# haampie/Homogenization.jl

Hardware: AMD Instinct MI355X
Metric: fine-DOF updates/sec per V-cycle (3D Tet64) (higher is better)
Workload: dtype f64; 1 GPU; 3D Tet64 checkerboard, 32^3 unit cubes x 6 tets, refinements=5 (BASELINE config 3); cells=196608, nf=6545, levels=6, smoothing_steps=3, smoothing_steps_coarse=2, coarse_solver=device CG, Chebyshev(4)-of-Jacobi preconditioner, rtol 1e-13, spare_vector_bytes=10294394880, lazy_top_form=2

## Files before the change

homogenization.jl_amd/csrc/hmg_apply_small.hip:

```cpp
#include "hmg_device.hpp"
#include "hmg_stencil.hpp"

#include <algorithm>
#include <stdexcept>

namespace hmg {

namespace {
constexpr int SW = 15 * WAVE_ROW;

__device__ __forceinline__ uint32_t small_opaque_zero()
{
    uint32_t z;
    asm volatile("v_mov_b32 %0, 0" : "=v"(z));
    return z;
}
}

template <int SPT, bool FUSED>
__global__ void __launch_bounds__(64, SPT == 1 ? 5 : 4)
k_apply_small(LevelDev lv, const uint16_t *__restrict__ dmask, const int32_t *__restrict__ cell_class, ApplyArgs a)
{
    extern __shared__ double smem[];
    double *W = smem;
    double *xs = smem + SW + lv.lds_g0;
    const int lane = threadIdx.x, nf = lv.nf, m = lv.m;
    double *cs = xs + nf + lv.lds_g1;
    const int64_t ld = lv.ld;

    uint32_t pw[SPT], par[SPT];
    int lp[SPT];
    bool has[SPT];
#pragma unroll
    for (int q = 0; q < SPT; ++q) {
        const int t = lane + 64 * q;
        has[q] = t < nf;
        const int tc = has[q] ? t : nf - 1;
        pw[q] = lv.pos32[tc];
        lp[q] = (int)lv.lpos[tc];
        par[q] = FUSED && a.xcoarse ? lv.par32[tc] : 0u;
    }
    for (int q = lane; q < lv.lds_g0; q += 64) smem[SW + q] = 0.0;
    for (int q = lane; q < lv.lds_g1; q += 64) xs[nf + q] = 0.0;
    const bool neg = a.alpha < 0.0;
    double beta = 0.0, ax = 0.0, c2 = 0.0;
    if constexpr (FUSED) {
        beta = a.x2 ? a.scal[a.s_num] / a.scal[a.s_den] : 0.0;
        ax = a.xacc || a.x3 ? a.scal[a.a_num] / a.scal[a.a_den] : 0.0;
        c2 = a.x3 ? a.scal[a.c_num] / a.scal[a.c_den] : 0.0;
    }
    const bool xzero = FUSED && (a.flags & 128);
    const int64_t G = gridDim.x;
    auto cell_of = [&](int64_t blk) -> int64_t { return a.cell_list ? (int64_t)HMG_KP(int32_t, a.cell_list)[blk] : blk; };

    double pwv[4], pxv[SPT], px2[SPT], pxa[SPT], psv[SPT], pcv = 0.0;
    auto issue = [&](int64_t cell, int wsel) {
        const double *wc = lv.wcache + (size_t)wsel * WAVE_WSTRIDE;
#pragma unroll
        for (int q = 0; q < 4; ++q) pwv[q] = wc[lane + 64 * q < SW ? lane + 64 * q : SW - 1];
        const double *xc = a.x + cell * ld;
#pragma unroll
        for (int q = 0; q < SPT; ++q) {
            const int t = has[q] ? lane + 64 * q : nf - 1;
            pxv[q] = xzero ? 0.0 : xc[t];
            if (FUSED && a.x2) px2[q] = a.x2[cell * ld + t];
            if (FUSED && a.xacc)
                pxa[q] = a.xacc[cell * ld + t];
            else if (FUSED && a.x3)
                pxa[q] = a.x3[cell * ld + t];
            if (a.src) psv[q] = a.src[cell * ld + t];
        }
        if (FUSED && a.xcoarse) pcv = a.xcoarse[cell * a.ldc + (lane < lv.nf_coarse ? lane : lv.nf_coarse - 1)];
    };
    struct Uni {
        int wsel;
        uint32_t dm, mq[4];
    };
    auto uniform_of = [&](int64_t cell) {
        Uni u;
        u.wsel = 2 * HMG_KP(int32_t, cell_class)[cell] + (neg ? 1 : 0);
        u.dm = 0u;
        if (a.flags & 1) {
            const uint32_t w2 = HMG_KP(uint32_t, dmask)[cell >> 1];
            u.dm = (cell & 1) ? w2 >> 16 : w2 & 0xffffu;
        }
#pragma unroll
        for (int q = 0; q < 4; ++q) u.mq[q] = FUSED && a.mult ? HMG_KP(uint32_t, a.mult)[cell * 4 + q] : 0x01010101u;
        return u;
    };

    int64_t blk = blockIdx.x;
    if (blk >= a.nwork) return;
    int64_t cell = cell_of(blk);
    Uni cur = uniform_of(cell);
    issue(cell, cur.wsel);
    int64_t cell_n = blk + G < a.nwork ? cell_of(blk + G) : cell;
    Uni nxt = uniform_of(cell_n);

    for (;;) {
        double rr = 0.0, pap = 0.0, sv[SPT];
#pragma unroll
        for (int q = 0; q < 4; ++q)
            if (lane + 64 * q < SW) W[lane + 64 * q] = pwv[q];
        double v[SPT];
        if constexpr (FUSED) {
            if (a.xcoarse && lane < lv.nf_coarse) cs[lane] = pcv;
#pragma unroll
            for (int q = 0; q < SPT; ++q) {
                const int t = lane + 64 * q;
                double val = pxv[q];
                if (a.xcoarse) {
                    const uint32_t pa = par[q] & 0xffffu, pb = par[q] >> 16;
                    const double ca = lds_ld(cs + pa), cb = lds_ld(cs + pb);
                    const double vi = val + ca;
                    double vm = val;
                    vm += 0.5 * ca;
                    vm = vm + 0.5 * cb;
                    val = pa == pb ? vi : vm;
                }
                if (a.xacc && has[q]) a.xacc[cell * ld + t] = axpy1(ax, px2[q], pxa[q]);
                if (a.x3) {
                    const double t1 = axpy1(ax, px2[q], val);
                    const double p2 = axpy1(beta, px2[q], pxa[q]);
                    val = axpy1(c2, p2, t1);
                } else if (a.x2)
                    val = axpy1(beta, px2[q], val);
                if (a.xout && has[q]) a.xout[cell * ld + t] = val;
                if (!has[q]) val = 0.0;
                rr += val * val;
                v[q] = val;
            }
        } else {
#pragma unroll
            for (int q = 0; q < SPT; ++q) v[q] = pxv[q];
        }
#pragma unroll
        for (int q = 0; q < SPT; ++q) {
            if (has[q]) xs[lp[q]] = v[q];
            sv[q] = a.src ? psv[q] : 0.0;
        }
        const Uni me = cur;
        const int64_t mycell = cell;
        const bool more = blk + G < a.nwork;
        if (more) {
            issue(cell_n, nxt.wsel);
            cell = cell_n;
            cur = nxt;
            cell_n = blk + 2 * G < a.nwork ? cell_of(blk + 2 * G) : cell_n;
            nxt = uniform_of(cell_n);
        }
        double *oc = a.out ? a.out + mycell * ld : nullptr;
#pragma unroll
        for (int q = 0; q < SPT; ++q) {
            const uint32_t word = pw[q] | small_opaque_zero();
            int L, len, A, B, cls;
            decode32<3>(word, m, L, len, A, B, cls);
            double ctr;
            double o = stencil_eval_c<3>(W + cls * WAVE_ROW, xs, L, len, A, B, ctr);
            o = sv[q] + o;
            if (cls > 0 && ((me.dm >> (cls - 1)) & 1u)) o = 0.0;
            if (has[q] && (!FUSED || oc)) oc[lane + 64 * q] = o;
            if (FUSED && has[q]) {
                uint32_t mu = 1u;
                if (cls > 0) {
                    const int e = cls - 1;
                    const uint32_t wd = e < 4 ? me.mq[0] : e < 8 ? me.mq[1] : e < 12 ? me.mq[2] : me.mq[3];
                    mu = (wd >> (8 * (e & 3))) & 0xffu;
                }
                pap += (double)mu * (ctr * o);
            }
        }
        if constexpr (FUSED) {
            const double s_pap = wave_sum63(pap), s_rr = wave_sum63(rr);
            if (lane == 63) {
                a.blockpart[2 * mycell] = s_pap;
                a.blockpart[2 * mycell + 1] = s_rr;
            }
        }
        if (!more) break;
        blk += G;
    }
}


template <bool FUSED>
__global__ void __launch_bounds__(64, 4)
k_apply_pack(LevelDev lv, const uint16_t *__restrict__ dmask, const int32_t *__restrict__ cell_class, ApplyArgs a)
{
    extern __shared__ double smem[];
    const int lane = threadIdx.x, sub = lane >> 4, t = lane & 15, nf = lv.nf, m = lv.m;
    const bool has = t < nf;
    const int tc = has ? t : nf - 1;
    const int imgp = lv.lds_g0 + nf + lv.lds_g1;
    double *xs = smem + sub * imgp + lv.lds_g0;
    const int64_t ld = lv.ld;
    for (int q = lane; q < 4 * imgp; q += 64) smem[q] = 0.0;

    int L, len, A, B, cls;
    decode32<3>(lv.pos32[tc], m, L, len, A, B, cls);
    const int lp = (int)lv.lpos[tc];
    const uint32_t par = FUSED && a.xcoarse ? lv.par32[tc] : 0u;
    const int pa = (int)(par & 0xffffu), pb = (int)(par >> 16);
    const int e = cls > 0 ? cls - 1 : 0;
    const bool neg = a.alpha < 0.0;
    double beta = 0.0, ax = 0.0, c2 = 0.0;
    if constexpr (FUSED) {
        beta = a.x2 ? a.scal[a.s_num] / a.scal[a.s_den] : 0.0;
        ax = a.xacc || a.x3 ? a.scal[a.a_num] / a.scal[a.a_den] : 0.0;
        c2 = a.x3 ? a.scal[a.c_num] / a.scal[a.c_den] : 0.0;
    }
    const bool xzero = FUSED && (a.flags & 128);
    const int64_t G = gridDim.x, nquad = (a.nwork + 3) >> 2;

    struct Meta {
        int cell, wsel;
        uint32_t dm, mw;
        bool valid;
    };
    auto meta_of = [&](int64_t Q) {
        Meta mt;
        int64_t w = 4 * Q + sub;
        mt.valid = w < a.nwork;
        if (!mt.valid) w = a.nwork - 1;
        mt.cell = a.cell_list ? a.cell_list[w] : (int)w;
        mt.wsel = 2 * cell_class[mt.cell] + (neg ? 1 : 0);
        mt.dm = (a.flags & 1) ? (uint32_t)dmask[mt.cell] : 0u;
        mt.mw = FUSED && a.mult && cls > 0 ? (uint32_t)a.mult[(int64_t)mt.cell * 16 + e] : 1u;
        return mt;
    };
    double2 pw2[8];
    double pxv = 0.0, px2 = 0.0, pxa = 0.0, psv = 0.0, pca = 0.0, pcb = 0.0;
    auto issue = [&](const Meta &mt) {
        const double2 *wr = reinterpret_cast<const double2 *>(lv.wcache + (size_t)mt.wsel * WAVE_WSTRIDE + cls * WAVE_ROW);
#pragma unroll
        for (int q = 0; q < 8; ++q) pw2[q] = wr[q];
        const int64_t o = (int64_t)mt.cell * ld + tc;
        pxv = xzero ? 0.0 : a.x[o];
        if (FUSED && a.x2) px2 = a.x2[o];
        if (FUSED && a.xacc)
            pxa = a.xacc[o];
        else if (FUSED && a.x3)
            pxa = a.x3[o];
        if (a.src) psv = a.src[o];
        if (FUSED && a.xcoarse) {
            pca = a.xcoarse[(int64_t)mt.cell * a.ldc + pa];
            pcb = a.xcoarse[(int64_t)mt.cell * a.ldc + pb];
        }
    };

    int64_t Q = blockIdx.x;
    if (Q >= nquad) return;
    Meta cur = meta_of(Q);
    issue(cur);
    Meta nxt = meta_of(Q + G < nquad ? Q + G : Q);

    for (;;) {
        const Meta me = cur;
        const int64_t o = (int64_t)me.cell * ld + t;
        const bool live = has && me.valid;
        double w[16];
#pragma unroll
        for (int q = 0; q < 8; ++q) {
            w[2 * q] = pw2[q].x;
            w[2 * q + 1] = pw2[q].y;
        }
        double val = pxv, rr = 0.0, pap = 0.0;
        if constexpr (FUSED) {
            if (a.xcoarse) {
                const double ca = pca, cb = pcb;
                const double vi = val + ca;
                double vm = val;
                vm += 0.5 * ca;
                vm = vm + 0.5 * cb;
                val = pa == pb ? vi : vm;
            }
            if (a.xacc && live) a.xacc[o] = axpy1(ax, px2, pxa);
            if (a.x3) {
                const double t1 = axpy1(ax, px2, val);
                const double p2 = axpy1(beta, px2, pxa);
                val = axpy1(c2, p2, t1);
            } else if (a.x2)
                val = axpy1(beta, px2, val);
            if (a.xout && live) a.xout[o] = val;
            if (!has) val = 0.0;
            rr += val * val;
        }
        if (has) xs[lp] = val;
        const double sv = a.src ? psv : 0.0;
        const bool more = Q + G < nquad;
        if (more) {
            issue(nxt);
            cur = nxt;
            nxt = meta_of(Q + 2 * G < nquad ? Q + 2 * G : Q + G);
        }
        auto at = [&](int off) { return lds_ld(xs + max(L + off, 0)); };
        const double ctr = lds_ld(xs + L);
        double acc = w[0] * ctr;
        acc += w[1] * lds_ld(xs + L + 1);
        acc += w[2] * at(-1);
        acc += w[3] * lds_ld(xs + L + len - 1);
        acc += w[4] * at(-len);
        acc += w[5] * lds_ld(xs + L + len);
        acc += w[6] * at(-len - 1);
        acc += w[7] * lds_ld(xs + L + A - len);
        acc += w[8] * at(len + 1 - B);
        acc += w[9] * lds_ld(xs + L + A - 1);
        acc += w[10] * at(1 - B);
        acc += w[11] * lds_ld(xs + L + A);
        acc += w[12] * at(-B);
        acc += w[13] * lds_ld(xs + L + A + 1 - len);
        acc += w[14] * at(len - B);
        double out = sv + acc;
        if (cls > 0 && ((me.dm >> (cls - 1)) & 1u)) out = 0.0;
        if (live && (!FUSED || a.out)) a.out[o] = out;
        if constexpr (FUSED) {
            if (has) {
                const uint32_t mu = me.mw;
                pap += (double)mu * (ctr * out);
            }
            pap = dpp_add<0x111, 0xf>(pap);
            rr = dpp_add<0x111, 0xf>(rr);
            pap = dpp_add<0x112, 0xf>(pap);
            rr = dpp_add<0x112, 0xf>(rr);
            pap = dpp_add<0x114, 0xf>(pap);
            rr = dpp_add<0x114, 0xf>(rr);
            pap = dpp_add<0x118, 0xf>(pap);
            rr = dpp_add<0x118, 0xf>(rr);
            if (t == 15 && me.valid) {
                a.blockpart[2 * (int64_t)me.cell] = pap;
                a.blockpart[2 * (int64_t)me.cell + 1] = rr;
            }
        }
        if (!more) break;
        Q += G;
    }
}

bool apply_small_ok(const Launch &L, const LevelDev &lv, const MeshDev &mesh, const ApplyArgs &a, bool fused)
{
    if (!L.apply_small || L.apply_threads != 0) return false;
    if (!L.weight_cache || !lv.wcache || !mesh.cell_class) return false;
    if (lv.dim != 3 || lv.ncls != 15 || lv.nf > 192 || lv.nf < 4 || lv.m > 63 || !lv.pos32 || !lv.lpos) return false;
    if (a.flags & (2 | 8 | 16)) return false;
    if (!(a.alpha == 1.0 || a.alpha == -1.0) || a.lambda != mesh.wc_lambda) return false;
    if (a.rcoarse) return false;
    if (!fused) return !a.xcoarse;
    if ((a.x3 || a.xacc) && !a.x2) return false;
    if (a.x3 && a.xacc) return false;
    if (a.xcoarse && (!lv.par32 || lv.nf_coarse < 1 || lv.nf_coarse > 64 || !a.xout || a.x2 || a.xacc || a.x3)) return false;
    return true;
}

void launch_apply_small(const Launch &L, const LevelDev &lv, const MeshDev &mesh, const ApplyArgs &a0, bool fused)
{
    ApplyArgs a = a0;
    const int64_t nblocks = a.cell_list ? a.ncell_list : a.ncells_prefix ? a.ncells_prefix : mesh.ncells;
    if (nblocks == 0) return;
    if (!a.x) throw std::runtime_error("operator apply: null input vector");
    if (!fused && !a.out) throw std::runtime_error("operator apply: a plain launch needs an output vector");
    if (fused && (!a.blockpart || !a.scal)) throw std::runtime_error("operator apply: fused launch without its reduction scratch");
    if ((a.flags & 1) && !mesh.dmask) throw std::runtime_error("operator apply: constraint requested without a Dirichlet mask");
    if ((a.flags & 128) && !(fused && a.x3 && a.x2 && a.xout && !a.xcoarse))
        throw std::runtime_error("operator apply: the zero-input form exists for the residual with two pending x-updates only");
    a.nwork = nblocks;
    if (lv.nf <= 16 && L.apply_pack && nblocks >= 4 && nblocks < (int64_t(1) << 31)) {
        const int64_t nquad = (nblocks + 3) / 4;
        const dim3 gq((unsigned)std::min<int64_t>(nquad, (int64_t)16 * L.num_cu)), bq(64);
        const size_t ldsq = sizeof(double) * (size_t)(4 * (lv.lds_g0 + lv.nf + lv.lds_g1) + 64);
        if (fused)
            hipLaunchKernelGGL((k_apply_pack<true>), gq, bq, ldsq, L.stream, lv, mesh.dmask, mesh.cell_class, a);
        else
            hipLaunchKernelGGL((k_apply_pack<false>), gq, bq, ldsq, L.stream, lv, mesh.dmask, mesh.cell_class, a);
        check_launch();
        if (L.n_small_launches) *L.n_small_launches += 1;
        return;
    }
    const int64_t grid = std::min<int64_t>(nblocks, (int64_t)(lv.nf > 64 ? 16 : 20) * L.num_cu);
    const size_t lds = sizeof(double) * (size_t)(SW + lv.lds_g0 + lv.nf + lv.lds_g1 + 64);
    const dim3 g((unsigned)grid), b(64);
    if (lv.nf > 64) {
        if (fused)
            hipLaunchKernelGGL((k_apply_small<3, true>), g, b, lds, L.stream, lv, mesh.dmask, mesh.cell_class, a);
        else
            hipLaunchKernelGGL((k_apply_small<3, false>), g, b, lds, L.stream, lv, mesh.dmask, mesh.cell_class, a);
    } else {
        if (fused)
            hipLaunchKernelGGL((k_apply_small<1, true>), g, b, lds, L.stream, lv, mesh.dmask, mesh.cell_class, a);
        else
            hipLaunchKernelGGL((k_apply_small<1, false>), g, b, lds, L.stream, lv, mesh.dmask, mesh.cell_class, a);
    }
    check_launch();
    if (L.n_small_launches) *L.n_small_launches += 1;
}

}
```

homogenization.jl_amd/csrc/hmg_apply_wave.hip:

```cpp
#include "hmg_device.hpp"
#include "hmg_stencil.hpp"

#include <algorithm>
#include <stdexcept>
#include <type_traits>

namespace hmg {

namespace {

__device__ __forceinline__ uint32_t opaque_zero()
{
    uint32_t z;
    asm volatile("v_mov_b32 %0, 0" : "=v"(z));
    return z;
}

__device__ __forceinline__ void wdecode(uint32_t w, int &L, int &len, int &A, int &B)
{
    L = (int)(w & 1023u);
    len = (int)((w >> 10) & 31u);
    A = (int)((w >> 15) & 255u);
    B = (int)((w >> 23) & 255u);
}
// ... 246 lines not shown
                using T_ = std::true_type;
                using F_ = std::false_type;
                if (x3c) {
                    if (xzero)
                        general(F_{}, T_{}, T_{}, std::integral_constant<int, 8>{});
                    else
                        general(F_{}, T_{}, F_{}, std::integral_constant<int, 8>{});
                } else if (xac)
                    general(T_{}, F_{}, F_{}, std::integral_constant<int, 8>{});
                else
                    general(F_{}, F_{}, F_{}, std::integral_constant<int, 16>{});
            }
        }

        double *oc = a.out ? a.out + cell * ld : nullptr;
        double kf[8], kec[2], ki[3][WR];
        __builtin_amdgcn_sched_barrier(0);
        issue_src_interior();
        __builtin_amdgcn_sched_barrier(0);
        {
            const double fm0 = (double)(mq[0] & 0xffu), fm1 = (double)((mq[0] >> 8) & 0xffu), fm2 = (double)((mq[0] >> 16) & 0xffu),
                         fm3 = (double)(mq[0] >> 24);
            wave_face<0, FUSED, FUSED && !RS, SRC>(wc + 1 * WAVE_ROW, xs, TW(0), TW(1), (dm >> 0) & 1u, fm0, sf[0], sf[1], oc, pap, lane, kf[0], kf[1]);
            wave_face<1, FUSED, FUSED && !RS, SRC>(wc + 2 * WAVE_ROW, xs, TW(2), TW(3), (dm >> 1) & 1u, fm1, sf[2], sf[3], oc, pap, lane, kf[2], kf[3]);
            wave_face<2, FUSED, FUSED && !RS, SRC>(wc + 3 * WAVE_ROW, xs, TW(4), TW(5), (dm >> 2) & 1u, fm2, sf[4], sf[5], oc, pap, lane, kf[4], kf[5]);
            wave_face<3, FUSED, FUSED && !RS, SRC>(wc + 4 * WAVE_ROW, xs, TW(6), TW(7), (dm >> 3) & 1u, fm3, sf[6], sf[7], oc, pap, lane, kf[6], kf[7]);
        }
#pragma unroll
        for (int r = 0; r < 2; ++r) {
            const int t = r * 64 + lane;
            const bool valid = t < WNEC;
            const int cls = (int)((TW(14) >> (16 + 8 * r)) & 0xffu);
            const double sv = SRC ? sec[r] : 0.0;
            int L, len, A, B;
            wdecode(TW(8 + r), L, len, A, B);
            double ctr;
            double o = stencil_eval_c<3>(smem + (cls - 5) * WAVE_ROW, xs, L, len, A, B, ctr);
            o = sv + o;
            if ((dm >> (cls - 1)) & 1u) o = 0.0;
            if (valid && (!FUSED || oc)) oc[t] = o;
            if (FUSED && !RS && valid) {
                const int e = cls - 1;
                const uint32_t word = e < 4 ? mq[0] : e < 8 ? mq[1] : e < 12 ? mq[2] : mq[3];
                const uint32_t mu = (word >> (8 * (e & 3))) & 0xffu;
                pap += (double)mu * (ctr * o);
            }
            kec[r] = o;
        }
        {
            double w0[15];
#pragma unroll
            for (int d = 0; d < 15; ++d) w0[d] = wc[d];
#pragma unroll
            for (int r = 0; r < 3; ++r) {
                const uint32_t word = TW(10 + r);
                const int slot0 = (int)(r == 0 ? TW(13) & 0xffffu : r == 1 ? TW(13) >> 16 : TW(14) & 0xffffu);
                if (r < 2 || lane < WNBLK - 128) {
                    const int nv = (int)(word >> 28);
#pragma unroll
                    for (int q = 0; q < WR; ++q) ki[r][q] = SRC && q < nv ? si[r][q] : 0.0;
                    interior_block_core<WR, FUSED, false, RS>(w0, xs, WM, WNF >> 1, word, slot0, oc, pap, ki[r]);
                }
            }
        }

        if constexpr (RS) {
#pragma unroll
            for (int f = 0; f < 8; ++f)
                if (!(f & 1) || lane < WNFI - 64) xs[TW(f) & 1023u] = kf[f];
#pragma unroll
            for (int r = 0; r < 2; ++r)
                if (r * 64 + lane < WNEC) xs[TW(8 + r) & 1023u] = kec[r];
#pragma unroll
            for (int r = 0; r < 3; ++r)
                if (r < 2 || lane < WNBLK - 128) {
                    int pos[WR];
                    block_positions<WR>(WM, TW(10 + r), pos);
                    const int nv = (int)(TW(10 + r) >> 28);
#pragma unroll
                    for (int q = 0; q < WR; ++q)
                        if (q < nv) xs[pos[q]] = ki[r][q];
                }
            double *rc = a.rcoarse + cell * a.ldrc;
#pragma unroll
            for (int q = 0; q < 3; ++q) {
                const int c = lane + 64 * q;
                if (c < WNFC) {
                    const uint4 ta = reinterpret_cast<const uint4 *>(lv.wave_rs)[2 * c];
                    const uint4 tb = reinterpret_cast<const uint4 *>(lv.wave_rs)[2 * c + 1];
                    const uint32_t e[8] = {ta.x, ta.y, ta.z, ta.w, tb.x, tb.y, tb.z, tb.w};
                    const int n = (int)(e[7] >> 16);
                    double tmp = 0.0;
                    tmp += 1.0 * lds_ld(xs + (e[0] & 0xffffu));
#pragma unroll
                    for (int u = 1; u < 15; ++u) {
                        const double t2 = tmp + 0.5 * lds_ld(xs + ((u & 1) ? e[u >> 1] >> 16 : e[u >> 1] & 0xffffu));
                        tmp = u < n ? t2 : tmp;
                    }
                    rc[c] = tmp;
                }
            }
        }
        if (FUSED && !RS) {
            const double s_pap = wave_sum63(pap), s_rr = wave_sum63(rr);
            if (lane == 63) {
                a.blockpart[2 * cell] = s_pap;
                a.blockpart[2 * cell + 1] = s_rr;
            }
        }
    }
}

__global__ void __launch_bounds__(256)
k_weight_cache(LevelDev lv, const double *__restrict__ coef_rep, int64_t nsets, double lambda, double *__restrict__ wcache)
{
    for (int64_t set = blockIdx.x; set < nsets; set += gridDim.x) {
        const int64_t cls = set >> 1;
        const double alpha = (set & 1) ? -1.0 : 1.0;
        double s[7];
        cell_scales<3>(coef_rep + (size_t)cls * 8, alpha, lambda, s, 0);
        double *out = wcache + (size_t)set * WAVE_WSTRIDE;
        for (int idx = threadIdx.x; idx < 15 * WAVE_ROW; idx += 256) {
            const int c = idx / WAVE_ROW, d = idx % WAVE_ROW;
            double w = 0.0;
            if (c < lv.ncls && d < 15) {
                const double *ct = lv.ctab + ((size_t)c * 15 + d) * 7;
#pragma unroll
                for (int t = 0; t < 7; ++t) w += ct[t] * s[t];
            }
            out[idx] = w;
        }
    }
}

void launch_weight_cache(const Launch &L, const LevelDev &lv, const double *coef_rep, int nclasses, double lambda, double *wcache)
{
    if (nclasses <= 0) return;
    if (lv.dim != 3 || lv.ncls != 15 || lv.ndir != 15 || lv.nterm != 7) throw std::runtime_error("weight cache: not a 3D level");
    const int64_t nsets = 2 * (int64_t)nclasses;
    const int64_t grid = std::min<int64_t>(nsets, (int64_t)1 << 20);
    hipLaunchKernelGGL(k_weight_cache, dim3((unsigned)grid), dim3(256), 0, L.stream, lv, coef_rep, nsets, lambda, wcache);
    check_launch();
}

bool apply_wave_ok(const Launch &L, const LevelDev &lv, const MeshDev &mesh, const ApplyArgs &a, bool fused)
{
    if (!L.apply_wave || L.apply_threads != 0) return false;
    if (!lv.wave_tab || !lv.wave_lpos || !lv.wcache || !mesh.cell_class) return false;
    if (lv.dim != 3 || lv.m != WM || lv.nf != WNF || lv.nfi != WNFI || lv.nei != WNEI || lv.ncorner != WNCORNER || lv.nedge != 6 ||
        lv.nface != 4 || lv.nblk != WNBLK || lv.blk_R != WR || lv.off_edge != WOFF_EDGE || lv.off_face != WOFF_FACE ||
        lv.lds_g0 != 0 || lv.lds_g1 < WM + 8 || lv.lds_g1 > 64 || lv.ncls != 15)
        return false;
    if (a.flags & (2 | 8 | 16)) return false;
    if (!(a.alpha == 1.0 || a.alpha == -1.0) || a.lambda != mesh.wc_lambda) return false;
    if (!fused) return !a.xcoarse && !a.rcoarse;
    if (a.xcoarse && a.rcoarse) return false;
    if ((a.x3 || a.xacc) && !(a.x2 && a.xout)) return false;
    if (a.xcoarse) return a.src && a.xout && lv.wave_par && lv.wave_cl && lv.nf_coarse == WNFC && !a.x2 && !a.xacc && !a.x3;
    if (a.rcoarse) return a.src && lv.wave_rs && lv.nf_coarse == WNFC;
    return true;
}

void launch_apply_wave(const Launch &L, const LevelDev &lv, const MeshDev &mesh, const ApplyArgs &a0, bool fused)
{
    ApplyArgs a = a0;
    const int64_t nblocks = a.cell_list ? a.ncell_list : a.ncells_prefix ? a.ncells_prefix : mesh.ncells;
    if (nblocks == 0) return;
    if (!a.x) throw std::runtime_error("operator apply: null input vector");
    if (!fused && !a.out) throw std::runtime_error("operator apply: a plain launch needs an output vector");
    if (fused && (!a.blockpart || !a.scal)) throw std::runtime_error("operator apply: fused launch without its reduction scratch");
    if ((a.flags & 1) && !mesh.dmask) throw std::runtime_error("operator apply: constraint requested without a Dirichlet mask");
    if (a.xcoarse && !a.xout) throw std::runtime_error("operator apply: folded prolongation without xout");
    if (a.rcoarse && a.ldrc <= 0) throw std::runtime_error("operator apply: epilogue restriction without the coarse column stride");
    if ((a.flags & 128) && !(fused && a.x3 && a.x2 && a.xout && !a.xcoarse))
        throw std::runtime_error("operator apply: the zero-input form exists for the residual with two pending x-updates only");
    a.nwork = nblocks;
    if (L.cell_order && !a.cell_list && !a.ncells_prefix && mesh.cell_perm) {
        a.cell_list = mesh.cell_perm;
        a.ncell_list = nblocks;
    }
    int64_t grid = std::min<int64_t>(nblocks, L.wave_grid > 0 ? L.wave_grid : 16 * (int64_t)L.num_cu);
    if (grid >= 8) grid -= grid % 8;
    const size_t lds = sizeof(double) * (size_t)(WVZ + WNF + lv.lds_g1);
    const dim3 g((unsigned)grid), b(64);
#define HMG_WAVE_LAUNCH(F, C, R, S) \
    hipLaunchKernelGGL((k_apply_wave<F, C, R, S>), g, b, lds, L.stream, lv, mesh.dmask, mesh.cell_class, a)
    if (!fused) {
        if (a.src)
            HMG_WAVE_LAUNCH(false, false, false, true);
        else
            HMG_WAVE_LAUNCH(false, false, false, false);
    } else if (a.xcoarse)
        HMG_WAVE_LAUNCH(true, true, false, true);
    else if (a.rcoarse)
        HMG_WAVE_LAUNCH(true, false, true, true);
    else if (a.src)
        HMG_WAVE_LAUNCH(true, false, false, true);
    else
        HMG_WAVE_LAUNCH(true, false, false, false);
#undef HMG_WAVE_LAUNCH
    check_launch();
    if (L.n_wave_launches) *L.n_wave_launches += 1;
}

}
```

homogenization.jl_amd/csrc/hmg_context.cpp:

```cpp
#include "../../include/hmg.h"
#include "hmg_objects.hpp"

#include <algorithm>

namespace hmg {

std::recursive_mutex &lifetime_mutex()
{
    static std::recursive_mutex m;
    return m;
}

std::atomic<int64_t> &device_allocs()
{
    static std::atomic<int64_t> n{0};
    return n;
}

namespace {

void vec_pool_trim(hmg_ctx *c)
{
    LifetimeLock lock(lifetime_mutex());
    if (c->vec_pool.empty()) return;
// ... 97 lines not shown
}

}

void grid_unref(hmg_grid *grid)
{
    LifetimeLock lock(lifetime_mutex());
    if (!grid || --grid->refs > 0) return;
    hmg_ctx *c = grid->ctx;
    if (c) {
        (void)hipSetDevice(c->device);
        (void)hipStreamSynchronize(c->stream);
    }
    probe_unlist(grid);
    release_top_spare(grid);
    release_weight_cache(grid);
    release_smoother_diag(grid);
    if (grid->probe && grid->probe->h) (void)hipHostFree(grid->probe->h);
    if (grid->probe && grid->probe->ev) (void)hipEventDestroy(grid->probe->ev);
    delete grid;
    ctx_unref(c);
}

double read_scalar(hmg_ctx *c, int slot)
{
    double h = 0.0;
    HIPCHK(hipMemcpyAsync(&h, c->L.scal + slot, sizeof(double), hipMemcpyDeviceToHost, c->stream));
    HIPCHK(hipStreamSynchronize(c->stream));
    judge_probes(c);
    return h;
}

}

extern "C" {

const char *hmg_last_error(void) { return last_error().c_str(); }
int hmg_version(void) { return 1; }

static int ctx_create(int device, void *stream, bool use_given, hmg_ctx **out)
{
    HMG_TRY
    need(out != nullptr, "null out pointer");
    int ndev = 0;
    hipError_t e = hipGetDeviceCount(&ndev);
    if (e != hipSuccess || ndev == 0)
        throw std::runtime_error("no HIP device available: libhmg_hip needs an MI355X (gfx950); there is no CPU fallback");
    need(device >= 0 && device < ndev, "device index out of range");
    HIPCHK(hipSetDevice(device));
    std::unique_ptr<hmg_ctx> c(new hmg_ctx);
    c->device = device;
    if (use_given) {
        c->stream = (hipStream_t)stream;
    } else {
        HIPCHK(hipStreamCreateWithFlags(&c->stream, hipStreamNonBlocking));
        c->own_stream = true;
    }
    hipDeviceProp_t prop;
    HIPCHK(hipGetDeviceProperties(&prop, device));
    c->partials.alloc(4096);
    c->scal.alloc(S_COUNT);
    HIPCHK(hipMemsetAsync(c->scal.p, 0, S_COUNT * sizeof(double), c->stream));
    c->L.stream = c->stream;
    c->L.partials = c->partials.p;
    c->L.rpart = nullptr;
    c->L.rpart_cap = 0;
    c->L.scal = c->scal.p;
    c->L.num_cu = prop.multiProcessorCount > 0 ? prop.multiProcessorCount : 256;
    c->L.apply_threads = 0;
    c->L.apply_mass_only = 0;
    c->L.cell_order = 1;
    c->L.weight_cache = 1;
    c->L.apply_wave = 1;
    c->L.wave_grid = 16 * (int64_t)c->L.num_cu;
    c->L.n_wave_launches = &c->wave_launches;
    c->L.apply_slab2 = 1;
    c->L.n_slab2_launches = &c->slab2_launches;
    c->L.n_rows_launches = &c->rows_launches;
    c->L.slab2_grid = 0;
    c->L.slab2_force = 0;
    c->L.restrict_slab2 = 1;
    c->L.apply_pack = 1;
    c->L.apply_small = 1;
    c->L.n_small_launches = &c->small_launches;
    c->L.n_wc_launches = &c->wc_launches;
    c->L.apply_wg512 = 1;
    {
        LifetimeLock lock(lifetime_mutex());
        live_contexts().push_back(c.get());
    }
    *out = c.release();
    HMG_END
}

int hmg_ctx_create(int device, void *stream, hmg_ctx **out) { return ctx_create(device, stream, stream != nullptr, out); }

int hmg_ctx_create_on_stream(int device, void *stream, hmg_ctx **out) { return ctx_create(device, stream, true, out); }

int hmg_ctx_destroy(hmg_ctx *ctx)
{
    HMG_TRY
    ctx_unref(ctx);
    HMG_END
}

int hmg_ctx_sync(hmg_ctx *ctx)
{
    HMG_TRY
    need(ctx != nullptr, "null ctx");
    HIPCHK(hipStreamSynchronize(ctx->stream));
    judge_probes(ctx);
    HMG_END
}

int64_t hmg_ctx_counter(hmg_ctx *ctx, const char *name)
{
    if (!ctx || !name) return -1;
    const std::string n(name);
    if (n == "wave_launches") return ctx->wave_launches;
    if (n == "slab2_launches") return ctx->slab2_launches;
    if (n == "rows_launches") return ctx->rows_launches;
    if (n == "small_launches") return ctx->small_launches;
    if (n == "weight_cache_launches") return ctx->wc_launches;
    if (n == "comm_calls") return ctx->comm_calls;
    if (n == "device_allocs") return device_allocs().load();
    if (n == "spare_bytes") return ctx->spare_bytes;
    if (n == "weight_cache_classes") return ctx->wc_classes;
    if (n == "weight_cache_bytes") return ctx->wc_bytes;
    if (n == "weight_cache_refusals") return ctx->wc_refusals;
    if (n == "fcg_bytes") return ctx->fcg_bytes;
    if (n == "smoother_diag_bytes") return ctx->smoother_diag_bytes;
    if (n == "smoother_diag_builds") return ctx->smoother_diag_builds;
    if (n == "lazy_top_form") return ctx->last_top_form;
    if (n == "lazy_pre_form") return ctx->last_pre_form;
    if (n == "coarse_x_folds") return ctx->coarse_x_folds;
    if (n == "cell_moments_kernel_ns") return ctx->moments_kernel_ns;
    if (n == "cell_moments_download_ns") return ctx->moments_download_ns;
    if (n == "comm_nranks") return ctx->comm ? ctx->comm_nranks : 0;
    return -1;
}

int hmg_ctx_release_memory(hmg_ctx *ctx)
{
    HMG_TRY
    need(ctx != nullptr, "null ctx");
    vec_pool_trim(ctx);
    HMG_END
}

int hmg_ctx_set_option(hmg_ctx *ctx, const char *name, int64_t value)
{
    HMG_TRY
    need(ctx && name, "null argument");
    std::string n(name);
    static const std::pair<const char *, bool hmg_ctx::*> flags[] = {
        {"coarse_probe", &hmg_ctx::coarse_probe}, {"fuse_cg", &hmg_ctx::fuse_cg_default}, {"fold_x", &hmg_ctx::fold_x},
        {"swap_rp", &hmg_ctx::swap_rp}, {"fold_prolong", &hmg_ctx::fold_prolong}, {"zero_entry", &hmg_ctx::zero_entry},
        {"fold_restrict", &hmg_ctx::fold_restrict}, {"lazy_dead", &hmg_ctx::lazy_dead}, {"lazy_pre", &hmg_ctx::lazy_pre}, {"fold_coarse_x", &hmg_ctx::fold_coarse_x}, {"fold_faces", &hmg_ctx::fold_faces},
        {"lean_post", &hmg_ctx::lean_post}, {"lazy_post", &hmg_ctx::lazy_post}, {"prolong_in_image", &hmg_ctx::prolong_in_image},
        {"comm_rehearsal", &hmg_ctx::comm_rehearsal}};
    for (const auto &f : flags)
        if (n == f.first) {
            ctx->*f.second = value != 0;
            return 0;
        }
    if (n == "apply_threads")
        ctx->L.apply_threads = (int)value;
    else if (n == "apply_wg512")
        ctx->L.apply_wg512 = value != 0;
    else if (n == "apply_pack")
        ctx->L.apply_pack = value != 0;
    else if (n == "apply_small")
        ctx->L.apply_small = value != 0;
    else if (n == "weight_cache")
        ctx->L.weight_cache = value != 0;
    else if (n == "weight_cache_classes")
        ctx->wc_max_classes = std::max<int64_t>(0, value);
    else if (n == "apply_slab2")
        ctx->L.apply_slab2 = value != 0;
    else if (n == "restrict_slab2")
        ctx->L.restrict_slab2 = value != 0;
    else if (n == "slab2_force")
        ctx->L.slab2_force = value != 0;
    else if (n == "slab2_grid")
        ctx->L.slab2_grid = std::max<int64_t>(0, value);
    else if (n == "apply_wave")
        ctx->L.apply_wave = value != 0;
    else if (n == "wave_grid")
        ctx->L.wave_grid = std::max<int64_t>(1, value) * (int64_t)ctx->L.num_cu;
    else if (n == "wave_grid_total")
        ctx->L.wave_grid = std::max<int64_t>(1, value);
    else if (n == "cell_order")
        ctx->L.cell_order = value != 0;
    else if (n == "coarse_poly")
        ctx->coarse_poly = std::max<int>(1, std::min<int>(16, (int)value));
    else if (n == "coarse_maxit")
        ctx->coarse_maxit = (int)value;
    else if (n == "coarse_check")
        ctx->coarse_check = std::max<int>(1, (int)value);
    else if (n == "lazy_top")
        ctx->lazy_top = (int)value;
    else if (n == "overlap_min_doubles")
        ctx->overlap_min_doubles = value;
    else if (n == "vec_pool") {
        ctx->vec_pool_on = value != 0;
        if (!ctx->vec_pool_on) vec_pool_trim(ctx);
    }
    else if (n == "time_apply") {
        ctx->timer.on = value > 0;
        ctx->timer.min_level = (int)value;
        ctx->timer.used = 0;
        ctx->timer.ev_level.clear();
        ctx->timer.ev_bytes.clear();
    }
    else
        throw std::runtime_error("unknown option: " + n);
    HMG_END
}

int hmg_ctx_set_option_f64(hmg_ctx *ctx, const char *name, double value)
{
    HMG_TRY
    need(ctx && name, "null argument");
    std::string n(name);
    if (n == "coarse_rtol")
        ctx->coarse_rtol = value;
    else if (n == "coarse_poly_ratio")
        ctx->coarse_poly_ratio = value;
    else
        throw std::runtime_error("unknown option: " + n);
    HMG_END
}

void *hmg_ctx_scalar_bank(hmg_ctx *ctx) { return ctx ? (void *)ctx->L.scal : nullptr; }

int hmg_ctx_set_scalar_bank(hmg_ctx *ctx, void *device_doubles16)
{
    HMG_TRY
    need(ctx != nullptr, "null argument");
    HIPCHK(hipStreamSynchronize(ctx->stream));
    double *to = device_doubles16 ? (double *)device_doubles16 : ctx->scal.p;
    if (to != ctx->L.scal) HIPCHK(hipMemcpy(to, ctx->L.scal, S_COUNT * sizeof(double), hipMemcpyDeviceToDevice));
    ctx->L.scal = to;
    HMG_END
}

static int apply_timing(hmg_ctx *ctx, bool every, int level, int64_t *launches, double *total_ms, double *total_bytes)
{
    HMG_TRY
    need(ctx && launches && total_ms && total_bytes, "null argument");
    HIPCHK(hipStreamSynchronize(ctx->stream));
    const ApplyTimer &tm = ctx->timer;
    double ms = 0.0, by = 0.0;
    int64_t n = 0;
// ... 93 lines not shown
```

homogenization.jl_amd/csrc/hmg_device.hpp:

```cpp
#pragma once
#include <hip/hip_runtime.h>

#include <cstdint>

namespace hmg {

constexpr int TABLE_PAD = 3 * 1024;

__host__ __device__ inline int rows_slot(int m, int i, int j, int nei, int off_int, int &cls)
{
    if (j == 0) {
        cls = i == 0 ? 4 : i == m ? 5 : 1;
        return i == 0 ? 0 : i == m ? 1 : 3 + i - 1;
    }
    if (i == 0) {
        cls = j == m ? 6 : 2;
        return j == m ? 2 : 3 + nei + j - 1;
    }
    if (i + j == m) {
        cls = 3;
        return 3 + 2 * nei + j - 1;
    }
    cls = 0;
    return off_int + (j - 1) * (m - 1) - (((j - 1) * j) >> 1) + i - 1;
}

struct LevelDev {
    int dim, level, m;
    int nf, ld;
    int ncorner, nedge, nface;
    int nei, nfi, nint;
    int off_edge, off_face, off_int;
    int ncls, ndir, nterm;
    int lds_g0, lds_g1;
    int nf_coarse;
    const uint64_t *meta;
    const uint16_t *lpos;
    const uint16_t *sweep_slot;
    int nsweep;
    const uint32_t *pos32;
    const uint32_t *pos32w;
    const uint32_t *sweep32;
    const uint32_t *blk_word;
    const uint16_t *blk_slot;
    int nblk, blk_R;
    const double *ctab;
    const int32_t *hier2slot;
    const int32_t *par_a, *par_b;
    const uint32_t *par32;
    const uint64_t *par64;
    const uint16_t *clpos;
    const uint32_t *rs_word;
    const double *rs_w;
    const uint16_t *rs_lp;
    const int32_t *rptr, *ridx;
    const double *dphi;
    const uint32_t *wave_tab;
    const uint32_t *wave_lpos;
    const uint32_t *wave_par;
    const uint32_t *wave_cl;
    const uint32_t *wave_rs;
    const double *wcache;
};

constexpr int WM = 16, WNF = 969, WNFI = 105, WNEI = 15, WNCORNER = 4, WNBLK = 152, WNFC = 165, WR = 4;
constexpr int WOFF_EDGE = 4, WOFF_FACE = 94, WNEC = 94;
constexpr int WNQ = 16;
constexpr int WVZ = 168;
constexpr int WAVE_TAB_ROWS = 15;
constexpr int WAVE_ROW = 16;
constexpr int WAVE_WSTRIDE = 15 * WAVE_ROW;

struct SlabTables {
    const int *head;
    const uint32_t *ld_word;
    const uint32_t *cp_word;
    const uint16_t *cp_slot;
    int nslab, lds_nodes;
    int max_surf;
    int max_int;
};

struct MeshDev {
    int dim;
    int64_t ncells, nnodes;
    const int32_t *cells;
    const int32_t *face_pairs;
    int64_t nfacepairs;
    const int32_t *face_partner;
    const int32_t *edge_ptr, *edge_ent;
    int64_t nsharededges;
    const int32_t *node_ptr, *node_ent;
    int64_t nsharednodes;
    const int32_t *node_first;
    const uint16_t *dmask, *dupmask;
    const double *coef;
    int64_t ncut_edge_groups, ncut_node_groups;
    int64_t ncut_face_pairs;
    const int32_t *cells_cut, *cells_inner;
    const int32_t *cell_perm;
    int64_t ncells_cut, ncells_inner;
    const uint8_t *mult;
    const int32_t *cell_class;
    int nclasses;
    double wc_lambda;
    double *blockpart;
    SlabTables slab;
};

struct ApplyArgs {
    double alpha, lambda;
    const double *x;
    const double *x2;
    double *xout;
    double *xacc;
    int a_num, a_den;
    const double *x3;
    int c_num, c_den;
    const double *x4;
    int d_num, d_den;
    const double *xcoarse;
    int64_t ldc;
    const double *xc_p, *xc_r;
    const double *src;
    double *out;
    double *rcoarse;
    int64_t ldrc;
    const double *scal;
    int s_num, s_den;
    double *blockpart;
    const uint8_t *mult;
    int flags;
    int64_t ncells_prefix;
    int64_t out_ld;
    const int32_t *cell_list;
    int64_t ncell_list;
    int64_t nwork;
    const int32_t *cell_class;
};

struct CoarseDev {
    int64_t n;
    const int32_t *rowptr, *colidx;
    const double *val, *diag;
    const int32_t *interior;
};

enum { S_RS = 0, S_PAP = 1, S_RS2 = 2, S_TMP = 3, S_C0 = 4, S_C1 = 5, S_C2 = 6, S_C3 = 7, S_PAP2 = 8, S_DONE = 9, S_ITER = 10,
       S_CRR = 11, S_HOST = 12, S_COUNT = 16,
       S_RS3 = S_C1, S_PAP3 = S_TMP };

struct Launch {
    hipStream_t stream;
    double *partials;
    double *rpart;
    int64_t rpart_cap;
    double *scal;
    int num_cu;
    int apply_threads;
    int apply_mass_only;
    int apply_wg512;
    int cell_order;
    int weight_cache;
    int apply_pack;
    int apply_small;
    int64_t *n_small_launches;
    int64_t *n_wc_launches;
    int apply_wave;
    int64_t wave_grid;
    int64_t *n_wave_launches;
    int apply_slab2;
    int64_t *n_slab2_launches;
    int64_t slab2_grid;
    int restrict_slab2;
    int slab2_force;
    int64_t *n_rows_launches;
};

void launch_apply(const Launch &L, const LevelDev &lv, const MeshDev &mesh, double alpha, double lambda,
                  const double *x, const double *src, double *out, int use_mask);
size_t apply_lds_bytes(const LevelDev &lv);
bool apply_restricts(const Launch &L, const LevelDev &lv);
bool apply_folds_coarse_x(const Launch &L, const LevelDev &lv);
bool apply_defers3(const Launch &L, const LevelDev &lv);
void launch_apply_fused_kernel(const Launch &L, const LevelDev &lv, const MeshDev &mesh, ApplyArgs a);
void launch_apply_fused_reduce(const Launch &L, const MeshDev &mesh, int slot_pap, int slot_rr);
void launch_apply_args(const Launch &L, const LevelDev &lv, const MeshDev &mesh, ApplyArgs a);
bool apply_wave_ok(const Launch &L, const LevelDev &lv, const MeshDev &mesh, const ApplyArgs &a, bool fused);
void launch_apply_wave(const Launch &L, const LevelDev &lv, const MeshDev &mesh, const ApplyArgs &a, bool fused);
bool apply_slab2_ok(const Launch &L, const LevelDev &lv, const MeshDev &mesh, const ApplyArgs &a);
void launch_apply_slab2(const Launch &L, const LevelDev &lv, const MeshDev &mesh, const ApplyArgs &a, bool fused);
void launch_apply_rows(const Launch &L, const LevelDev &lv, const MeshDev &mesh, const ApplyArgs &a, bool fused, bool wd);
void launch_prolong_add_wide(const Launch &L, const LevelDev &fine, const LevelDev &coarse, int64_t ncells, const double *xc,
                             double *xf);
int64_t launch_norm2_unique_wide(const Launch &L, const LevelDev &lv, const MeshDev &mesh, const double *x);
bool apply_small_ok(const Launch &L, const LevelDev &lv, const MeshDev &mesh, const ApplyArgs &a, bool fused);
void launch_apply_small(const Launch &L, const LevelDev &lv, const MeshDev &mesh, const ApplyArgs &a, bool fused);
void launch_weight_cache(const Launch &L, const LevelDev &lv, const double *coef_rep, int nclasses, double lambda, double *wcache);

void launch_interface_sum(const Launch &L, const LevelDev &lv, const MeshDev &mesh, double *x, int which = 0,
                          bool faces = true);
void launch_mask(const Launch &L, const LevelDev &lv, const MeshDev &mesh, double *x, int which );
void launch_restrict_slab(const Launch &L, const LevelDev &fine_rtab, const MeshDev &mesh, const SlabTables &st, int ldc,
                          const double *rf, double *bc);
void launch_restrict(const Launch &L, const LevelDev &fine, const LevelDev &coarse, int64_t ncells,
                     const double *rf, double *bc);
void launch_prolong_add(const Launch &L, const LevelDev &fine, const LevelDev &coarse, int64_t ncells,
                        const double *xc, double *xf);

void launch_fill(const Launch &L, double *x, int64_t n, double v);
void launch_copy(const Launch &L, double *dst, const double *src, int64_t n);
void launch_axpy(const Launch &L, double a, const double *x, double *y, int64_t n);
void launch_xpby(const Launch &L, const double *r, double b, double *p, int64_t n);
void launch_dot(const Launch &L, const double *x, const double *y, int64_t n, int slot);
void launch_norm2_unique(const Launch &L, const LevelDev &lv, const MeshDev &mesh, const double *x, int slot);
void launch_copy_dot(const Launch &L, double *p, const double *r, int64_t n, int slot);
void launch_cg_update(const Launch &L, double *x, double *r, const double *p, const double *q, int64_t n,
                      int s_num, int s_den, int s_out);
void launch_cg_rupdate(const Launch &L, const double *r, double *rout, const double *q, int64_t n, int s_num, int s_den,
                       int s_out);
void launch_cg_rupdate_faces(const Launch &L, const LevelDev &lv, const MeshDev &mesh, const double *r, double *rout,
                             const double *q, int64_t n, int s_num, int s_den, int s_out);
void launch_cg_rupdate_faces_x(const Launch &L, const LevelDev &lv, const MeshDev &mesh, const double *r, double *rout,
                               const double *q, int64_t n, int s_num, int s_den, int s_out, double *x, const double *p, int a_num,
                               int a_den, int b_num, int b_den, const double *p0, int z_num, int z_den);
void launch_cg_xp_update(const Launch &L, double *x, double *p, const double *r, int64_t n, int a_num, int a_den,
                         int s_num, int s_den, int with_p);
void launch_cg_x2_update(const Launch &L, double *x, const double *p, const double *r, int64_t n, int a_num, int a_den, int b_num,
                         int b_den, int c_num, int c_den);
void launch_cg_pupdate(const Launch &L, double *p, const double *r, int64_t n, int s_num, int s_den);

void launch_gather_base(const Launch &L, const MeshDev &mesh, int ld1, const double *v1, double *u);
void launch_scatter_base(const Launch &L, const MeshDev &mesh, int ld1, const double *u, double *v1);

void launch_gather_owned(const Launch &L, const MeshDev &mesh, const int32_t *nodes_g, const int32_t *owned, int ld1,
                         const double *v1, double *ug);
void launch_scatter_cells(const Launch &L, const int32_t *cell_nodes, int64_t ncells, int npc, int ld1, const double *u,
                          double *v1);

void launch_permute(const Launch &L, const LevelDev &lv, int64_t ncells, const double *src, double *dst,
                    int to_storage);
void launch_fill_random(const Launch &L, const LevelDev &lv, int64_t ncells, double *x, uint64_t seed,
                        int64_t cell_offset);

void launch_coarse_gather_rhs(const Launch &L, const CoarseDev &A, const double *u, double *b);
void launch_coarse_scatter_sol(const Launch &L, const CoarseDev &A, int64_t nnodes, const double *x, double *u);
void launch_coarse_init(const Launch &L, const CoarseDev &A, const double *b, double *x, double *r, double *z,
                        double *p, double zscale = 1.0, double *dcheb = nullptr);
void launch_coarse_cheb(const Launch &L, const CoarseDev &A, const double *r, const double *zin, double *zout, double *d, double c1,
                        double c2, int last);
void launch_coarse_rz_from_cheb(const Launch &L, const CoarseDev &A);
void launch_coarse_update(const Launch &L, const CoarseDev &A, double *x, double *r, double *z, const double *p,
                          const double *q, int slot_old, double zscale = 1.0, double *dcheb = nullptr);
void launch_coarse_residual_norm(const Launch &L, const CoarseDev &A);
void launch_coarse_direction(const Launch &L, const CoarseDev &A, double *p, double *q, const double *z, int slot_old, int slot_new,
                             double rtol2, int mode, int count_it, int rz_from_cheb = 0);

void launch_rhs_dphi(const Launch &L, const LevelDev &lv, int64_t ncells, const double *pvec, double *b);

void launch_integrate(const Launch &L, const LevelDev &lv, const MeshDev &mesh, int mode, int64_t nsub, const double *v,
                      const double *second, int slot);
void launch_integrate_load(const Launch &L, const LevelDev &lv, const MeshDev &mesh, int64_t nsub, const double *v,
                           const double *load, int slot);

struct CutPackArgs {
    int64_t n[3];
    const int64_t *pos[3];
    const int32_t *cell_lid[3];
    const uint8_t *first[3];
};
void launch_cut_pack(const Launch &L, const LevelDev &lv, const CutPackArgs &c, double *buf, double *x, int unpack);
void launch_seg_sum(const Launch &L, const int64_t *plan, int64_t ndoubles, double *buf, const double *stage);

}
```

homogenization.jl_amd/csrc/hmg_host.hpp:

```cpp
#pragma once
#include <algorithm>
#include <cstdint>
#include <string>
#include <thread>
#include <vector>

namespace hmg {

int setup_threads();

template <class F>
void parallel_for(int64_t n, F f)
{
    const int T = (int)std::max<int64_t>(1, std::min<int64_t>(setup_threads(), n / 4096));
    if (T == 1) {
        f((int64_t)0, n);
        return;
    }
    std::vector<std::thread> th;
    for (int t = 0; t < T; ++t) th.emplace_back([&, t] { f(n * t / T, n * (t + 1) / T); });
    for (auto &x : th) x.join();
}

template <class T, class Cmp>
// ... 68 lines not shown
    int dim = 0;
    int64_t nnodes = 0, ncells = 0;
    std::vector<double> coords;
    std::vector<int32_t> cells;

    std::vector<int32_t> face_pairs;
    std::vector<int32_t> edge_ptr, edge_ent;
    std::vector<int32_t> node_ptr, node_ent;
    std::vector<int32_t> node_first;
    std::vector<int32_t> node_all_ptr, node_all_ent;
    std::vector<uint16_t> dmask, dupmask;
    std::vector<uint8_t> mult;
    std::vector<uint8_t> node_on_boundary;

    int64_t ncut_edge_groups = 0, ncut_node_groups = 0;
    int64_t ncut_face_pairs = 0;
    std::vector<int32_t> cells_cut, cells_inner;

    std::vector<double> detj, jinv;
};

void build_mesh_tables(int dim, int64_t nnodes, const double *coords, int64_t ncells,
                       const int64_t *cells_1based, MeshTables &out);

void restrict_mesh_tables(const MeshTables &full, int64_t ncells_prefix, int64_t nnodes_prefix,
                          MeshTables &out);

inline int sym_ncomp(int dim) { return dim * (dim + 1) / 2; }
inline int sym_index(int dim, int a, int b)
{
    if (a > b) std::swap(a, b);
    return a * dim - a * (a - 1) / 2 + (b - a);
}
void build_cell_coefficients(const MeshTables &mesh, const double *sigma, int sn, std::vector<double> &coef);

struct CoarseMatrix {
    int64_t n = 0;
    std::vector<int32_t> interior;
    std::vector<int32_t> node2int;
    std::vector<int32_t> rowptr, colidx;
    std::vector<double> val, diag;
};
void assemble_coarse_matrix(const MeshTables &mesh, const double *sigma, int sn, double lambda,
                            CoarseMatrix &out);


struct AddressTables {
    std::vector<uint16_t> lpos;
    std::vector<uint32_t> pos32;
    std::vector<uint32_t> pos32w;
    std::vector<uint32_t> sweep32;
    std::vector<uint16_t> sweep_slot;
};
AddressTables build_address_tables(const LevelTables &T);

struct BlockedInterior {
    int nblk = 0, R = 0;
    std::vector<uint32_t> word;
    std::vector<uint16_t> slot;
};
BlockedInterior build_blocked_interior(const LevelTables &T);

struct SlabWindows {
    int nslab = 0, lds_nodes = 0, max_surf = 0, max_int = 0;
    std::vector<int> head;
    std::vector<uint32_t> ld_word;
    std::vector<uint32_t> cp_word;
    std::vector<uint16_t> cp_slot;
    int rs_max_surf = 0, rs_max_int = 0;
    std::vector<int> rs_head;
    std::vector<uint32_t> rs_word;
    std::vector<uint16_t> rs_slot;
    std::vector<double> rtab;
};
SlabWindows build_slab_windows(const LevelTables &T, const LevelTables *coarse, int lds_kb);

struct TransferTables {
    std::vector<uint32_t> par32;
    std::vector<uint16_t> clpos;
    std::vector<uint64_t> par64;
    std::vector<uint32_t> rs_word;
    std::vector<double> rs_w;
    std::vector<uint16_t> rs_lp;
};
TransferTables build_transfer_tables(const LevelTables &T, const LevelTables *coarse, const BlockedInterior &blk);

struct WaveTables {
    std::vector<uint32_t> tab, lpos, par, cl, rs;
};
WaveTables build_wave_tables(const LevelTables &T, const LevelTables *coarse, const BlockedInterior &blk,
                             const std::vector<uint16_t> &clpos);

struct MeshKernelTables {
    std::vector<int32_t> face_partner;
    std::vector<uint16_t> dmask;
    std::vector<int32_t> cell_perm;
    std::vector<int32_t> cells_cut, cells_inner;
};
MeshKernelTables build_mesh_kernel_tables(const MeshTables &M, bool xcd_lists);

struct Partition {
    int rank = 0, nranks = 1;
    MeshTables global;
    std::vector<int32_t> cells_g;
    std::vector<int32_t> nodes_g;
    std::vector<int32_t> owned_node;
    int64_t nglobal[3] = {0, 0, 0};
    std::vector<int64_t> gid[3];
    std::vector<int32_t> cell_lid[3];
    bool global_ids = true;
    struct Segment {
        std::vector<int32_t> members;
        int64_t count[3] = {0, 0, 0};
    };
    std::vector<Segment> segs;
    std::vector<int32_t> seg_of[3];
    std::vector<int64_t> seg_idx[3];
};

void build_partition(int dim, int64_t nnodes, const double *coords, int64_t ncells, const int64_t *cells_1based,
                     const int32_t *owner, int rank, int nranks, MeshTables &local, Partition &part,
                     const int32_t *cut_owner = nullptr, bool halo_only = false);

std::string &last_error();

}
```

homogenization.jl_amd/csrc/hmg_kernel_tables.cpp:

```cpp
#include "hmg_device.hpp"
#include "hmg_host.hpp"

#include <algorithm>
#include <numeric>
#include <stdexcept>
#include <utility>

namespace hmg {

namespace {

uint32_t word32w(uint32_t i, uint32_t j, uint32_t k, uint32_t c) { return (i & 127u) | (j & 127u) << 7 | (k & 127u) << 14 | c << 21; }

uint32_t word_lattice(uint32_t L, uint32_t j, uint32_t k) { return L | ((j & 127u) << 16) | ((k & 127u) << 23); }

uint32_t lattice_pos(const LevelTables &T, int slot) { return (uint32_t)(T.meta[(size_t)slot] & 0xffffu); }

struct LatticeIndex {
    int n;
    std::vector<int32_t> slot;
    explicit LatticeIndex(const LevelTables &T) : n(T.m + 1), slot((size_t)n * n * (T.dim == 3 ? n : 1), -1)
    {
        for (int q = 0; q < T.nf; ++q) slot[idx(T.slot_ijk[3 * q], T.slot_ijk[3 * q + 1], T.slot_ijk[3 * q + 2])] = q;
    }
// ... 127 lines not shown
    for (int e = 0; e < T.nedge; ++e) seg.push_back({T.off_edge + e * T.nei, T.off_edge + (e + 1) * T.nei});
    for (int f = 0; f < T.nface; ++f) seg.push_back({T.off_face + f * T.nfi, T.off_face + (f + 1) * T.nfi});
    seg.push_back({T.off_int, T.nf});
    auto run = [&](std::pair<int, int> sg, int ka, int kb) {
        auto in = [&](int t) { return T.slot_ijk[3 * t + 2] >= ka && T.slot_ijk[3 * t + 2] < kb; };
        int b = sg.second, e = sg.first;
        for (int t = sg.first; t < sg.second; ++t)
            if (in(t)) { b = std::min(b, t); e = t + 1; }
        for (int t = b; t < e; ++t)
            if (!in(t)) throw std::runtime_error("apply slabs: plane range is not contiguous");
        return b < e ? std::make_pair(b, e) : std::make_pair(0, 0);
    };
    S.head.assign((size_t)S.nslab * 8, 0);
    for (int sl = 0; sl < S.nslab; ++sl) {
        S.head[sl * 8 + 0] = sk[sl];
        S.head[sl * 8 + 1] = (int)S.ld_word.size();
        for (const auto &sg : seg) {
            const auto ld = run(sg, sl == 0 ? 0 : sk[sl] + 1, sk[sl + 1] + 1);
            for (int t = ld.first; t < ld.second; ++t) S.ld_word.push_back(lattice_pos(T, t) | ((uint32_t)t << 16));
        }
        S.head[sl * 8 + 2] = (int)S.ld_word.size() - S.head[sl * 8 + 1];
    }
    auto eval_lists = [&](std::vector<int> &head, std::vector<uint32_t> &word, std::vector<uint16_t> &slot, int &max_surf,
                          int &max_int, auto out) {
        for (int sl = 0; sl < S.nslab; ++sl) {
            int *h = &head[(size_t)sl * 8];
            h[3] = (int)word.size();
            for (size_t si = 0; si < seg.size(); ++si) {
                const bool interior = si + 1 == seg.size();
                if (interior) h[5] = (int)word.size() - h[3];
                const auto cp = run(seg[si], sk[sl], sk[sl + 1]);
                for (int t = cp.first; t < cp.second; ++t) {
                    const int o = out(t);
                    if (o < 0) continue;
                    const uint32_t i = T.slot_ijk[3 * t], j = T.slot_ijk[3 * t + 1], k = T.slot_ijk[3 * t + 2];
                    word.push_back(interior ? word_lattice(lattice_pos(T, t), j, k) : word32w(i, j, k, T.slot_cls[t]));
                    slot.push_back((uint16_t)o);
                }
            }
            h[4] = (int)word.size() - h[3];
            max_surf = std::max(max_surf, h[5]);
            max_int = std::max(max_int, h[4] - h[5]);
        }
    };
    eval_lists(S.head, S.cp_word, S.cp_slot, S.max_surf, S.max_int, [](int t) { return t; });
    if ((int)S.ld_word.size() != T.nf || (int)S.cp_word.size() != T.nf)
        throw std::runtime_error("apply slabs: the slab lists do not cover the cell exactly once");
    for (int sl = 0; sl < S.nslab; ++sl)
        for (int q = S.head[sl * 8 + 3] + S.head[sl * 8 + 5] + 1; q < S.head[sl * 8 + 3] + S.head[sl * 8 + 4]; ++q)
            if (S.cp_slot[(size_t)q] != S.cp_slot[(size_t)q - 1] + 1)
                throw std::runtime_error("apply slabs: interior slots of a slab are not consecutive");
    S.ld_word.resize(S.ld_word.size() + TABLE_PAD, 0u);
    S.cp_word.resize(S.cp_word.size() + TABLE_PAD, 0u);
    S.cp_slot.resize(S.cp_slot.size() + TABLE_PAD, (uint16_t)0);
    if (!coarse) return S;
    const LatticeIndex cslot(*coarse);
    S.rs_head = S.head;
    eval_lists(S.rs_head, S.rs_word, S.rs_slot, S.rs_max_surf, S.rs_max_int, [&](int t) {
        const int i = T.slot_ijk[3 * t], j = T.slot_ijk[3 * t + 1], k = T.slot_ijk[3 * t + 2];
        if ((i | j | k) & 1) return -1;
        const int cs = cslot(i / 2, j / 2, k / 2);
        if (cs < 0) throw std::runtime_error("slab restriction: even node without a coarse slot");
        return cs;
    });
    if ((int)S.rs_word.size() != coarse->nf) throw std::runtime_error("slab restriction: lists do not cover the coarse cell");
    S.rs_word.resize(S.rs_word.size() + TABLE_PAD, 0u);
    S.rs_slot.resize(S.rs_slot.size() + TABLE_PAD, (uint16_t)0);
    S.rtab.assign(T.ctab.size(), 0.0);
    for (int c = 0; c < T.ncls; ++c)
        for (int d = 0; d < T.ndir; ++d) S.rtab[((size_t)c * T.ndir + d) * T.nterm + T.nterm - 1] = restriction_weight(T, c, d);
    return S;
}

TransferTables build_transfer_tables(const LevelTables &T, const LevelTables *coarse, const BlockedInterior &blk)
{
    TransferTables X;
    if (!coarse || coarse->nf <= 0x10000) {
        X.par32.resize(T.par_a.size());
        for (size_t q = 0; q < X.par32.size(); ++q) {
            if ((uint32_t)T.par_a[q] > 0xffffu || (uint32_t)T.par_b[q] > 0xffffu) throw std::runtime_error("coarse slot exceeds 16 bits");
            X.par32[q] = (uint32_t)T.par_a[q] | ((uint32_t)T.par_b[q] << 16);
        }
    }
    if (!(coarse && T.dim == 3 && blk.nblk > 0 && T.nf <= 0xffff)) return X;
    const LevelTables &C = *coarse;
    const LatticeIndex fslot(T);
    X.clpos.resize((size_t)C.nf);
    X.rs_word.resize((size_t)C.nf);
    for (int c = 0; c < C.nf; ++c) {
        const int i = 2 * C.slot_ijk[3 * c], j = 2 * C.slot_ijk[3 * c + 1], k = 2 * C.slot_ijk[3 * c + 2];
        const int fs = fslot(i, j, k);
        if (fs < 0) throw std::runtime_error("prolongation tables: coarse node without a fine lattice node");
        if (i > 127 || j > 127 || k > 127) throw std::runtime_error("restriction tables: bad coarse node");
        X.clpos[c] = (uint16_t)lattice_pos(T, fs);
        X.rs_word[c] = word32w(i, j, k, T.slot_cls[fs]);
    }
    X.par64.resize((size_t)T.nf);
    for (int q = 0; q < T.nf; ++q) {
        const uint64_t a = X.clpos[(size_t)T.par_a[q]], b = X.clpos[(size_t)T.par_b[q]], self = lattice_pos(T, q);
        if (T.par_a[q] == T.par_b[q] && a != self) throw std::runtime_error("prolongation tables: identity row off its node");
        X.par64[q] = a | (b << 16) | (self << 32);
    }
    X.rs_w.resize((size_t)T.ncls * T.ndir);
    for (int c = 0; c < T.ncls; ++c)
        for (int d = 0; d < T.ndir; ++d) X.rs_w[(size_t)c * T.ndir + d] = restriction_weight(T, c, d);
    if (T.nf <= 2048) {
        X.rs_lp.resize(T.ridx.size());
        for (size_t e = 0; e < X.rs_lp.size(); ++e) X.rs_lp[e] = (uint16_t)lattice_pos(T, T.ridx[e]);
    }
    return X;
}

WaveTables build_wave_tables(const LevelTables &T, const LevelTables *coarse, const BlockedInterior &blk,
                             const std::vector<uint16_t> &clpos)
{
    WaveTables W;
    if (!(T.dim == 3 && T.m == WM && T.nf == WNF && blk.nblk == WNBLK && blk.R == WR && T.lds_g0 == 0 && T.nfi == WNFI &&
          T.nei == WNEI && T.ncorner == WNCORNER && T.nedge == 6 && T.nface == 4 && T.off_edge == WOFF_EDGE &&
          T.off_face == WOFF_FACE))
        return W;
    const int m = T.m, WDUMMY = WVZ - 1;
    auto surf_word = [&](int t, bool valid) -> uint32_t {
        const uint32_t L = lattice_pos(T, t);
        const int j = T.slot_ijk[3 * t + 1], k = T.slot_ijk[3 * t + 2];
        const int len = m + 1 - j - k, n = m - k, Tk = (n + 1) * (n + 2) / 2, A = Tk - j, Bo = Tk + n + 2 - j;
        if (L > 1023u || len < 0 || len > 31 || A < 0 || A > 255 || Bo < 0 || Bo > 255)
            throw std::runtime_error("wave tables: addressing word out of range");
        return L | ((uint32_t)len << 10) | ((uint32_t)A << 15) | ((uint32_t)Bo << 23) | (valid ? 1u << 31 : 0u);
    };
    W.tab.assign((size_t)WAVE_TAB_ROWS * 64, 0u);
    W.lpos.assign(8 * 64, 0u);
    for (int l = 0; l < 64; ++l) {
        for (int r = 0; r < 8; ++r) {
            const int f = r >> 1, ti = (r & 1) * 64 + l;
            const bool valid = ti < WNFI;
            W.tab[(size_t)r * 64 + l] = surf_word(WOFF_FACE + f * WNFI + (valid ? ti : 0), valid);
        }
        uint32_t cls[2];
        for (int r = 0; r < 2; ++r) {
            const int t = r * 64 + l;
            const bool valid = t < WNEC;
            W.tab[(size_t)(8 + r) * 64 + l] = surf_word(valid ? t : 0, valid);
            cls[r] = T.slot_cls[(size_t)(valid ? t : WOFF_EDGE)];
            if (cls[r] < 5 || cls[r] > 14) throw std::runtime_error("wave tables: edge / corner class out of range");
        }
        uint32_t bsl[3];
        for (int r = 0; r < 3; ++r) {
            const int u = r * 64 + l;
            const bool valid = u < WNBLK;
            W.tab[(size_t)(10 + r) * 64 + l] = valid ? blk.word[(size_t)u] : (blk.word[0] & 0x0fffffffu);
            bsl[r] = blk.slot[(size_t)(valid ? u : 0)];
        }
        W.tab[(size_t)13 * 64 + l] = bsl[0] | (bsl[1] << 16);
        W.tab[(size_t)14 * 64 + l] = bsl[2] | (cls[0] << 16) | (cls[1] << 24);
        for (int q = 0; q < WNQ; ++q) {
            const int t = l + 64 * q;
            W.lpos[(size_t)(q / 2) * 64 + l] |= 8u * (uint32_t)(t < WNF ? WVZ + (int)lattice_pos(T, t) : WDUMMY) << (16 * (q & 1));
        }
    }
    if (!(coarse && !clpos.empty() && coarse->nf == WNFC)) return W;
    W.par.assign(16 * 64, 0u);
    W.cl.assign(3 * 64, 8u * (uint32_t)WDUMMY);
    W.rs.assign((size_t)192 * 8, 0u);
    for (int t = 0; t < T.nf; ++t) W.par[(size_t)t] = (uint32_t)clpos[(size_t)T.par_a[t]] | ((uint32_t)clpos[(size_t)T.par_b[t]] << 16);
    for (int c = 0; c < coarse->nf; ++c) {
        W.cl[(size_t)c] = 8u * (uint32_t)(WVZ + clpos[(size_t)c]);
// ... 31 lines not shown
```

homogenization.jl_amd/csrc/hmg_kernels.hip:

```cpp
#include "hmg_device.hpp"
#include "hmg_stencil.hpp"

#include <cstdio>
#include <stdexcept>
#include <string>

namespace hmg {

__global__ void __launch_bounds__(256) k_finalize(const double *__restrict__ partials, int n, double *scal, int slot)
{
    __shared__ double red[4];
    double v = 0.0;
    for (int i = threadIdx.x; i < n; i += 256) v += partials[i];
    double s = block_sum(v, red);
    if (threadIdx.x == 0) scal[slot] = s;
}

#ifdef HMG_PHASE_TIMING
#define HMG_STAMP(i)                                                                     \
    do {    \
        if (a.blockpart && !a.cell_list && tid == 0)                                     \
            a.blockpart[2 * (size_t)a.nwork + 8 * cell + (i)] = (double)wall_clock64(); \
    } while (0)
#define HMG_SLAB_T0() const long long _t0 = wall_clock64(); long long _tl = _t0; double _ph[5] = {0, 0, 0, 0, 0}
#define HMG_SLAB_PHASE(i)                              \
    do {                                               \
        const long long _n = wall_clock64();           \
        _ph[i] += (double)(_n - _tl);                  \
        _tl = _n;                                      \
    } while (0)
#define HMG_SLAB_STORE()                                                                      \
    do {                                                                                      \
        if (a.blockpart && tid == 0) {                                                        \
            double *_o = a.blockpart + 2 * (size_t)a.nwork + 8 * cell;                        \
            _o[0] = (double)_t0;                                                              \
            for (int _q = 0; _q < 5; ++_q) _o[1 + _q] = _ph[_q];                              \
            _o[6] = (double)wall_clock64();                                                   \
        }                                                                                     \
    } while (0)
#else
#define HMG_STAMP(i)
#define HMG_SLAB_T0()
#define HMG_SLAB_PHASE(i)
#define HMG_SLAB_STORE()
#endif

template <int DIM, int NT, int SPT, bool FUSED, int RB, bool WD = false, bool CG = false, bool RS = false, bool WC = false, int LF = 0>
__global__ void __launch_bounds__(NT, NT >= 640 ? 8 : RB && NT == 512 ? 6 : 1)
k_apply(LevelDev lv, const double *__restrict__ coef, const uint16_t *__restrict__ dmask, ApplyArgs a)
{
    constexpr int NDIR = DIM == 3 ? 15 : 7;
    constexpr int NTERM = DIM == 3 ? 7 : 4;
    constexpr int WS = RB ? WSZ_RB : WSZ;
    extern __shared__ double smem[];
    double *W = smem;
    double *xs = smem + WS + lv.lds_g0;
    const int tid = threadIdx.x;
    constexpr bool LOOP = NT == 64;
    int64_t blk = blockIdx.x;
    do {
    const int64_t cell = a.cell_list ? (int64_t)a.cell_list[blk] : blk;
    const int nf = lv.nf;
    HMG_STAMP(0);

    size_t wbase16 = 0;
    if constexpr (WC) wbase16 = (size_t)(2 * HMG_KP(int32_t, a.cell_class)[cell] + (a.alpha < 0.0 ? 1 : 0)) * WAVE_WSTRIDE;
    const double cv = RB && !WC ? coef[cell * 8 + (tid & 7)] : 0.0;
    if (!RB && (tid >= NT - 256 || NT <= 256)) {
        const int first = NT <= 256 ? tid : tid - (NT - 256);
        const int step = NT <= 256 ? NT : 256;
        if constexpr (WC) {
            for (int idx = first; idx < lv.ncls * NDIR; idx += step)
                W[idx] = lv.wcache[wbase16 + (size_t)((idx / NDIR) * WAVE_ROW + idx % NDIR)];
        } else {
        double s[NTERM];
        cell_scales<DIM>(coef + cell * 8, a.alpha, a.lambda, s, a.flags);
        for (int idx = first; idx < lv.ncls * NDIR; idx += step) {
            const double *c = lv.ctab + (size_t)idx * NTERM;
            double w = 0.0;
#pragma unroll
            for (int t = 0; t < NTERM; ++t) w += c[t] * s[t];
            W[idx] = w;
        }
        }
    }
    for (int q = tid; q < lv.lds_g0; q += NT) smem[WS + q] = 0.0;
    for (int q = tid; q < lv.lds_g1; q += NT) xs[nf + q] = 0.0;
    const int m = lv.m;
    constexpr int NW = NT / 64, WPF = NW / 4 > 0 ? NW / 4 : 1, NE = NW >= 6 ? 1 : 2;
    constexpr int FI = RB && NT == 512 ? 4 : 2;
    constexpr int NPASS = RB && NT == 512 ? 2 : 1;
    constexpr bool EARLY = RB && (NT <= 256 || WC);
    const int wave = tid >> 6, lane = tid & 63;
    const int face = wave / WPF, ft0 = (wave % WPF) * (FI * 64);
    int edge[NE], ebase[NE];
#pragma unroll
    for (int q = 0; q < NE; ++q) {
        edge[q] = NW - 1 - wave + q * NW;
        if (edge[q] >= lv.nedge) edge[q] = -1;
        ebase[q] = lv.off_edge + (edge[q] < 0 ? 0 : edge[q]) * lv.nei;
    }
    uint32_t fw[FI], ew[NE][1], cw = 0u;
#pragma unroll
    for (int q = 0; q < FI; ++q) fw[q] = 0u;
    uint32_t p0 = 0u, p1 = 0u;
    double wv = 0.0;
    double c7[NTERM];
    uint32_t q0 = 0u, q1 = 0u;
    int s0 = 0, s1 = 0;
    uint32_t mq[4] = {0, 0, 0, 0};
    uint32_t mqr[4] = {0, 0, 0, 0};
    uint32_t dm = 0u;
    const uint32_t *iw = RB ? lv.blk_word : lv.sweep32;
    const uint16_t *is = RB ? lv.blk_slot : lv.sweep_slot;
    double cwl = 0.0;
    auto issue_rows = [&]() {
        if constexpr (WC) {
            if (a.flags & 1) {
                const uint32_t w2 = HMG_KP(uint32_t, dmask)[cell >> 1];
                dm = (cell & 1) ? w2 >> 16 : w2 & 0xffffu;
            }
            if (RB) {
                int row = 0;
                if (lane < 15)
                    row = lane;
                else if (lane >= 16 && lane < 31)
                    row = (1 + face) * WAVE_ROW + lane - 16;
                else if (lane >= 32 && lane < 47 && edge[0] >= 0)
                    row = (1 + lv.nface + edge[0]) * WAVE_ROW + lane - 32;
                else if (NE > 1 && lane >= 48 && lane < 63 && edge[NE - 1] >= 0)
                    row = (1 + lv.nface + edge[NE - 1]) * WAVE_ROW + lane - 48;
                wv = lv.wcache[wbase16 + row];
                if (wave == NW - 1) {
                    const int cl = lane < 60 ? lane : 59;
                    cwl = lv.wcache[wbase16 + (1 + lv.nface + lv.nedge + cl / 15) * WAVE_ROW + cl % 15];
                }
            }
            if (FUSED && a.mult) {
#pragma unroll
                for (int q = 0; q < 4; ++q) mqr[q] = HMG_KP(uint32_t, a.mult)[cell * 4 + q];
            }
            return;
        }
        dm = (a.flags & 1) ? dmask[cell] : 0u;
        if (RB) {
            int row = 0;
            if (lane < 15)
                row = lane;
            else if (lane >= 16 && lane < 31)
                row = (1 + face) * NDIR + lane - 16;
            else if (lane >= 32 && lane < 47 && edge[0] >= 0)
                row = (1 + lv.nface + edge[0]) * NDIR + lane - 32;
            else if (NE > 1 && lane >= 48 && lane < 63 && edge[NE - 1] >= 0)
                row = (1 + lv.nface + edge[NE - 1]) * NDIR + lane - 48;
#pragma unroll
            for (int t = 0; t < NTERM; ++t) c7[t] = lv.ctab[(size_t)row * NTERM + t];
        }
        if (FUSED && a.mult) {
            const uint32_t *mp = reinterpret_cast<const uint32_t *>(a.mult + cell * 16);
#pragma unroll
            for (int q = 0; q < 4; ++q) mqr[q] = mp[q];
        }
    };
    auto issue_words = [&]() {
        if (RB) {
#pragma unroll
            for (int q = 0; q < FI; ++q) {
                const int ti = ft0 + q * 64 + lane;
                if (ti < lv.nfi) fw[q] = lv.pos32[lv.off_face + face * lv.nfi + ti];
            }
// ... 355 lines not shown
    for (int d = 0; d < NDIR; ++d) w0[d] = RB ? readlane_f64(wv, d) : to_sgpr(W[d]);
    if (RB) {
        if constexpr (!RS) {
        if (DIM == 3 && tid < nsw) {
            if (sc)
                interior_block<RB ? RB : 1, FUSED, true>(w0, xs, m, nf >> 1, q0, s0, sc, oc, pap, wdot, wself);
            else
                interior_block<RB ? RB : 1, FUSED, false>(w0, xs, m, nf >> 1, q0, s0, sc, oc, pap);
        }
        if (DIM == 3 && NPASS > 1 && tid + NT < nsw) {
            if (sc)
                interior_block<RB ? RB : 1, FUSED, true>(w0, xs, m, nf >> 1, q1, s1, sc, oc, pap, wdot, wself);
            else
                interior_block<RB ? RB : 1, FUSED, false>(w0, xs, m, nf >> 1, q1, s1, sc, oc, pap);
        }
        }
    } else {
        const int nit_sweep = (nsw + NT - 1) / NT;
        for (int it = 0; it < nit_sweep; ++it) {
            const int u = tid + it * NT;
            const uint32_t pw = q0;
            const int t = s0;
            q0 = q1;
            s0 = s1;
            q1 = iw[u + 2 * NT];
            s1 = (int)is[u + 2 * NT];
            if (t != 0xffff) {
                const double sv = sc ? sc[t] : 0.0;
                int L, len, A, B, cls;
                decode32<DIM>(pw, m, L, len, A, B, cls);
                double ctr;
                double o = stencil_eval_v<DIM>(w0, xs + L, len, A, B, ctr);
                if (!wdot) o = sv + o;
                if (!FUSED || oc) oc[t] = o;
                if (FUSED) pap += (wdot ? fma(wself, ctr, sv) : ctr) * o;
            }
        }
    }
    HMG_STAMP(5);
    if constexpr (RS && RB != 0 && DIM == 3) {
        int fl[FI], el[NE], cl = 0;
        uint32_t b0 = 0u, b1 = 0u;
        if (face < 4) {
#pragma unroll
            for (int q = 0; q < FI; ++q) {
                const int ti = ft0 + q * 64 + lane;
                fl[q] = ti < lv.nfi ? (int)lv.lpos[lv.off_face + face * lv.nfi + ti] : 0;
            }
        }
#pragma unroll
        for (int q = 0; q < NE; ++q) el[q] = edge[q] >= 0 && lane < lv.nei ? (int)lv.lpos[ebase[q] + lane] : 0;
        if (wave == NW - 1 && lane < lv.ncorner) cl = (int)lv.lpos[lane];
        if (tid < nsw) b0 = lv.blk_word[tid];
        if (NPASS > 1 && tid + NT < nsw) b1 = lv.blk_word[tid + NT];
        __syncthreads();
        if (face < 4) {
#pragma unroll
            for (int q = 0; q < FI; ++q)
                if (ft0 + q * 64 + lane < lv.nfi) xs[fl[q]] = kf[q];
        }
#pragma unroll
        for (int q = 0; q < NE; ++q)
            if (edge[q] >= 0 && lane < lv.nei) xs[el[q]] = ke[q];
        if (wave == NW - 1 && lane < lv.ncorner) xs[cl] = kc;
        {
            int pos[RB ? RB : 1];
            if (tid < nsw) {
                block_positions<RB ? RB : 1>(m, b0, pos);
                const int nv = (int)(b0 >> 28);
#pragma unroll
                for (int r = 0; r < (RB ? RB : 1); ++r)
                    if (r < nv) xs[pos[r]] = ki[0][r];
            }
            if (NPASS > 1 && tid + NT < nsw) {
                block_positions<RB ? RB : 1>(m, b1, pos);
                const int nv = (int)(b1 >> 28);
#pragma unroll
                for (int r = 0; r < (RB ? RB : 1); ++r)
                    if (r < nv) xs[pos[r]] = ki[NPASS - 1][r];
            }
        }
        __syncthreads();
        double *rc = a.rcoarse + cell * a.ldrc;
        if (lv.rs_lp) {
            for (int c = tid; c < lv.nf_coarse; c += NT) {
                const int b = lv.rptr[c], n = lv.rptr[c + 1] - b;
                int lp[15];
#pragma unroll
                for (int q = 0; q < 15; ++q) lp[q] = lv.rs_lp[b + (q < n ? q : 0)];
                double tmp = 0.0;
                tmp += 1.0 * lds_ld(xs + lp[0]);
#pragma unroll
                for (int q = 1; q < 15; ++q)
                    if (q < n) tmp += 0.5 * lds_ld(xs + lp[q]);
                rc[c] = tmp;
            }
        } else
        for (int c = tid; c < lv.nf_coarse; c += NT) {
            int L, len, A, B, cls, k;
            decode32w(lv.rs_word[c], m, L, len, A, B, cls, k);
            const double *w = lv.rs_w + cls * NDIR;
            auto at = [&](int off) { return lds_ld(xs + max(L + off, 0)); };
            double acc = w[0] * lds_ld(xs + L);
            acc += w[1] * lds_ld(xs + L + 1);
            acc += w[2] * at(-1);
            acc += w[3] * lds_ld(xs + L + len - 1);
            acc += w[4] * at(-len);
            acc += w[5] * lds_ld(xs + L + len);
            acc += w[6] * at(-len - 1);
            acc += w[7] * lds_ld(xs + L + A - len);
            acc += w[8] * at(len + 1 - B);
            acc += w[9] * lds_ld(xs + L + A - 1);
            acc += w[10] * at(1 - B);
            acc += w[11] * lds_ld(xs + L + A);
            acc += w[12] * at(-B);
            acc += w[13] * lds_ld(xs + L + A + 1 - len);
            acc += w[14] * at(len - B);
            rc[c] = 0.0 + acc;
        }
    }
    if (FUSED && !RS) {
        __syncthreads();
        const double s_pap = block_sum(pap, smem);
        const double s_rr = block_sum(rr, smem);
        if (tid == 0) {
            a.blockpart[2 * cell] = s_pap;
            a.blockpart[2 * cell + 1] = s_rr;
        }
    }
    HMG_STAMP(6);
    if (LOOP) {
        blk += gridDim.x;
        if (blk >= a.nwork) break;
        __syncthreads();
    }
    } while (LOOP);
}

template <int DIM, int NT, bool FUSED, bool WD = false>
__global__ void __launch_bounds__(NT, 8)
k_apply_slab(LevelDev lv, const double *__restrict__ coef, const uint16_t *__restrict__ dmask, ApplyArgs a, SlabTables st)
{
    constexpr int NDIR = DIM == 3 ? 15 : 7;
    constexpr int NTERM = DIM == 3 ? 7 : 4;
    constexpr int HB = FUSED ? 3 : 4;
    constexpr int MV = 5;
    extern __shared__ double smem[];
    double *W = smem;
    double *img = smem + WSZ;
    const int tid = threadIdx.x;
    const int64_t cell = a.cell_list ? (int64_t)a.cell_list[blockIdx.x] : (int64_t)blockIdx.x;
    const int m = lv.m;

    if (a.flags & 4) {
        for (int idx = tid; idx < lv.ncls * NDIR; idx += NT) W[idx] = lv.ctab[(size_t)idx * NTERM + NTERM - 1];
    } else {
        double s[NTERM];
        cell_scales<DIM>(coef + cell * 8, a.alpha, a.lambda, s, a.flags);
        for (int idx = tid; idx < lv.ncls * NDIR; idx += NT) {
            const double *c = lv.ctab + (size_t)idx * NTERM;
            double w = 0.0;
#pragma unroll
            for (int t = 0; t < NTERM; ++t) w += c[t] * s[t];
            W[idx] = w;
        }
    }
    const double *xc = a.x + cell * lv.ld;
    const double *x2c = FUSED && a.x2 ? a.x2 + cell * lv.ld : nullptr;
    double *xoc = FUSED && a.xout ? a.xout + cell * lv.ld : nullptr;
    double *xac = FUSED && a.xacc ? a.xacc + cell * lv.ld : nullptr;
    const double *x3c = FUSED && a.x3 ? a.x3 + cell * lv.ld : nullptr;
    const double beta = to_sgpr(x2c ? a.scal[a.s_num] / a.scal[a.s_den] : 0.0);
    const double ax = to_sgpr(xac || x3c ? a.scal[a.a_num] / a.scal[a.a_den] : 0.0);
    const double c2 = to_sgpr(x3c ? a.scal[a.c_num] / a.scal[a.c_den] : 0.0);
    const uint32_t dm = (a.flags & 1) ? dmask[cell] : 0u;
    const double *sc = a.src ? a.src + cell * lv.ld : nullptr;
    double *oc = a.out ? a.out + cell * (a.out_ld ? a.out_ld : (int64_t)lv.ld) : nullptr;
    uint32_t mq[4] = {0, 0, 0, 0};
    if (FUSED) {
        const uint32_t *mp = reinterpret_cast<const uint32_t *>(a.mult + cell * 16);
#pragma unroll
        for (int q = 0; q < 4; ++q) mq[q] = a.mult ? __builtin_amdgcn_readfirstlane(mp[q]) : 0x01010101u;
    }
    const bool wdot = WD && FUSED && (a.flags & 8);
    const double wself = (wdot && (a.flags & 256)) ? 0.0 : 1.0;
    double rr = 0.0, pap = 0.0;
    auto plane_off = [&](int k) {
        if (k <= 0) return 0;
        if (k > m + 1) k = m + 1;
        const long long n1 = m + 1, n2 = m + 1 - k;
        return (int)((n1 * (n1 + 1) * (n1 + 2) - n2 * (n2 + 1) * (n2 + 2)) / 6);
    };
    HMG_SLAB_T0();
    __syncthreads();
    HMG_SLAB_PHASE(0);
    double w0[NDIR];
#pragma unroll
    for (int d = 0; d < NDIR; ++d) w0[d] = to_sgpr(W[d]);
    int lo_prev = 0;
    for (int sl = 0; sl < st.nslab; ++sl) {
        const int *hd = st.head + 8 * sl;
// ... 96 lines not shown
                if (!wdot) o = sv + o;
                if ((dm >> (cls - 1)) & 1u) o = 0.0;
                if (!FUSED || oc) oc[t] = o;
                if (FUSED) {
                    const int en = cls - 1;
                    const uint32_t word = en < 4 ? mq[0] : en < 8 ? mq[1] : en < 12 ? mq[2] : mq[3];
                    const uint32_t mu = (word >> (8 * (en & 3))) & 0xffu;
                    pap += (double)mu * ((wdot ? fma(wself, ctr, sv) : ctr) * o);
                }
            }
        }
        HMG_SLAB_PHASE(3);
        const int n_int = cp_cnt - cp_surf;
        const int nit_i = (n_int + NT - 1) / NT;
        for (int it = 0; it < nit_i; ++it) {
            const int v = it * NT + tid;
            const uint32_t pw = q0;
            const int t = t0;
            q0 = q1;
            t0 = t1;
            q1 = st.cp_word[ib + v + 2 * NT];
            t1 = (int)st.cp_slot[ib + v + 2 * NT];
            if (v < n_int) {
                const double sv = sc ? sc[t] : 0.0;
                int L, len, A, B;
                decode_lattice(pw, m, L, len, A, B);
                double ctr;
                double o = stencil_eval_v<DIM>(w0, xs + L, len, A, B, ctr);
                if (!wdot) o = sv + o;
                if (!FUSED || oc) oc[t] = o;
                if (FUSED) pap += (wdot ? fma(wself, ctr, sv) : ctr) * o;
            }
        }
        lo_prev = lo;
        HMG_SLAB_PHASE(4);
    }
    HMG_SLAB_STORE();
    if (FUSED) {
        __syncthreads();
        const double s_pap = block_sum(pap, smem);
        const double s_rr = block_sum(rr, smem);
        if (tid == 0) {
            a.blockpart[2 * cell] = s_pap;
            a.blockpart[2 * cell + 1] = s_rr;
        }
    }
}

__global__ void __launch_bounds__(256)
k_reduce_pairs(const double *__restrict__ blockpart, int64_t n, double *partials)
{
    __shared__ double red[4];
    double s0 = 0.0, s1 = 0.0;
    for (int64_t c = (int64_t)blockIdx.x * 256 + threadIdx.x; c < n; c += (int64_t)gridDim.x * 256) {
        s0 += blockpart[2 * c];
        s1 += blockpart[2 * c + 1];
    }
    const double r0 = block_sum(s0, red);
    const double r1 = block_sum(s1, red);
    if (threadIdx.x == 0) {
        partials[blockIdx.x] = r0;
        partials[2048 + blockIdx.x] = r1;
    }
}

__global__ void __launch_bounds__(256)
k_reduce_weighted(const double *__restrict__ blockpart, const double *__restrict__ coef, int jterm, int64_t n, double *partials)
{
    __shared__ double red[4];
    double s0 = 0.0;
    for (int64_t c = (int64_t)blockIdx.x * 256 + threadIdx.x; c < n; c += (int64_t)gridDim.x * 256)
        s0 += blockpart[2 * c] * coef[c * 8 + jterm];
    const double r0 = block_sum(s0, red);
    if (threadIdx.x == 0) partials[blockIdx.x] = r0;
}

size_t apply_lds_bytes(const LevelDev &lv)
{
    return sizeof(double) * (size_t)(WSZ + lv.lds_g0 + lv.nf + lv.lds_g1);
}

bool apply_restricts(const Launch &L, const LevelDev &lv)
{
    if (!(lv.dim == 3 && apply_lds_bytes(lv) <= 160 * 1024 && L.apply_threads == 0 && lv.rs_word &&
          lv.rs_w && lv.nf_coarse > 0 && lv.nei <= 64 && lv.nedge == 6 && lv.ncorner == 4))
        return false;
    if (lv.nf > 2048)
        return lv.blk_R == 6 && lv.nblk <= 960 && L.apply_wg512 && lv.nfi <= 512;
    return lv.nf > 192 && lv.nf <= 1024 && lv.blk_R == 4 && lv.nblk <= 192 && lv.nfi <= 128 && lv.rs_lp != nullptr;
}

bool apply_defers3(const Launch &L, const LevelDev &lv)
{
    return apply_restricts(L, lv) && lv.nf > 2048 && lv.nf <= 13 * 512;
}

bool apply_folds_coarse_x(const Launch &L, const LevelDev &lv)
{
    return lv.dim == 3 && apply_lds_bytes(lv) <= 160 * 1024 && L.apply_threads == 0 && L.apply_wg512 && lv.blk_R == 6 && lv.nblk <= 960 &&
           lv.nei <= 64 && lv.nedge == 6 && lv.ncorner == 4 && lv.nfi <= 512 && lv.par64 && lv.clpos && lv.nf > 2048 &&
           lv.nf <= 13 * 512 && lv.nf_coarse > 0 && lv.nf_coarse <= 2 * 512;
}

static size_t apply_lds_bytes_rb(const LevelDev &lv)
{
    return sizeof(double) * (size_t)(WSZ_RB + lv.lds_g0 + lv.nf + lv.lds_g1);
}

template <bool FUSED>
static void check_apply_bases(const ApplyArgs &a, const MeshDev &mesh)
{
    if (!a.x) throw std::runtime_error("operator apply: null input vector");
    if (!FUSED && !a.out) throw std::runtime_error("operator apply: a plain launch needs an output vector");
    if (a.rcoarse && a.ldrc <= 0) throw std::runtime_error("operator apply: epilogue restriction without the coarse column stride");
    if (FUSED && (!a.blockpart || !a.scal)) throw std::runtime_error("operator apply: fused launch without its reduction scratch");
    if (!mesh.coef) throw std::runtime_error("operator apply: no operator coefficients on the device (hmg_grid_set_operator)");
    if ((a.flags & 1) && !mesh.dmask) throw std::runtime_error("operator apply: constraint requested without a Dirichlet mask");
    if (a.xcoarse && !a.xout) throw std::runtime_error("operator apply: folded prolongation without xout");
    if ((a.flags & 128) && !(FUSED && a.x3 && a.x2 && a.xout && !a.xcoarse))
        throw std::runtime_error("operator apply: the zero-input form exists for the residual with two pending x-updates only");
}

static bool weight_cache_ok(const Launch &L, const LevelDev &lv, const MeshDev &mesh, const ApplyArgs &a)
{
    return L.weight_cache && lv.wcache && mesh.cell_class && lv.dim == 3 && lv.ncls == 15 && !(a.flags & (2 | 8 | 16)) &&
           (a.alpha == 1.0 || a.alpha == -1.0) && a.lambda == mesh.wc_lambda;
}

template <int DIM, int NT, int SPT, bool FUSED, int RB = 0, bool WD = false, bool CG = false, bool RS = false, bool WC = false, int LF = 0>
static void launch_apply_generic(const Launch &L, const LevelDev &lv, const MeshDev &mesh, const ApplyArgs &a, size_t lds)
{
    auto kern = k_apply<DIM, NT, SPT, FUSED, RB, WD, CG, RS, WC, LF>;
    if (a.rcoarse && !RS) throw std::runtime_error("operator apply: this instantiation cannot restrict in its epilogue");
    if (a.xc_p && !(CG && LF == 5)) throw std::runtime_error("operator apply: this instantiation cannot finish the coarse x");
    if (a.x4 && LF != 4) throw std::runtime_error("operator apply: this instantiation cannot carry a third pending x-update");
    if ((a.flags & 128) && !(FUSED && (RS || RB == 0)))
        throw std::runtime_error("operator apply: this instantiation cannot take a zero input that is not in memory");
    if (FUSED && a.xcoarse && !CG) lds += sizeof(double) * (size_t)lv.nf_coarse;
    if (lds > 48 * 1024)
        HMG_HIP_CHECK(hipFuncSetAttribute((const void *)kern, hipFuncAttributeMaxDynamicSharedMemorySize, (int)lds));
    const int64_t nblocks = a.cell_list ? a.ncell_list : a.ncells_prefix ? a.ncells_prefix : mesh.ncells;
    if (nblocks == 0) return;
    check_apply_bases<FUSED>(a, mesh);
    ApplyArgs b = a;
    b.nwork = nblocks;
    b.cell_class = WC ? mesh.cell_class : nullptr;
    if (WC && !weight_cache_ok(L, lv, mesh, a)) throw std::runtime_error("operator apply: class-weight cache not usable for this launch");
    if (L.cell_order && RB && !a.cell_list && !a.ncells_prefix && mesh.cell_perm) {
        b.cell_list = mesh.cell_perm;
        b.ncell_list = nblocks;
    }
    const int64_t grid = NT == 64 ? std::min<int64_t>(nblocks, 32 * (int64_t)L.num_cu) : nblocks;
    hipLaunchKernelGGL(kern, dim3((unsigned)grid), dim3(NT), lds, L.stream, lv, mesh.coef, mesh.dmask, b);
    check_launch();
    if (WC && L.n_wc_launches) *L.n_wc_launches += 1;
}

template <int DIM, bool FUSED, bool WD = false>
static void launch_apply_dim(const Launch &L, const LevelDev &lv, const MeshDev &mesh, const ApplyArgs &a)
{
    const size_t lds = apply_lds_bytes(lv);
    if (a.x4 && !(FUSED && DIM == 3 && !WD && a.x3 && a.x2 && a.xout && a.rcoarse && !a.xcoarse && !a.xacc && !(a.flags & 128) &&
                  apply_defers3(L, lv)))
        throw std::runtime_error("operator apply: a third pending x-update (x4) where no kernel carries it");
    if ((a.xc_p || a.xc_r) && !(FUSED && DIM == 3 && !WD && a.xc_p && a.xc_r && a.xcoarse && (a.flags & 64) && !a.x2 && !a.xacc && !a.x3 &&
                                !a.rcoarse && apply_folds_coarse_x(L, lv)))
        throw std::runtime_error("operator apply: pending coarse x-updates (xc_p, xc_r) where no kernel carries them");
    if constexpr (DIM == 3 && !WD) {
        if (apply_wave_ok(L, lv, mesh, a, FUSED)) {
            launch_apply_wave(L, lv, mesh, a, FUSED);
            return;
        }
        if (apply_small_ok(L, lv, mesh, a, FUSED)) {
            launch_apply_small(L, lv, mesh, a, FUSED);
            return;
        }
    }
    const bool force_slab2 = DIM == 3 && !WD && L.slab2_force && mesh.slab.head && mesh.slab.nslab >= 2 && lv.nf > 2048 &&
                             !a.xcoarse && !a.rcoarse && !(a.flags & (4 | 8));
    if (DIM == 2 && lds > 160 * 1024) {
        launch_apply_rows(L, lv, mesh, a, FUSED, WD);
        return;
    }
    if (lds > 160 * 1024 || force_slab2) {
        if (DIM != 3 || !mesh.slab.head) throw std::runtime_error("operator apply: cell does not fit the LDS");
        if constexpr (DIM == 3 && !WD) {
            if (apply_slab2_ok(L, lv, mesh, a)) {
                launch_apply_slab2(L, lv, mesh, a, FUSED);
                return;
            }
        }
        auto kern = k_apply_slab<3, 1024, FUSED, WD>;
        const size_t bytes = sizeof(double) * (size_t)(WSZ + mesh.slab.lds_nodes);
        HMG_HIP_CHECK(hipFuncSetAttribute((const void *)kern, hipFuncAttributeMaxDynamicSharedMemorySize, (int)bytes));
        const int64_t nblocks = a.cell_list ? a.ncell_list : a.ncells_prefix ? a.ncells_prefix : mesh.ncells;
        if (nblocks == 0) return;
        check_apply_bases<FUSED>(a, mesh);
        ApplyArgs b = a;
        b.nwork = nblocks;
        if (L.cell_order && !a.cell_list && !a.ncells_prefix && mesh.cell_perm) {
            b.cell_list = mesh.cell_perm;
            b.ncell_list = nblocks;
        }
        hipLaunchKernelGGL(kern, dim3((unsigned)nblocks), dim3(1024), bytes, L.stream, lv, mesh.coef, mesh.dmask, b,
                           mesh.slab);
        check_launch();
        return;
    }
    const int nf = lv.nf;
    int nt = WD ? 0 : L.apply_threads;
    if (nt == 0) nt = nf <= 192 ? 64 : nf <= 2048 ? 256 : 1024;
    if (nt <= 64) {
        if constexpr (DIM == 3 && !WD) {
            if (weight_cache_ok(L, lv, mesh, a)) {
                if (nf > 64)
                    launch_apply_generic<DIM, 64, 3, FUSED, 0, false, false, false, DIM == 3>(L, lv, mesh, a, lds);
// ... 287 lines not shown
void launch_mask(const Launch &L, const LevelDev &lv, const MeshDev &mesh, double *x, int which)
{
    hipLaunchKernelGGL(k_mask, dim3((unsigned)mesh.ncells), dim3(64), 0, L.stream, lv, mesh.ncells,
                       which == 0 ? mesh.dmask : mesh.dupmask, x);
    check_launch();
}

template <int NT>
__global__ void __launch_bounds__(NT)
k_prolong_add(LevelDev fine, int nfc, int ldc, const double *__restrict__ xc, double *xf)
{
    extern __shared__ double smem[];
    const int64_t cell = blockIdx.x;
    const double *c = xc + cell * ldc;
    for (int t = threadIdx.x; t < nfc; t += NT) smem[t] = c[t];
    __syncthreads();
    double *f = xf + cell * fine.ld;
    for (int t = threadIdx.x; t < fine.nf; t += NT) {
        const int a = fine.par_a[t], b = fine.par_b[t];
        double y = f[t];
        if (a == b)
            y += 1.0 * smem[a];
        else {
            y += 0.5 * smem[a];
            y += 0.5 * smem[b];
        }
        f[t] = y;
    }
}

template <int NT, int SPT>
__global__ void __launch_bounds__(NT)
k_prolong_add_big(LevelDev fine, int nfc, int ldc, const double *__restrict__ xc, double *xf)
{
    extern __shared__ double smem[];
    const int64_t cell = blockIdx.x;
    const double *c = xc + cell * ldc;
    for (int t0 = threadIdx.x; t0 < nfc; t0 += NT * SPT) {
        double v[SPT];
#pragma unroll
        for (int q = 0; q < SPT; ++q) {
            const int t = t0 + q * NT;
            v[q] = t < nfc ? c[t] : 0.0;
        }
#pragma unroll
        for (int q = 0; q < SPT; ++q) {
            const int t = t0 + q * NT;
            if (t < nfc) smem[t] = v[q];
        }
    }
    __syncthreads();
    double *f = xf + cell * fine.ld;
    for (int t0 = threadIdx.x; t0 < fine.nf; t0 += NT * SPT) {
        double y[SPT];
        uint32_t w[SPT];
#pragma unroll
        for (int q = 0; q < SPT; ++q) {
            const int t = t0 + q * NT;
            if (t < fine.nf) {
                y[q] = f[t];
                w[q] = fine.par32[t];
            }
        }
#pragma unroll
        for (int q = 0; q < SPT; ++q) {
            const int t = t0 + q * NT;
            if (t < fine.nf) {
                const uint32_t a = w[q] & 0xffffu, b = w[q] >> 16;
                double r = y[q];
                if (a == b)
                    r += 1.0 * smem[a];
                else {
                    r += 0.5 * smem[a];
                    r += 0.5 * smem[b];
                }
                f[t] = r;
            }
        }
    }
}

template <int NT, bool USE_LDS>
__global__ void __launch_bounds__(NT)
k_restrict(LevelDev fine, int nfc, int ldc, const double *__restrict__ rf, double *bc)
{
    extern __shared__ double smem[];
    const int64_t cell = blockIdx.x;
    const double *f = rf + cell * fine.ld;
    const double *fs = f;
    if (USE_LDS) {
        constexpr int SPT = 8;
        for (int t0 = threadIdx.x; t0 < fine.nf; t0 += NT * SPT) {
            double v[SPT];
#pragma unroll
            for (int q = 0; q < SPT; ++q) {
                const int t = t0 + q * NT;
                v[q] = t < fine.nf ? f[t] : 0.0;
            }
#pragma unroll
            for (int q = 0; q < SPT; ++q) {
                const int t = t0 + q * NT;
                if (t < fine.nf) smem[t] = v[q];
            }
        }
        __syncthreads();
        fs = smem;
    }
    double *c = bc + cell * ldc;
    for (int t = threadIdx.x; t < nfc; t += NT) {
        const int b = fine.rptr[t], n = fine.rptr[t + 1] - b;
        int idx[15];
#pragma unroll
        for (int q = 0; q < 15; ++q) idx[q] = fine.ridx[b + (q < n ? q : 0)];
        double tmp = 0.0;
        tmp += 1.0 * fs[idx[0]];
#pragma unroll
        for (int q = 1; q < 15; ++q)
            if (q < n) tmp += 0.5 * fs[idx[q]];
        c[t] = tmp;
    }
}

void launch_prolong_add(const Launch &L, const LevelDev &fine, const LevelDev &coarse, int64_t ncells,
                        const double *xc, double *xf)
{
    size_t lds = sizeof(double) * coarse.nf;
    if (lds > 160 * 1024 && fine.dim == 2) {
        launch_prolong_add_wide(L, fine, coarse, ncells, xc, xf);
        return;
    }
    if (lds > 160 * 1024) throw std::runtime_error("prolongation: coarse cell does not fit LDS");
    if (fine.nf <= 256) {
        auto k = k_prolong_add<64>;
        hipLaunchKernelGGL(k, dim3((unsigned)ncells), dim3(64), lds, L.stream, fine, coarse.nf, coarse.ld, xc, xf);
    } else if (fine.nf > 8192) {
        auto k = k_prolong_add_big<1024, 4>;
        if (lds > 48 * 1024)
            HMG_HIP_CHECK(hipFuncSetAttribute((const void *)k, hipFuncAttributeMaxDynamicSharedMemorySize, (int)lds));
        hipLaunchKernelGGL(k, dim3((unsigned)ncells), dim3(1024), lds, L.stream, fine, coarse.nf, coarse.ld, xc, xf);
    } else {
        auto k = k_prolong_add<256>;
        if (lds > 48 * 1024)
            HMG_HIP_CHECK(hipFuncSetAttribute((const void *)k, hipFuncAttributeMaxDynamicSharedMemorySize, (int)lds));
        hipLaunchKernelGGL(k, dim3((unsigned)ncells), dim3(256), lds, L.stream, fine, coarse.nf, coarse.ld, xc, xf);
    }
    check_launch();
}

void launch_restrict_slab(const Launch &L, const LevelDev &fine_rtab, const MeshDev &mesh, const SlabTables &st,
                          int ldc, const double *rf, double *bc)
{
    ApplyArgs a{};
    a.alpha = 1.0;
    a.x = rf;
    a.out = bc;
    a.out_ld = ldc;
    a.flags = 4;
    {
        MeshDev m2 = mesh;
        m2.slab = st;
        if (L.restrict_slab2 && apply_slab2_ok(L, fine_rtab, m2, a)) {
            launch_apply_slab2(L, fine_rtab, m2, a, false);
            return;
        }
    }
    auto kern = k_apply_slab<3, 1024, false>;
    const size_t bytes = sizeof(double) * (size_t)(WSZ + st.lds_nodes);
    HMG_HIP_CHECK(hipFuncSetAttribute((const void *)kern, hipFuncAttributeMaxDynamicSharedMemorySize, (int)bytes));
    hipLaunchKernelGGL(kern, dim3((unsigned)mesh.ncells), dim3(1024), bytes, L.stream, fine_rtab, mesh.coef, mesh.dmask, a, st);
    check_launch();
}

void launch_restrict(const Launch &L, const LevelDev &fine, const LevelDev &coarse, int64_t ncells,
                     const double *rf, double *bc)
{
    size_t lds = sizeof(double) * fine.nf;
    if (fine.nf <= 256) {
        hipLaunchKernelGGL((k_restrict<64, true>), dim3((unsigned)ncells), dim3(64), lds, L.stream, fine, coarse.nf,
                           coarse.ld, rf, bc);
    } else if (lds <= 160 * 1024 && fine.nf > 2048) {
        auto k = k_restrict<1024, true>;
        if (lds > 48 * 1024)
            HMG_HIP_CHECK(hipFuncSetAttribute((const void *)k, hipFuncAttributeMaxDynamicSharedMemorySize, (int)lds));
        hipLaunchKernelGGL(k, dim3((unsigned)ncells), dim3(1024), lds, L.stream, fine, coarse.nf, coarse.ld, rf, bc);
    } else if (lds <= 160 * 1024) {
        auto k = k_restrict<256, true>;
        if (lds > 48 * 1024)
            HMG_HIP_CHECK(hipFuncSetAttribute((const void *)k, hipFuncAttributeMaxDynamicSharedMemorySize, (int)lds));
        hipLaunchKernelGGL(k, dim3((unsigned)ncells), dim3(256), lds, L.stream, fine, coarse.nf, coarse.ld, rf, bc);
    } else {
        hipLaunchKernelGGL((k_restrict<256, false>), dim3((unsigned)ncells), dim3(256), 0, L.stream, fine, coarse.nf,
                           coarse.ld, rf, bc);
    }
    check_launch();
}

constexpr int SB = 256;

static inline int strided_blocks(const Launch &L, int64_t n, int per_thread)
{
    int64_t b = (n + (int64_t)256 * per_thread - 1) / ((int64_t)256 * per_thread);
    int64_t cap = (int64_t)L.num_cu * 8;
    if (b > cap) b = cap;
    if (b < 1) b = 1;
    return (int)b;
}

static inline int64_t stream_blocks(int64_t n)
{
    const int64_t b = ((n >> 1) + SB - 1) / SB;
    return b < 1 ? 1 : b;
}

static void check_grid(int64_t nb)
{
    if (nb > 0x7fffffffLL) throw std::runtime_error("vector too long for one launch");
}

__global__ void __launch_bounds__(256) k_reduce_partials(const double *__restrict__ part, int64_t nb, double *out)
{
    __shared__ double red[4];
    const int64_t per = (nb + gridDim.x - 1) / gridDim.x;
    const int64_t b0 = (int64_t)blockIdx.x * per, b1 = b0 + per < nb ? b0 + per : nb;
    double a = 0.0;
    for (int64_t i = b0 + threadIdx.x; i < b1; i += 256) a += part[i];
    const double s = block_sum(a, red);
    if (threadIdx.x == 0) out[blockIdx.x] = s;
}

__global__ void __launch_bounds__(SB) k_fill(double *x, int64_t n, double v)
{
    const int64_t i = (int64_t)blockIdx.x * SB + threadIdx.x;
    if (i < (n >> 1)) reinterpret_cast<double2 *>(x)[i] = make_double2(v, v);
    if ((n & 1) && blockIdx.x == 0 && threadIdx.x == 0) x[n - 1] = v;
}

__global__ void __launch_bounds__(SB) k_copy(double *dst, const double *__restrict__ src, int64_t n)
{
    const int64_t i = (int64_t)blockIdx.x * SB + threadIdx.x;
    if (i < (n >> 1)) reinterpret_cast<double2 *>(dst)[i] = reinterpret_cast<const double2 *>(src)[i];
    if ((n & 1) && blockIdx.x == 0 && threadIdx.x == 0) dst[n - 1] = src[n - 1];
}

__global__ void __launch_bounds__(SB) k_axpy(double a, const double *__restrict__ x, double *y, int64_t n)
{
    const int64_t i = (int64_t)blockIdx.x * SB + threadIdx.x;
    if (i < (n >> 1)) {
        double2 *y2 = reinterpret_cast<double2 *>(y);
        const double2 xv = reinterpret_cast<const double2 *>(x)[i];
        double2 yv = y2[i];
        yv.x = axpy1(a, xv.x, yv.x);
        yv.y = axpy1(a, xv.y, yv.y);
        y2[i] = yv;
    }
    if ((n & 1) && blockIdx.x == 0 && threadIdx.x == 0) y[n - 1] = axpy1(a, x[n - 1], y[n - 1]);
}

__global__ void __launch_bounds__(SB) k_xpby(const double *__restrict__ r, double b, double *p, int64_t n)
{
    const int64_t i = (int64_t)blockIdx.x * SB + threadIdx.x;
    if (i < (n >> 1)) {
        double2 *p2 = reinterpret_cast<double2 *>(p);
        const double2 rv = reinterpret_cast<const double2 *>(r)[i];
        double2 pv = p2[i];
        pv.x = axpy1(b, pv.x, rv.x);
        pv.y = axpy1(b, pv.y, rv.y);
        p2[i] = pv;
    }
    if ((n & 1) && blockIdx.x == 0 && threadIdx.x == 0) p[n - 1] = axpy1(b, p[n - 1], r[n - 1]);
}

__global__ void __launch_bounds__(SB)
k_dot(const double *__restrict__ x, const double *__restrict__ y, int64_t n, double *partials)
{
    __shared__ double red[4];
// ... 935 lines not shown
```

homogenization.jl_amd/csrc/hmg_objects.hpp:

```cpp
#pragma once

#include "../../include/hmg.h"
#include "hmg_device.hpp"
#include "hmg_host.hpp"

#include <atomic>
#include <memory>
#include <mutex>
#include <stdexcept>
#include <string>
#include <vector>

struct ncclComm;

using namespace hmg;

#define HIPCHK(expr)                                                                            \
    do {                                                                                        \
        hipError_t _e = (expr);                                                                 \
        if (_e != hipSuccess)                                                                   \
            throw std::runtime_error(std::string("HIP error: ") + hipGetErrorString(_e) + " (" #expr ")"); \
    } while (0)

namespace hmg {

std::recursive_mutex &lifetime_mutex();
using LifetimeLock = std::lock_guard<std::recursive_mutex>;

std::atomic<int64_t> &device_allocs();

hipError_t device_malloc(void **p, size_t bytes);

struct DryUploads {
    static DryUploads *&current()
    {
        static thread_local DryUploads *c = nullptr;
        return c;
    }
    bool dry;
    uint64_t *hash;
    DryUploads *prev;
    DryUploads(bool dry_, uint64_t *hash_) : dry(dry_), hash(hash_), prev(current()) { current() = this; }
    ~DryUploads() { current() = prev; }
    DryUploads(const DryUploads &) = delete;
    DryUploads &operator=(const DryUploads &) = delete;
    static bool active() { return current() && current()->dry; }
    static void note(const void *data, size_t bytes)
    {
        uint64_t h = *current()->hash ^ (bytes * 0x9e3779b97f4a7c15ull);
        const unsigned char *b = (const unsigned char *)data;
        for (size_t i = 0; i < bytes; ++i) h = (h ^ b[i]) * 1099511628211ull;
        *current()->hash = h;
    }
};

template <class T>
struct DevBuf {
    T *p = nullptr;
    size_t n = 0;
    DevBuf() = default;
    DevBuf(const DevBuf &) = delete;
    DevBuf &operator=(const DevBuf &) = delete;
    ~DevBuf() { release(); }
    void release()
    {
        if (p) (void)hipFree(p);
        p = nullptr;
        n = 0;
    }
    void alloc(size_t count)
    {
        release();
        n = count;
        if (!count || DryUploads::active()) return;
        HIPCHK(device_malloc((void **)&p, count * sizeof(T)));
    }
    void upload(const std::vector<T> &h, hipStream_t s)
    {
        alloc(h.size());
        if (DryUploads::active()) {
            DryUploads::note(h.data(), h.size() * sizeof(T));
            return;
        }
        if (!h.empty()) {
            HIPCHK(hipMemcpyAsync(p, h.data(), h.size() * sizeof(T), hipMemcpyHostToDevice, s));
            HIPCHK(hipStreamSynchronize(s));
        }
    }
};

struct LevelBufs {
    DevBuf<uint64_t> meta;
    DevBuf<uint16_t> lpos, sweep_slot;
    DevBuf<int> slab_head, slab_rs_head;
    DevBuf<uint32_t> slab_ld_word, slab_cp_word, slab_rs_word;
    DevBuf<uint16_t> slab_cp_slot, slab_rs_slot;
    DevBuf<double> rtab;
    int nslab = 0, slab_lds_nodes = 0, slab_max_surf = 0, slab_rs_max_surf = 0, slab_max_int = 0, slab_rs_max_int = 0;
    DevBuf<uint32_t> pos32, pos32w, sweep32, par32, blk_word;
    DevBuf<uint64_t> par64;
    DevBuf<uint16_t> clpos;
    DevBuf<uint32_t> rs_word;
    DevBuf<double> rs_w;
    DevBuf<uint16_t> rs_lp;
    DevBuf<uint16_t> blk_slot;
    DevBuf<uint32_t> wave_tab, wave_lpos, wave_par, wave_cl, wave_rs;
    DevBuf<double> wcache;
    DevBuf<double> ctab;
    DevBuf<int32_t> hier2slot, par_a, par_b, rptr, ridx;
    DevBuf<double> dphi;
};

struct CutKind {
    int64_t nglobal = 0;
    int64_t nentries = 0;
    std::vector<int64_t> gid;
    std::vector<int32_t> seg;
    std::vector<int64_t> sidx;
    DevBuf<int32_t> cell_lid;
    DevBuf<uint8_t> first;
};

struct CutLevel {
    bool ready = false;
    DevBuf<int64_t> pos[3];
    int64_t ndoubles = 0;
    std::vector<int64_t> ops;
    int64_t nstage = 0;
    DevBuf<int64_t> plan;
};

struct ApplyTimer {
    bool on = false;
    int min_level = 0;
    std::vector<std::pair<hipEvent_t, hipEvent_t>> pool;
    std::vector<int> ev_level;
    std::vector<double> ev_bytes;
    size_t used = 0;
};

struct CoarseProbe {
    double *h = nullptr;
    hipEvent_t ev = nullptr;
    bool pending = false;
    int budget = 0;
    int generation = 0;
};

}

struct hmg_ctx {
    int refs = 1;
    ApplyTimer timer;
    bool fuse_cg_default = true;
    bool fold_x = true;
    bool swap_rp = true;
    bool fold_prolong = true;
    bool lazy_dead = true;
    bool lazy_pre = true;
    bool fold_faces = true;
    bool lean_post = true;
    bool lazy_post = true;
    bool fold_coarse_x = true;
    int lazy_top = 2;
    bool zero_entry = true;
    bool fold_restrict = true;
    bool prolong_in_image = true;
    int device = 0;
    hipStream_t stream = nullptr;
    bool own_stream = false;
    DevBuf<double> partials, scal, rpart;
    Launch L{};
    int coarse_maxit = 5000;
    int coarse_check = 25;
    bool coarse_probe = true;
    double coarse_rtol = 1e-13;
    int coarse_poly = 4;
    double coarse_poly_ratio = 20.0;
    ncclComm *comm = nullptr;
    int comm_nranks = 1, comm_rank = 0;
    hipStream_t comm_stream = nullptr;
    hipEvent_t ev_packed = nullptr, ev_summed = nullptr;
    int64_t comm_calls = 0, comm_doubles = 0;
    int64_t small_launches = 0;
    int64_t wc_launches = 0;
    int64_t wave_launches = 0;
    int64_t slab2_launches = 0;
    int64_t rows_launches = 0;
    int64_t wc_max_classes = 0;
    int64_t wc_classes = 0, wc_bytes = 0;
    int64_t wc_refusals = 0;
    int64_t spare_bytes = 0;
    int64_t fcg_bytes = 0;
    int64_t smoother_diag_bytes = 0;
    int64_t smoother_diag_builds = 0;
    int64_t moments_kernel_ns = 0, moments_download_ns = 0;
    int64_t coarse_x_folds = 0;
    int last_pre_form = 0;
    int last_top_form = 0;
    bool vec_pool_on = true;
    std::vector<std::pair<size_t, void *>> vec_pool;
    bool comm_rehearsal = false;
    int64_t overlap_min_doubles = 524288;
    std::vector<struct hmg_grid *> probe_grids;
};

struct hmg_grid {
    int refs = 1;
    hmg_ctx *ctx = nullptr;
    int dim = 0, nlevels = 0;
    std::vector<LevelTables> lt;
    std::vector<std::unique_ptr<LevelBufs>> lb;
    std::vector<LevelDev> ld;
    MeshTables mesh_full, mesh;
    bool shrunk = false;
    MeshDev md{};
    DevBuf<int32_t> d_cells, d_face_pairs, d_face_partner, d_edge_ptr, d_edge_ent, d_node_ptr, d_node_ent, d_node_first;
    DevBuf<uint16_t> d_dmask, d_dupmask;
    DevBuf<uint8_t> d_mult;
    DevBuf<double> d_blockpart;
    bool fuse_cg = true;
    DevBuf<double> d_coef;
    std::vector<double> sigma, coef;
    int sig_n = 0;
    DevBuf<int32_t> d_cell_class;
    DevBuf<double> d_coef_rep;
    int nclasses = 0;
    std::vector<int32_t> cell_class;
    int64_t wc_limit = 0;
    bool wc_trim = false;
    int64_t wc_counted_classes = 0, wc_counted_bytes = 0;
    double wc_lambda = 0.0;
    bool wc_ready = false;
    double lambda = 0.0;
    bool has_op = false;
    uint64_t op_epoch = 0;
    CoarseMatrix cm;
    CoarseDev cd{};
    bool coarse_ready = false;
    DevBuf<int32_t> c_rowptr, c_colidx, c_interior;
    DevBuf<double> c_val, c_diag, c_b, c_x, c_r, c_z, c_p, c_q, c_u, c_z2, c_d;
    DevBuf<double> top_spare;
    bool top_spare_refused = false;
    int smoother = 0;
    std::vector<std::unique_ptr<DevBuf<double>>> dinv;
    bool dinv_ready = false;
    std::vector<char> dinv_level_ready;
    bool dinv_build_counted = false;
    double c_lmax = 2.0;
    int coarse_last_it = 0;
    int coarse_budget = 0;
    int coarse_generation = 0;
    int64_t coarse_misses = 0;
    std::unique_ptr<CoarseProbe> probe{new CoarseProbe};
    std::unique_ptr<Partition> part;
    std::vector<double> sigma_global;
    std::vector<double> part_coords;
    std::vector<int64_t> part_cells;
    std::vector<int32_t> part_owner, part_cut_owner;
    bool part_halo = true;
    int64_t part_nnodes = 0, part_ncells = 0;
    DevBuf<int32_t> d_nodes_g, d_owned, d_cells_gnode;
    CutKind cut[3];
    int64_t cut_agreed[3] = {0, 0, 0};
    bool cut_agreed_ready = false;
    std::vector<std::unique_ptr<CutLevel>> cutlv;
    bool sharers = false;
    hmg_exchange_fn exchange = nullptr, scalar_sum = nullptr;
    hmg_exchange_fn ex_begin = nullptr;
    int (*ex_end)(void *) = nullptr;
    hmg_p2p_fn p2p = nullptr, p2p_begin = nullptr;
    double *stage = nullptr;
    int64_t stage_cap = 0;
    DevBuf<double> own_stage;
    bool overlap = true;
    DevBuf<int32_t> d_cells_cut, d_cells_inner, d_cell_perm;
    void *ex_user = nullptr;
    double *ex_buf = nullptr;
    int64_t ex_cap = 0;
    DevBuf<double> own_exbuf;

    uint64_t upload_hash = 1469598103934665603ull;

    const MeshTables &cur() const { return shrunk ? mesh : mesh_full; }
};

struct hmg_vec {
    hmg_grid *g = nullptr;
    int level = 0;
    double *d = nullptr;
    bool own = false;
    int64_t alloc_cells = 0;
    size_t bytes = 0;
};

namespace hmg {

inline int fail(const std::exception &e)
{
    last_error() = e.what();
    return 1;
}

#define HMG_TRY try {
#define HMG_END                      \
    }                                \
    catch (const std::exception &e)  \
    {                                \
        return fail(e);              \
    }                                \
    catch (...)                      \
    {                                \
        last_error() = "unknown error"; \
        return 1;                    \
    }                                \
    return 0;

inline void need(bool c, const char *msg)
{
    if (!c) throw std::runtime_error(msg);
}

inline const LevelDev &lev(const hmg_grid *g, int level)
{
    need(g != nullptr, "null grid");
    need(g->ctx != nullptr, "this grid was created without a device context (host tables only): no compute path exists on the CPU");
    need(level >= 1 && level <= g->nlevels, "level out of range");
    return g->ld[level - 1];
}

inline void check_vec(const hmg_grid *g, int level, const hmg_vec *v, const char *name)
{
    if (!v) throw std::runtime_error(std::string("null vector: ") + name);
    if (v->g != g) throw std::runtime_error(std::string("vector belongs to another grid: ") + name);
    if (v->level != level) throw std::runtime_error(std::string("vector has the wrong level: ") + name);
    if (v->alloc_cells < g->md.ncells) throw std::runtime_error(std::string("vector too small: ") + name);
}

inline int64_t vec_len(const hmg_vec *v) { return (int64_t)v->g->ld[v->level - 1].ld * v->g->md.ncells; }

inline bool has_exchange(const hmg_grid *g) { return g->exchange || g->ex_begin || g->p2p || g->p2p_begin; }

double *vec_alloc(hmg_ctx *c, size_t bytes);
void vec_release(hmg_ctx *c, void *p, size_t bytes);
void grid_unref(hmg_grid *grid);
double read_scalar(hmg_ctx *c, int slot);

void ensure_weight_cache(hmg_grid *g);
void release_weight_cache(hmg_grid *g);

void set_slab(hmg_grid *g, const LevelDev &lv);
void apply(hmg_grid *g, const LevelDev &lv, double alpha, const double *x, const double *src, double *out, int mask);
void restrict_level(hmg_grid *g, int level_fine, const double *rf, double *bc);
void interface_sum(hmg_grid *g, const LevelDev &lv, double *x, bool faces = true);
void scalar_sum(hmg_grid *g, int slot, int count);
bool reserve_top_spare(hmg_grid *g, bool must);
void release_top_spare(hmg_grid *g);
bool wants_top_spare(const hmg_grid *g, int level);
void ensure_smoother_diag(hmg_grid *g, int level, double *scratch);
void ensure_smoother_diag(hmg_grid *g, int top, hmg_vec **states);
void release_smoother_diag(hmg_grid *g);
void vcycle(hmg_grid *g, int k, int steps, int steps_coarse, hmg_vec **st, bool top = true, bool zero_guess = false);

void coarse_solve(hmg_grid *g, hmg_vec *b1, hmg_vec *x1);
void probe_unlist(hmg_grid *g);
void judge_probes(hmg_ctx *c);

void exchange_cut(hmg_grid *g, const LevelDev &lv, double *x);
void cut_pack(hmg_grid *g, const LevelDev &lv, double *x, int unpack);
void exchange_prepare(hmg_grid *g, const LevelDev &lv);
void exchange_run(hmg_grid *g, const LevelDev &lv, bool async);
void exchange_finish(hmg_grid *g, const LevelDev &lv, bool async);
void comm_drop(hmg_ctx *c);

}
```

homogenization.jl_amd/csrc/hmg_smooth.cpp:

```cpp
#include "../../include/hmg.h"
#include "hmg_objects.hpp"
#include "hmg_pcg.hpp"

#include <algorithm>
#include <cmath>

namespace hmg {

void set_slab(hmg_grid *g, const LevelDev &lv)
{
    const LevelBufs &B = *g->lb[lv.level - 1];
    g->md.slab.head = B.slab_head.p;
    g->md.slab.ld_word = B.slab_ld_word.p;
    g->md.slab.cp_word = B.slab_cp_word.p;
    g->md.slab.cp_slot = B.slab_cp_slot.p;
    g->md.slab.nslab = B.nslab;
    g->md.slab.lds_nodes = B.slab_lds_nodes;
    g->md.slab.max_surf = B.slab_max_surf;
    g->md.slab.max_int = B.slab_max_int;
}

namespace {

struct TimedRegion {
    hmg_ctx *c;
    bool timed;
    int level;
    double bytes;
    TimedRegion(hmg_grid *g, const LevelDev &lv, double bytes_) : c(g->ctx), level(lv.level), bytes(bytes_)
    {
        ApplyTimer &t = c->timer;
        timed = t.on && lv.level >= t.min_level;
        if (!timed) return;
        if (t.used == t.pool.size()) {
            hipEvent_t a, b;
            HIPCHK(hipEventCreate(&a));
            HIPCHK(hipEventCreate(&b));
            t.pool.emplace_back(a, b);
        }
        HIPCHK(hipEventRecord(t.pool[t.used].first, c->stream));
    }
    void stop()
    {
        if (!timed) return;
        ApplyTimer &t = c->timer;
        HIPCHK(hipEventRecord(t.pool[t.used].second, c->stream));
        t.used += 1;
        t.ev_level.push_back(level);
        t.ev_bytes.push_back(bytes);
        timed = false;
    }
};

}

void apply(hmg_grid *g, const LevelDev &lv, double alpha, const double *x, const double *src, double *out, int mask)
{
    TimedRegion tr(g, lv, 8.0 * (double)lv.nf * (double)g->md.ncells * (src ? 3.0 : 2.0));
    set_slab(g, lv);
    ensure_weight_cache(g);
    launch_apply(g->ctx->L, lv, g->md, alpha, g->lambda, x, src, out, mask);
    tr.stop();
}

void restrict_level(hmg_grid *g, int level_fine, const double *rf, double *bc)
{
    const LevelDev &fine = lev(g, level_fine), &coarse = lev(g, level_fine - 1);
    const LevelBufs &B = *g->lb[level_fine - 1];
    if (B.slab_rs_head.p) {
        LevelDev fr = fine;
        fr.ctab = B.rtab.p;
        SlabTables st{};
        st.head = B.slab_rs_head.p;
        st.ld_word = B.slab_ld_word.p;
        st.cp_word = B.slab_rs_word.p;
        st.cp_slot = B.slab_rs_slot.p;
        st.nslab = B.nslab;
        st.lds_nodes = B.slab_lds_nodes;
        st.max_surf = B.slab_rs_max_surf;
        st.max_int = B.slab_rs_max_int;
        launch_restrict_slab(g->ctx->L, fr, g->md, st, coarse.ld, rf, bc);
        return;
    }
    launch_restrict(g->ctx->L, fine, coarse, g->md.ncells, rf, bc);
}

void interface_sum(hmg_grid *g, const LevelDev &lv, double *x, bool faces)
{
    launch_interface_sum(g->ctx->L, lv, g->md, x, 0, faces);
    if (has_exchange(g)) exchange_cut(g, lv, x);
}

void scalar_sum(hmg_grid *g, int slot, int count)
{
    if (g->scalar_sum) {
        if (g->scalar_sum(g->ex_user, g->ctx->L.scal + slot, count) != 0)
            throw std::runtime_error("scalar_sum callback failed");
    }
}

namespace {

void agree_on_cut(hmg_grid *g)
{
    if (g->cut_agreed_ready) return;
    const Partition &P = *g->part;
    hmg_ctx *c = g->ctx;
    if (P.global_ids) {
        for (int k = 0; k < 3; ++k) g->cut_agreed[k] = g->cut[k].nglobal;
    } else if (!g->scalar_sum) {
        for (int k = 0; k < 3; ++k) g->cut_agreed[k] = -1;
    } else {
        double lead[3] = {0.0, 0.0, 0.0};
        for (const Partition::Segment &S : P.segs)
            if (!S.members.empty() && S.members.front() == P.rank)
                for (int k = 0; k < 3; ++k) lead[k] += (double)S.count[k];
        double *d = c->L.scal + S_HOST;
        HIPCHK(hipMemcpyAsync(d, lead, sizeof(lead), hipMemcpyHostToDevice, c->stream));
        scalar_sum(g, S_HOST, 3);
        HIPCHK(hipMemcpyAsync(lead, d, sizeof(lead), hipMemcpyDeviceToHost, c->stream));
        HIPCHK(hipStreamSynchronize(c->stream));
        for (int k = 0; k < 3; ++k) g->cut_agreed[k] = (int64_t)std::llround(lead[k]);
    }
    g->cut_agreed_ready = true;
}

void apply_then_sum(hmg_grid *g, const LevelDev &lv, ApplyArgs a, bool fused, int slot_pap, int slot_rr,
                    bool sum_out = true, bool faces = true)
{
    hmg_ctx *c = g->ctx;
    const Launch &L = c->L;
    set_slab(g, lv);
    ensure_weight_cache(g);
    const double streams = ((a.flags & 128) ? 0.0 : 1.0) + (a.out ? 1.0 : 0.0) + (a.src ? 1.0 : 0.0) + (a.x2 ? 1.0 : 0.0) + (a.xout ? 1.0 : 0.0) +
                           (a.xacc ? 2.0 : 0.0) + (a.x3 ? 1.0 : 0.0) + (a.x4 ? 1.0 : 0.0) + (a.xcoarse ? (double)lv.nf_coarse / (double)lv.nf : 0.0) +
                           (a.rcoarse ? (double)lv.nf_coarse / (double)lv.nf : 0.0) + (a.xc_p ? 2.0 * (double)lv.nf_coarse / (double)lv.nf : 0.0);
    TimedRegion tr(g, lv, 8.0 * (double)lv.nf * (double)g->md.ncells * streams);
    if (has_exchange(g) && g->part) agree_on_cut(g);
    const bool has_cut = has_exchange(g) && g->part && g->cut_agreed[0] >= 0 &&
                         g->cut_agreed[0] + g->cut_agreed[1] + g->cut_agreed[2] > 0;
    const int64_t global_cut = has_cut ? g->cut_agreed[0] * lv.nfi + g->cut_agreed[1] * lv.nei + g->cut_agreed[2] : 0;
    const bool overlap = has_cut && (g->sharers ? g->p2p_begin != nullptr : g->ex_begin != nullptr) && g->ex_end && g->overlap &&
                         global_cut >= std::max<int64_t>(1, c->overlap_min_doubles);
    auto launch = [&](const int32_t *list, int64_t n) {
        ApplyArgs b = a;
        b.cell_list = list;
        b.ncell_list = n;
        if (fused)
            launch_apply_fused_kernel(L, lv, g->md, b);
        else
            launch_apply_args(L, lv, g->md, b);
    };
    auto sums = [&]() {
        if (!fused || slot_pap < 0) return;
        launch_apply_fused_reduce(L, g->md, slot_pap, slot_rr);
        if (slot_rr >= 0 && (slot_rr == slot_pap + 1 || slot_rr + 1 == slot_pap))
            scalar_sum(g, std::min(slot_rr, slot_pap), 2);
        else {
            if (slot_rr >= 0) scalar_sum(g, slot_rr, 1);
            scalar_sum(g, slot_pap, 1);
        }
    };
    if (!a.out && a.rcoarse) {
        need(fused && !sum_out, "epilogue restriction belongs to the cell-local residual");
        launch(nullptr, 0);
        tr.stop();
        return;
    }
    if (!a.out) {
        need(fused, "apply without an output vector");
        launch(nullptr, 0);
        tr.stop();
        sums();
        return;
    }
    if (!sum_out) {
        launch(nullptr, 0);
        tr.stop();
        return;
    }
    if (!overlap) {
        launch(nullptr, 0);
        tr.stop();
        sums();
        interface_sum(g, lv, a.out, faces);
        return;
    }
    if (g->md.ncells_cut > 0) launch(g->md.cells_cut, g->md.ncells_cut);
    launch_interface_sum(L, lv, g->md, a.out, 1);
    exchange_prepare(g, lv);
    cut_pack(g, lv, a.out, 0);
    exchange_run(g, lv, true);
    if (g->md.ncells_inner > 0)
        launch(g->md.cells_inner, g->md.ncells_inner);
    tr.stop();
    launch_interface_sum(L, lv, g->md, a.out, 2, faces);
    sums();
    exchange_finish(g, lv, true);
    cut_pack(g, lv, a.out, 1);
}

enum class Role {
    Plain,
    Pre,
    PostTop,
    PostBelow,
};

enum class Tail {
    Full,
    ScratchP,
    Top2,
    Top3,
    DeadXp,
    DeadDefer,
    DeadDefer2,
    DeadDefer3,
    DeadX2,
};

struct SmoothForm {
    bool swap_rp = false;
    bool ride = false;
    Tail tail = Tail::Full;
    bool hand_up = false;
    bool x_zero = false;
};

struct DeferredX {
    int rs = -1;
    int pap = S_PAP;
    bool two_updates = false;
    int a_num = -1, a_den = -1, b_num = -1, b_den = -1;
    bool three_updates = false;
    int d_num = -1, d_den = -1;
    const double *p = nullptr, *r = nullptr;
};

SmoothForm smooth_form(const hmg_grid *g, int level, int steps, Role role)
{
    const LevelDev &lv = lev(g, level);
    const hmg_ctx *c = g->ctx;
    const bool lean = c->lean_post && (role == Role::PostTop || role == Role::PostBelow);
    const bool dead = role == Role::Pre || (lean && role == Role::PostBelow);
    SmoothForm f;
    if (!g->fuse_cg || g->smoother == 1) {
        f.tail = dead ? Tail::DeadXp : lean ? Tail::ScratchP : Tail::Full;
        return f;
    }
    const bool faces = c->fold_faces && lv.dim == 3 && lv.nfi > 0;
    f.swap_rp = role != Role::Plain && c->swap_rp && steps > 0;
    f.ride = faces;
    if (role == Role::Pre && c->fold_x) {
        f.tail = steps >= 2 && c->lazy_dead ? Tail::DeadDefer2 : Tail::DeadDefer;
        if (f.tail == Tail::DeadDefer2 && steps >= 3 && c->lazy_pre && faces && c->fold_restrict && apply_defers3(c->L, lv) &&
            g->top_spare.n >= (size_t)lv.ld * (size_t)g->md.ncells)
            f.tail = Tail::DeadDefer3;
    }
    else if (dead)
        f.tail = steps >= 2 && c->lazy_post ? Tail::DeadX2 : Tail::DeadXp;
    else if (lean && steps >= 2 && c->lazy_top > 0 && faces)
        f.tail = steps >= 3 && c->lazy_top > 1 && g->top_spare.n >= (size_t)lv.ld * (size_t)g->md.ncells ? Tail::Top3 : Tail::Top2;
    else if (lean)
        f.tail = Tail::ScratchP;
    return f;
}

}

bool reserve_top_spare(hmg_grid *g, bool must)
{
    hmg_ctx *c = g->ctx;
    const LevelDev &lv = g->ld[(size_t)g->nlevels - 1];
    const size_t n = (size_t)lv.ld * (size_t)g->mesh_full.ncells;
    if (g->top_spare.n >= n && n > 0) return true;
    if (g->top_spare_refused && !must) return false;
    HIPCHK(hipSetDevice(c->device));
    void *q = nullptr;
    if (device_malloc(&q, n * sizeof(double)) != hipSuccess) {
        (void)hipGetLastError();
        g->top_spare_refused = true;
        if (must)
            throw std::runtime_error("the spare direction vector of the finest level (" + std::to_string((n * sizeof(double)) >> 20) +
                                     " MiB, option lazy_top = 2) does not fit the device memory; V-cycles take the two-update form");
        return false;
    }
    c->spare_bytes -= (int64_t)(g->top_spare.n * sizeof(double));
    g->top_spare.release();
    g->top_spare.p = (double *)q;
    g->top_spare.n = n;
    g->top_spare_refused = false;
    c->spare_bytes += (int64_t)(n * sizeof(double));
    return true;
}

void release_top_spare(hmg_grid *g)
{
    if (g->ctx) {
        if (g->top_spare.p) (void)hipStreamSynchronize(g->ctx->stream);
        g->ctx->spare_bytes -= (int64_t)(g->top_spare.n * sizeof(double));
    }
    g->top_spare.release();
}

bool wants_top_spare(const hmg_grid *g, int level)
{
    return g->ctx && g->smoother == 0 && g->ctx->lazy_top > 1 && level == g->nlevels && g->dim == 3 && g->ld[(size_t)level - 1].nfi > 0;
}

void ensure_smoother_diag(hmg_grid *g, int level, double *scratch)
{
    if (g->smoother != 1 || level < 2) return;
    need(g->has_op, "operator not set");
    need(g->dinv.size() == (size_t)g->nlevels && level <= g->nlevels, "Jacobi-preconditioned smoother: the inverse diagonals were not reserved");
    if (!g->dinv_ready) {
        g->dinv_level_ready.assign((size_t)g->nlevels, 0);
        g->dinv_build_counted = false;
        g->dinv_ready = true;
    }
    if (g->dinv_level_ready[(size_t)level - 1]) return;
    const LevelDev &lv = lev(g, level);
    double *d = g->dinv[(size_t)level - 1]->p;
    need(scratch != nullptr && scratch != d, "Jacobi-preconditioned smoother: no scratch vector to form the diagonal with");
    for (int limb = diag_limbs() - 1; limb >= 0; --limb) {
        launch_operator_diag(g->ctx->L, lv, g->md, g->lambda, limb, scratch);
        interface_sum(g, lv, scratch);
        launch_diag_accum(g->ctx->L, lv, g->md, scratch, d, limb);
    }
    launch_dinv_finish(g->ctx->L, lv, g->md, d);
    g->dinv_level_ready[(size_t)level - 1] = 1;
    if (!g->dinv_build_counted) {
        g->ctx->smoother_diag_builds += 1;
        g->dinv_build_counted = true;
    }
}

void ensure_smoother_diag(hmg_grid *g, int top, hmg_vec **states)
{
    if (g->smoother != 1) return;
    for (int level = 2; level <= top; ++level) ensure_smoother_diag(g, level, states[5 * (level - 1) + 4]->d);
}

void release_smoother_diag(hmg_grid *g)
{
    int64_t bytes = 0;
    for (const auto &d : g->dinv)
        if (d) bytes += (int64_t)(d->n * sizeof(double));
    if (g->ctx) {
        if (bytes > 0) (void)hipStreamSynchronize(g->ctx->stream);
        g->ctx->smoother_diag_bytes -= bytes;
    }
    g->dinv.clear();
    g->dinv_level_ready.clear();
    g->dinv_ready = false;
}

namespace {

void first_residual(hmg_grid *g, int level, hmg_vec *x, hmg_vec *b, hmg_vec *r, const SmoothForm &f, const hmg_vec *xcoarse,
                    const DeferredX *cx)
{
    const LevelDev &lv = lev(g, level);
    const Launch &L = g->ctx->L;
    const int64_t n = vec_len(x);
    {
        ApplyArgs a{};
        a.alpha = -1.0;
        a.lambda = g->lambda;
        a.x = x->d;
        a.src = b->d;
        a.out = r->d;
        a.flags = 1;
        if (f.x_zero) {
            need(!xcoarse, "zero initial guess with a coarse-grid correction");
            launch_copy(L, r->d, b->d, n);
            launch_mask(L, lv, g->md, r->d, 0);
            interface_sum(g, lv, r->d);
        } else if (xcoarse) {
            a.xcoarse = xcoarse->d;
            a.ldc = lev(g, level - 1).ld;
            a.xout = x->d;
            if (g->ctx->prolong_in_image && apply_lds_bytes(lv) > 48 * 1024) a.flags |= 64;
            if (cx && cx->rs >= 0) {
                need(cx->two_updates && cx->p && cx->r && (a.flags & 64), "pending coarse x-updates where the residual cannot carry them");
                a.xc_p = cx->p;
                a.xc_r = cx->r;
                a.a_num = cx->a_num;
                a.a_den = cx->a_den;
                a.s_num = cx->b_num;
                a.s_den = cx->b_den;
                a.c_num = cx->rs;
                a.c_den = cx->pap;
                g->ctx->coarse_x_folds += 1;
            }
            apply_then_sum(g, lv, a, true, -1, -1);
        } else {
            apply_then_sum(g, lv, a, false, -1, -1);
        }
    }
}

void smooth_pcg(hmg_grid *g, int level, int steps, hmg_vec *x, hmg_vec *r, hmg_vec *p, hmg_vec *Ap, const SmoothForm &f)
{
    const LevelDev &lv = lev(g, level);
    const Launch &L = g->ctx->L;
    const int64_t n = vec_len(x);
    need(g->dinv_ready && g->dinv.size() == (size_t)g->nlevels && g->dinv_level_ready[(size_t)level - 1] && g->dinv[(size_t)level - 1] &&
             (g->dinv[(size_t)level - 1]->p || n == 0),
         "Jacobi-preconditioned smoother: no inverse diagonal for this level");
    need(f.tail == Tail::Full || f.tail == Tail::ScratchP || f.tail == Tail::DeadXp, "Jacobi-preconditioned smoother: unknown tail");
    const double *dinv = g->dinv[(size_t)level - 1]->p;
    int cur = S_RS, other = S_RS2;
    launch_pcg_start(L, p->d, r->d, dinv, n, cur);
    scalar_sum(g, cur, 1);
    for (int i = 0; i < steps; ++i) {
        if (g->fuse_cg) {
            ApplyArgs a{};
            a.alpha = 1.0;
            a.lambda = g->lambda;
            a.x = p->d;
            a.out = Ap->d;
            a.flags = 1;
            apply_then_sum(g, lv, a, true, S_PAP, -1);
        } else {
            apply(g, lv, 1.0, p->d, nullptr, Ap->d, 1);
            interface_sum(g, lv, Ap->d);
            launch_dot(L, p->d, Ap->d, n, S_PAP);
            scalar_sum(g, S_PAP, 1);
        }
        const bool last = i == steps - 1;
        if (last && f.tail != Tail::Full) {
            if (f.tail == Tail::ScratchP) {
                launch_pcg_rupdate(L, r->d, Ap->d, dinv, n, cur, S_PAP, other);
                scalar_sum(g, other, 1);
            }
            launch_cg_xp_update(L, x->d, p->d, r->d, n, cur, S_PAP, cur, other, 0);
            return;
        }
        launch_pcg_rupdate(L, r->d, Ap->d, dinv, n, cur, S_PAP, other);
        scalar_sum(g, other, 1);
        launch_pcg_xp(L, x->d, p->d, r->d, dinv, n, cur, S_PAP, other, cur);
        std::swap(cur, other);
    }
}

DeferredX smooth(hmg_grid *g, int level, int steps, hmg_vec *x, hmg_vec *b, hmg_vec *r, hmg_vec *p, hmg_vec *Ap,
                 const SmoothForm &f, const hmg_vec *xcoarse = nullptr, const DeferredX *cx = nullptr)
{
    const LevelDev &lv = lev(g, level);
    const Launch &L = g->ctx->L;
    const int64_t n = vec_len(x);
    first_residual(g, level, x, b, r, f, xcoarse, cx);
    if (g->smoother == 1) {
        smooth_pcg(g, level, steps, x, r, p, Ap, f);
        return {};
    }
    int cur = S_RS, other = S_RS2;
    if (!g->fuse_cg || steps <= 0) {
        launch_copy_dot(L, p->d, r->d, n, cur);
// ... 61 lines not shown
            apply_then_sum(g, lv, a, true, S_PAP2, -1, true, false);
            launch_cg_rupdate_faces(L, lv, g->md, r->d, r->d, Ap->d, n, cur, S_PAP2, S_RS3);
            scalar_sum(g, S_RS3, 1);
            continue;
        }
        step(i, f.ride);
    }
    if (f.tail == Tail::Top2 || f.tail == Tail::Top3) g->ctx->last_top_form = f.tail == Tail::Top3 ? 2 : 1;
    ApplyArgs a = args(last);
    switch (f.tail) {
    case Tail::Full:
    case Tail::ScratchP:
        step(last, f.ride && f.tail == Tail::ScratchP);
        launch_cg_xp_update(L, x->d, p->d, r->d, n, other, S_PAP, cur, other, f.tail == Tail::Full ? 1 : 0);
        return {};
    case Tail::DeadXp:
    case Tail::DeadDefer:
        a.out = nullptr;
        apply_then_sum(g, lv, a, true, S_PAP, last == 0 ? cur : -1, true, true);
        if (last == 0 && f.swap_rp) exchange_rp();
        if (f.tail == Tail::DeadDefer) return DeferredX{cur};
        launch_cg_xp_update(L, x->d, p->d, r->d, n, cur, S_PAP, cur, other, 0);
        return {};
    case Tail::DeadDefer2:
    case Tail::DeadX2:
        a.out = a.xout = a.xacc = nullptr;
        apply_then_sum(g, lv, a, true, S_PAP2, -1);
        if (f.tail == Tail::DeadX2 && f.hand_up) {
            DeferredX d{cur, S_PAP2, true, other, S_PAP, cur, other};
            d.p = p->d;
            d.r = r->d;
            return d;
        }
        if (f.tail == Tail::DeadX2) {
            launch_cg_x2_update(L, x->d, p->d, r->d, n, other, S_PAP, cur, other, cur, S_PAP2);
            return {};
        }
        return DeferredX{cur, S_PAP2, true, other, S_PAP, cur, other};
    case Tail::DeadDefer3:
        a.x2 = g->top_spare.p;
        a.out = a.xout = a.xacc = nullptr;
        a.s_num = S_RS3;
        a.s_den = cur;
        apply_then_sum(g, lv, a, true, S_PAP3, -1);
        {
            DeferredX d{S_RS3, S_PAP3, true, cur, S_PAP2, S_RS3, cur};
            d.three_updates = true;
            d.d_num = other;
            d.d_den = S_PAP;
            return d;
        }
    case Tail::Top2:
        a.xout = a.xacc = nullptr;
        apply_then_sum(g, lv, a, true, S_PAP2, -1, true, false);
        launch_cg_rupdate_faces_x(L, lv, g->md, r->d, r->d, Ap->d, n, cur, S_PAP2, other, x->d, p->d, other, S_PAP, cur, other,
                                  nullptr, 0, 0);
        scalar_sum(g, other, 1);
        return {};
    case Tail::Top3:
        a.x2 = g->top_spare.p;
        a.xout = a.xacc = nullptr;
        a.s_num = S_RS3;
        a.s_den = cur;
        apply_then_sum(g, lv, a, true, S_PAP3, -1, true, false);
        launch_cg_rupdate_faces_x(L, lv, g->md, r->d, r->d, Ap->d, n, S_RS3, S_PAP3, other, x->d, g->top_spare.p, cur, S_PAP2,
                                  S_RS3, cur, p->d, other, S_PAP);
        scalar_sum(g, other, 1);
        return {};
    }
    return {};
}

bool zero_entry_ok(const hmg_grid *g, int k, int steps)
{
    if (!g->ctx->zero_entry) return false;
    if (k == 1) return true;
    if (g->smoother == 1) return false;
    if (steps != 2 || smooth_form(g, k, steps, Role::Pre).tail != Tail::DeadDefer2) return false;
    const LevelDev &lv = g->ld[k - 1];
    if (lv.blk_R > 0) return g->ctx->fold_restrict && apply_restricts(g->ctx->L, lv);
    return true;
}

int vcycle_down(hmg_grid *g, int k, int steps, hmg_vec **st, bool inside = false, bool x_zero = false, int steps_next = -1)
{
    hmg_vec **cur = st + 5 * (k - 1);
    hmg_vec **nxt = st + 5 * (k - 2);
    const Launch &L = g->ctx->L;
    SmoothForm form = smooth_form(g, k, steps, Role::Pre);
    need(!x_zero || form.tail == Tail::DeadDefer2, "zero initial guess: the pre-smoother does not defer both x-updates");
    form.x_zero = x_zero;
    const DeferredX dx = smooth(g, k, steps, cur[0], cur[1], cur[2], cur[3], cur[4], form);
    const int deferred = dx.rs < 0 ? 0 : dx.three_updates ? 3 : dx.two_updates ? 2 : 1;
    const bool skip_fill = inside && steps_next >= 0 && zero_entry_ok(g, k - 1, steps_next);
    if (dx.rs >= 0) {
        ApplyArgs a{};
        a.alpha = -1.0;
        a.lambda = g->lambda;
        a.x = cur[0]->d;
        a.x2 = dx.three_updates ? g->top_spare.p : cur[3]->d;
        a.xout = cur[0]->d;
        if (dx.three_updates) {
            need(g->ctx->fold_restrict && apply_defers3(L, lev(g, k)), "three pending x-updates where the local residual cannot carry them");
            a.x4 = cur[3]->d;
            a.d_num = dx.d_num;
            a.d_den = dx.d_den;
        }
        if (dx.two_updates) {
            a.x3 = cur[2]->d;
            a.a_num = dx.a_num;
            a.a_den = dx.a_den;
            a.s_num = dx.b_num;
            a.s_den = dx.b_den;
            a.c_num = dx.rs;
            a.c_den = dx.pap;
        } else {
            a.s_num = dx.rs;
            a.s_den = dx.pap;
        }
        a.src = cur[1]->d;
        a.out = cur[2]->d;
        a.flags = 1 | (x_zero ? 128 : 0);
        if (g->ctx->fold_restrict && apply_restricts(L, lev(g, k))) {
            if (inside) a.out = nullptr;
            a.rcoarse = nxt[1]->d;
            a.ldrc = lev(g, k - 1).ld;
            apply_then_sum(g, lev(g, k), a, true, -1, -1, false);
            if (!skip_fill) launch_fill(L, nxt[0]->d, vec_len(nxt[0]), 0.0);
            return deferred;
        }
        apply_then_sum(g, lev(g, k), a, true, -1, -1, false);
    } else {
        apply(g, lev(g, k), -1.0, cur[0]->d, cur[1]->d, cur[2]->d, 1);
    }
    restrict_level(g, k, cur[2]->d, nxt[1]->d);
    if (!skip_fill) launch_fill(L, nxt[0]->d, vec_len(nxt[0]), 0.0);
    return deferred;
}

DeferredX vcycle_up(hmg_grid *g, int k, int steps, hmg_vec **st, Role role, const DeferredX *cx = nullptr, bool hand_up = false)
{
    hmg_vec **cur = st + 5 * (k - 1);
    hmg_vec **nxt = st + 5 * (k - 2);
    const Launch &L = g->ctx->L;
    const bool fold_p = g->ctx->fold_prolong && g->fuse_cg && apply_lds_bytes(lev(g, k)) <= 160 * 1024 &&
                        apply_lds_bytes(lev(g, k)) + sizeof(double) * (size_t)lev(g, k - 1).nf <= 80 * 1024;
    need(!(cx && cx->rs >= 0) || fold_p, "pending coarse x-updates without the folded prolongation");
    if (!fold_p) launch_prolong_add(L, lev(g, k), lev(g, k - 1), g->md.ncells, nxt[0]->d, cur[0]->d);
    SmoothForm form = smooth_form(g, k, steps, role);
    form.hand_up = hand_up && form.tail == Tail::DeadX2;
    return smooth(g, k, steps, cur[0], cur[1], cur[2], cur[3], cur[4], form, fold_p ? nxt[0] : nullptr, cx);
}

bool coarse_x_folds(const hmg_grid *g, int k, int steps_below)
{
    const hmg_ctx *c = g->ctx;
    if (k < 3 || g->smoother == 1 || !c->fold_coarse_x || !c->lazy_post || !c->fold_prolong || !c->lean_post || !g->fuse_cg || !c->prolong_in_image) return false;
    const LevelDev &lv = g->ld[(size_t)k - 1];
    if (!(apply_lds_bytes(lv) > 48 * 1024 && apply_lds_bytes(lv) <= 160 * 1024 &&
          apply_lds_bytes(lv) + sizeof(double) * (size_t)g->ld[(size_t)k - 2].nf <= 80 * 1024))
        return false;
    return apply_folds_coarse_x(c->L, lv) && smooth_form(g, k - 1, steps_below, Role::PostBelow).tail == Tail::DeadX2;
}

DeferredX vcycle_level(hmg_grid *g, int k, int steps, int steps_coarse, hmg_vec **st, bool top, bool zero_guess, bool hand_up)
{
    if (k == 1) {
        hmg_vec **cur = st;
        coarse_solve(g, cur[1], cur[0]);
        return {};
    }
    const bool x_zero = (zero_guess || !top) && zero_entry_ok(g, k, steps);
    if (top && zero_guess && !x_zero) launch_fill(g->ctx->L, st[5 * (k - 1)]->d, vec_len(st[5 * (k - 1)]), 0.0);
    const int deferred = vcycle_down(g, k, steps, st, true, x_zero, steps_coarse);
    if (top) g->ctx->last_pre_form = deferred;
    const DeferredX cx = vcycle_level(g, k - 1, steps_coarse, steps_coarse, st, false, false, coarse_x_folds(g, k, steps_coarse));
    if (top) g->ctx->last_top_form = 0;
    return vcycle_up(g, k, steps, st, top ? Role::PostTop : Role::PostBelow, &cx, hand_up);
}

}

void vcycle(hmg_grid *g, int k, int steps, int steps_coarse, hmg_vec **st, bool top, bool zero_guess)
{
    (void)vcycle_level(g, k, steps, steps_coarse, st, top, zero_guess, false);
}

}

extern "C" {

int hmg_grid_reserve_spare(hmg_grid *g, int enable)
{
    HMG_TRY
    need(g != nullptr, "null grid");
    need(g->ctx != nullptr, "this grid was created without a device context (host tables only)");
    if (enable) {
        (void)reserve_top_spare(g, true);
    } else {
        release_top_spare(g);
        g->top_spare_refused = true;
    }
    HMG_END
}

int hmg_grid_set_smoother(hmg_grid *g, int kind)
{
    HMG_TRY
    need(g != nullptr, "null grid");
    need(g->ctx != nullptr, "this grid was created without a device context (host tables only)");
    need(kind == 0 || kind == 1, "smoother kind must be 0 (CG) or 1 (Jacobi-preconditioned CG)");
    HIPCHK(hipSetDevice(g->ctx->device));
    if (kind == 1 && g->dinv.size() != (size_t)g->nlevels) {
        release_smoother_diag(g);
        std::vector<std::unique_ptr<DevBuf<double>>> bufs((size_t)g->nlevels);
        int64_t bytes = 0;
        for (int level = 2; level <= g->nlevels; ++level) {
            const size_t n = (size_t)g->ld[(size_t)level - 1].ld * (size_t)g->mesh_full.ncells;
            bufs[(size_t)level - 1].reset(new DevBuf<double>);
            try {
                bufs[(size_t)level - 1]->alloc(n);
            } catch (const std::exception &) {
                (void)hipGetLastError();
                throw std::runtime_error("hmg_grid_set_smoother: the inverse diagonal of level " + std::to_string(level) + " (" +
                                         std::to_string((n * sizeof(double)) >> 20) + " MiB) does not fit the device memory; the smoother is unchanged");
            }
            bytes += (int64_t)(n * sizeof(double));
        }
        g->dinv = std::move(bufs);
        g->ctx->smoother_diag_bytes += bytes;
    }
    if (kind == 0) {
        release_smoother_diag(g);
    }
    g->smoother = kind;
    g->dinv_ready = false;
    g->op_epoch += 1;
    HMG_END
}

int hmg_grid_smoother(const hmg_grid *g) { return g ? g->smoother : -1; }

int hmg_grid_smoother_diag(hmg_grid *g, int level, hmg_vec *out)
{
    HMG_TRY
    need(g != nullptr, "null grid");
    need(g->smoother == 1, "hmg_grid_smoother_diag: the grid's smoother has no diagonal (hmg_grid_set_smoother(grid, 1))");
    need(level >= 2 && level <= g->nlevels, "level out of range (2..nlevels: level 1 has no smoother)");
    check_vec(g, level, out, "out");
    ensure_smoother_diag(g, level, out->d);
    launch_copy(g->ctx->L, out->d, g->dinv[(size_t)level - 1]->p, vec_len(out));
    HMG_END
}

int hmg_smooth(hmg_grid *g, int level, int steps, hmg_vec *x, hmg_vec *b, hmg_vec *r, hmg_vec *p, hmg_vec *Ap)
{
    HMG_TRY
    need(g && g->has_op, "operator not set");
    check_vec(g, level, x, "x");
    check_vec(g, level, b, "b");
    check_vec(g, level, r, "r");
    check_vec(g, level, p, "p");
    check_vec(g, level, Ap, "Ap");
    ensure_smoother_diag(g, level, Ap->d);
    smooth(g, level, steps, x, b, r, p, Ap, smooth_form(g, level, steps, Role::Plain));
    HMG_END
}
// ... 160 lines not shown
```

homogenization.jl_amd/csrc/hmg_upload.cpp:

```cpp
#include "../../include/hmg.h"
#include "hmg_objects.hpp"

#include <cmath>
#include <cstdlib>
#include <cstring>
#include <unordered_map>

namespace hmg {
namespace {

void upload_mesh(hmg_grid *g)
{
    const MeshTables &M = g->cur();
    const char *xcd_env = std::getenv("HMG_XCD_LISTS");
    const MeshKernelTables K = build_mesh_kernel_tables(M, !(xcd_env && xcd_env[0] == '0'));
    DryUploads dry_scope(!g->ctx, &g->upload_hash);
    hipStream_t s = g->ctx ? g->ctx->stream : nullptr;
    g->d_cells.upload(M.cells, s);
    g->d_face_pairs.upload(M.face_pairs, s);
    g->d_face_partner.upload(K.face_partner, s);
    g->d_edge_ptr.upload(M.edge_ptr, s);
    g->d_edge_ent.upload(M.edge_ent, s);
    g->d_node_ptr.upload(M.node_ptr, s);
    g->d_node_ent.upload(M.node_ent, s);
// ... 11 lines not shown
    g->d_cells_inner.upload(K.cells_inner, s);
    g->d_cell_perm.upload(K.cell_perm, s);
    MeshDev &d = g->md;
    d.dim = M.dim;
    d.ncells = M.ncells;
    d.nnodes = M.nnodes;
    d.cells = g->d_cells.p;
    d.face_pairs = g->d_face_pairs.p;
    d.face_partner = g->d_face_partner.p;
    d.nfacepairs = (int64_t)M.face_pairs.size() / 3;
    d.edge_ptr = g->d_edge_ptr.p;
    d.edge_ent = g->d_edge_ent.p;
    d.nsharededges = (int64_t)M.edge_ptr.size() - 1;
    d.node_ptr = g->d_node_ptr.p;
    d.node_ent = g->d_node_ent.p;
    d.nsharednodes = (int64_t)M.node_ptr.size() - 1;
    d.node_first = g->d_node_first.p;
    d.dmask = g->d_dmask.p;
    d.dupmask = g->d_dupmask.p;
    d.mult = g->d_mult.p;
    d.blockpart = g->d_blockpart.p;
    d.cells_cut = g->d_cells_cut.p;
    d.cells_inner = g->d_cells_inner.p;
    d.ncells_cut = (int64_t)M.cells_cut.size();
    d.ncells_inner = (int64_t)M.cells_inner.size();
    d.cell_perm = g->d_cell_perm.p;
    d.ncut_edge_groups = M.ncut_edge_groups;
    d.ncut_node_groups = M.ncut_node_groups;
    d.ncut_face_pairs = M.ncut_face_pairs;
    d.coef = g->d_coef.p;
}

void upload_levels(hmg_grid *g)
{
    DryUploads dry_scope(!g->ctx, &g->upload_hash);
    hipStream_t s = g->ctx ? g->ctx->stream : nullptr;
    const char *kb_env = std::getenv("HMG_SLAB_LDS_KB");
    const int slab_kb = kb_env ? std::max(16, std::min(158, std::atoi(kb_env))) : 70;
    g->ld.resize(g->nlevels);
    for (int l = 0; l < g->nlevels; ++l) {
        const LevelTables &T = g->lt[l];
        const LevelTables *C = l > 0 ? &g->lt[l - 1] : nullptr;
        const AddressTables A = build_address_tables(T);
        const BlockedInterior blk = build_blocked_interior(T);
        const SlabWindows sw = build_slab_windows(T, C, slab_kb);
        const TransferTables X = build_transfer_tables(T, C, blk);
        const WaveTables W = build_wave_tables(T, C, blk, X.clpos);
        g->lb.emplace_back(new LevelBufs);
        LevelBufs &B = *g->lb.back();
        B.meta.upload(T.meta, s);
        B.lpos.upload(A.lpos, s);
        B.pos32.upload(A.pos32, s);
        B.pos32w.upload(A.pos32w, s);
        B.sweep32.upload(A.sweep32, s);
        B.blk_word.upload(blk.word, s);
        B.blk_slot.upload(blk.slot, s);
        B.slab_head.upload(sw.head, s);
        B.slab_ld_word.upload(sw.ld_word, s);
        B.slab_cp_word.upload(sw.cp_word, s);
        B.slab_cp_slot.upload(sw.cp_slot, s);
        B.slab_rs_head.upload(sw.rs_head, s);
        B.slab_rs_word.upload(sw.rs_word, s);
        B.slab_rs_slot.upload(sw.rs_slot, s);
        B.rtab.upload(sw.rtab, s);
        B.sweep_slot.upload(A.sweep_slot, s);
        B.ctab.upload(T.ctab, s);
        B.hier2slot.upload(T.hier2slot, s);
        B.par_a.upload(T.par_a, s);
        B.par32.upload(X.par32, s);
        B.par_b.upload(T.par_b, s);
        B.clpos.upload(X.clpos, s);
        B.par64.upload(X.par64, s);
        B.rs_word.upload(X.rs_word, s);
        B.rs_w.upload(X.rs_w, s);
        B.rs_lp.upload(X.rs_lp, s);
        B.wave_tab.upload(W.tab, s);
        B.wave_lpos.upload(W.lpos, s);
        B.wave_par.upload(W.par, s);
        B.wave_cl.upload(W.cl, s);
        B.wave_rs.upload(W.rs, s);
        B.rptr.upload(T.rptr, s);
        B.ridx.upload(T.ridx, s);
        B.dphi.upload(T.dphi, s);
        B.nslab = sw.nslab;
        B.slab_lds_nodes = sw.lds_nodes;
        B.slab_max_surf = sw.max_surf;
        B.slab_max_int = sw.max_int;
        B.slab_rs_max_surf = sw.rs_max_surf;
        B.slab_rs_max_int = sw.rs_max_int;
        LevelDev &D = g->ld[l];
        D.dim = T.dim;
        D.level = T.level;
        D.m = T.m;
        D.nf = T.nf;
        D.ld = T.ld;
        D.ncorner = T.ncorner;
        D.nedge = T.nedge;
        D.nface = T.nface;
        D.nei = T.nei;
        D.nfi = T.nfi;
        D.nint = T.nint;
        D.off_edge = T.off_edge;
        D.off_face = T.off_face;
        D.off_int = T.off_int;
        D.ncls = T.ncls;
        D.ndir = T.ndir;
        D.nterm = T.nterm;
        D.lds_g0 = T.lds_g0;
        D.lds_g1 = T.lds_g1;
        D.nf_coarse = C ? C->nf : 0;
        D.meta = B.meta.p;
        D.lpos = B.lpos.p;
        D.sweep_slot = B.sweep_slot.p;
        D.pos32 = B.pos32.p;
        D.pos32w = B.pos32w.p;
        D.sweep32 = B.sweep32.p;
        D.nsweep = (int)T.sweep_meta.size();
        D.blk_word = B.blk_word.p;
        D.blk_slot = B.blk_slot.p;
        D.nblk = blk.nblk;
        D.blk_R = blk.R;
        D.ctab = B.ctab.p;
        D.hier2slot = B.hier2slot.p;
        D.par_a = B.par_a.p;
        D.par32 = B.par32.p;
        D.par_b = B.par_b.p;
        D.par64 = B.par64.p;
        D.clpos = B.clpos.p;
        D.rs_word = B.rs_word.p;
        D.rs_w = B.rs_w.p;
        D.rs_lp = B.rs_lp.p;
        D.rptr = B.rptr.p;
        D.ridx = B.ridx.p;
        D.dphi = B.dphi.p;
        D.wave_tab = B.wave_tab.p;
        D.wave_lpos = B.wave_lpos.p;
        D.wave_par = B.wave_par.p;
        D.wave_cl = B.wave_cl.p;
        D.wave_rs = B.wave_rs.p;
        D.wcache = nullptr;
    }
}

void build_cell_classes(hmg_grid *g)
{
    g->nclasses = 0;
    g->wc_ready = false;
    g->md.cell_class = nullptr;
    g->md.nclasses = 0;
    g->cell_class.clear();
    for (auto &d : g->ld) d.wcache = nullptr;
    bool any = false;
    for (const auto &d : g->ld) any = any || d.level >= 2;
    if (!any || g->dim != 3) return;
    const int64_t n = g->cur().ncells;
    const int64_t limit = g->wc_limit;
    struct Key {
        uint64_t b[8];
        bool operator==(const Key &o) const { return std::memcmp(b, o.b, sizeof(b)) == 0; }
    };
    struct Hash {
        size_t operator()(const Key &k) const
        {
            uint64_t h = 1469598103934665603ull;
            for (int q = 0; q < 8; ++q) h = (h ^ k.b[q]) * 1099511628211ull;
            return (size_t)h;
        }
    };
    std::unordered_map<Key, int32_t, Hash> ids;
    std::vector<int32_t> cls((size_t)n);
    std::vector<double> rep;
    for (int64_t c = 0; c < n; ++c) {
        Key k;
        std::memcpy(k.b, g->coef.data() + (size_t)c * 8, sizeof(k.b));
        auto it = ids.find(k);
        if (it == ids.end()) {
            if (limit > 0 && (int64_t)ids.size() >= limit) {
                release_weight_cache(g);
                return;
            }
            it = ids.emplace(k, (int32_t)ids.size()).first;
            rep.insert(rep.end(), g->coef.begin() + (size_t)c * 8, g->coef.begin() + (size_t)c * 8 + 8);
        }
        cls[(size_t)c] = it->second;
    }
    g->nclasses = (int)ids.size();
    hipStream_t s = g->ctx ? g->ctx->stream : nullptr;
    g->d_cell_class.upload(cls, s);
    g->d_coef_rep.upload(rep, s);
    g->cell_class.swap(cls);
    g->md.cell_class = g->d_cell_class.p;
    g->md.nclasses = g->nclasses;
}

}

void release_weight_cache(hmg_grid *g)
{
    bool held = false;
    for (auto &b : g->lb) held = held || (b && b->wcache.p);
    if (held && g->ctx) (void)hipStreamSynchronize(g->ctx->stream);
    for (auto &b : g->lb)
        if (b) b->wcache.release();
    for (auto &d : g->ld) d.wcache = nullptr;
    if (g->ctx) {
        g->ctx->wc_classes -= g->wc_counted_classes;
        g->ctx->wc_bytes -= g->wc_counted_bytes;
    }
    g->wc_counted_classes = g->wc_counted_bytes = 0;
    g->wc_ready = false;
}

void ensure_weight_cache(hmg_grid *g)
{
// ... 453 lines not shown
```

Measured before the change: 11.41 billion fine-DOF updates/s.

## Fold restriction into small-level residual apply and deliver masked coarse residual

Adds RS variants of the small and packed per-cell apply kernels. They compute the residual, write it into LDS and restrict it to the coarse column in the epilogue, which removes a separate restriction launch on coarse levels. A second coarse copy with Dirichlet entries zeroed (rcoarse2) can also be written, either there, in the wave kernel or in the plain restrict kernel. The next level's zero-guess pre-smoother then skips its copy-and-mask of the right-hand side. In exchange the RS kernels need more LDS and registers, use a smaller grid cap, and add extra global writes.

```diff
diff --git a/homogenization.jl_amd/csrc/hmg_apply_small.hip b/homogenization.jl_amd/csrc/hmg_apply_small.hip
--- a/homogenization.jl_amd/csrc/hmg_apply_small.hip
+++ b/homogenization.jl_amd/csrc/hmg_apply_small.hip
@@ -15,11 +15,40 @@
     asm volatile("v_mov_b32 %0, 0" : "=v"(z));
     return z;
 }
-}
-
-template <int SPT, bool FUSED>
-__global__ void __launch_bounds__(64, SPT == 1 ? 5 : 4)
-k_apply_small(LevelDev lv, const uint16_t *__restrict__ dmask, const int32_t *__restrict__ cell_class, ApplyArgs a)
+
+struct RsList {
+    uint32_t e[8];
+};
+__device__ __forceinline__ RsList rs_list_of(const LevelDev &lv, int c, bool with_bit)
+{
+    RsList r;
+    const int b = lv.rptr[c], n = lv.rptr[c + 1] - b;
+    uint32_t pos[16];
+#pragma unroll
+    for (int q = 0; q < 15; ++q) pos[q] = q < n ? (uint32_t)lv.lpos[lv.ridx[b + q]] : 0u;
+    pos[15] = (uint32_t)n | ((with_bit ? (uint32_t)lv.rs_bit[c] : 31u) << 8);
+#pragma unroll
+    for (int q = 0; q < 8; ++q) r.e[q] = pos[2 * q] | (pos[2 * q + 1] << 16);
+    return r;
+}
+__device__ __forceinline__ double rs_sum(const RsList &r, const double *xs)
+{
+    const int n = (int)((r.e[7] >> 16) & 0xffu);
+    double tmp = 0.0;
+    tmp += 1.0 * lds_ld(xs + (r.e[0] & 0xffffu));
+#pragma unroll
+    for (int u = 1; u < 15; ++u) {
+        const double t2 = tmp + 0.5 * lds_ld(xs + ((u & 1) ? r.e[u >> 1] >> 16 : r.e[u >> 1] & 0xffffu));
+        tmp = u < n ? t2 : tmp;
+    }
+    return tmp;
+}
+__device__ __forceinline__ double rs_masked(const RsList &r, uint32_t dm, double v) { return ((dm >> (r.e[7] >> 24)) & 1u) ? 0.0 : v; }
+}
+
+template <int SPT, bool FUSED, bool RS>
+__device__ __forceinline__ void apply_small_body(LevelDev lv, const uint16_t *__restrict__ dmask, const int32_t *__restrict__ cell_class,
+                                                 ApplyArgs a)
 {
     extern __shared__ double smem[];
     double *W = smem;
@@ -52,6 +81,9 @@
     const bool xzero = FUSED && (a.flags & 128);
     const int64_t G = gridDim.x;
     auto cell_of = [&](int64_t blk) -> int64_t { return a.cell_list ? (int64_t)HMG_KP(int32_t, a.cell_list)[blk] : blk; };
+    const bool rs_lane = RS && lane < lv.nf_coarse;
+    RsList rsl{};
+    if constexpr (RS) rsl = rs_list_of(lv, rs_lane ? lane : 0, a.rcoarse2 != nullptr);
 
     double pwv[4], pxv[SPT], px2[SPT], pxa[SPT], psv[SPT], pcv = 0.0;
     auto issue = [&](int64_t cell, int wsel) {
@@ -84,6 +116,7 @@
             const uint32_t w2 = HMG_KP(uint32_t, dmask)[cell >> 1];
             u.dm = (cell & 1) ? w2 >> 16 : w2 & 0xffffu;
         }
+
 #pragma unroll
         for (int q = 0; q < 4; ++q) u.mq[q] = FUSED && a.mult ? HMG_KP(uint32_t, a.mult)[cell * 4 + q] : 0x01010101u;
         return u;
@@ -150,6 +183,7 @@
             nxt = uniform_of(cell_n);
         }
         double *oc = a.out ? a.out + mycell * ld : nullptr;
+        double res[SPT];
 #pragma unroll
         for (int q = 0; q < SPT; ++q) {
             const uint32_t word = pw[q] | small_opaque_zero();
@@ -160,7 +194,8 @@
             o = sv[q] + o;
             if (cls > 0 && ((me.dm >> (cls - 1)) & 1u)) o = 0.0;
             if (has[q] && (!FUSED || oc)) oc[lane + 64 * q] = o;
-            if (FUSED && has[q]) {
+            if constexpr (RS) res[q] = o;
+            if (FUSED && !RS && has[q]) {
                 uint32_t mu = 1u;
                 if (cls > 0) {
                     const int e = cls - 1;
@@ -170,7 +205,17 @@
                 pap += (double)mu * (ctr * o);
             }
         }
-        if constexpr (FUSED) {
+        if constexpr (RS) {
+#pragma unroll
+            for (int q = 0; q < SPT; ++q)
+                if (has[q]) xs[lp[q]] = res[q];
+            const double tmp = rs_sum(rsl, xs);
+            if (rs_lane) {
+                a.rcoarse[mycell * a.ldrc + lane] = tmp;
+                if (a.rcoarse2) a.rcoarse2[mycell * a.ldrc + lane] = rs_masked(rsl, me.dm, tmp);
+            }
+        }
+        if constexpr (FUSED && !RS) {
             const double s_pap = wave_sum63(pap), s_rr = wave_sum63(rr);
             if (lane == 63) {
                 a.blockpart[2 * mycell] = s_pap;
@@ -182,10 +227,24 @@
     }
 }
 
-
-template <bool FUSED>
+template <int SPT, bool FUSED>
+__global__ void __launch_bounds__(64, SPT == 1 ? 5 : 4)
+k_apply_small(LevelDev lv, const uint16_t *__restrict__ dmask, const int32_t *__restrict__ cell_class, ApplyArgs a)
+{
+    apply_small_body<SPT, FUSED, false>(lv, dmask, cell_class, a);
+}
+
+template <int SPT>
 __global__ void __launch_bounds__(64, 4)
-k_apply_pack(LevelDev lv, const uint16_t *__restrict__ dmask, const int32_t *__restrict__ cell_class, ApplyArgs a)
+k_apply_small_rs(LevelDev lv, const uint16_t *__restrict__ dmask, const int32_t *__restrict__ cell_class, ApplyArgs a)
+{
+    apply_small_body<SPT, true, true>(lv, dmask, cell_class, a);
+}
+
+
+template <bool FUSED, bool RS>
+__device__ __forceinline__ void apply_pack_body(const LevelDev &lv, const uint16_t *__restrict__ dmask, const int32_t *__restrict__ cell_class,
+                                                const ApplyArgs &a)
 {
     extern __shared__ double smem[];
     const int lane = threadIdx.x, sub = lane >> 4, t = lane & 15, nf = lv.nf, m = lv.m;
@@ -211,6 +270,16 @@
     }
     const bool xzero = FUSED && (a.flags & 128);
     const int64_t G = gridDim.x, nquad = (a.nwork + 3) >> 2;
+    const bool rs_lane = RS && t < lv.nf_coarse;
+    typedef __attribute__((address_space(3))) uint32_t lds_u32;
+    volatile lds_u32 *rst = (volatile lds_u32 *)(lds_u32 *)reinterpret_cast<uint32_t *>(smem + 4 * imgp + 64) + 8 * t;
+    if constexpr (RS) {
+        if (sub == 0) {
+            const RsList r0 = rs_list_of(lv, rs_lane ? t : 0, a.rcoarse2 != nullptr);
+#pragma unroll
+            for (int q = 0; q < 8; ++q) rst[q] = r0.e[q];
+        }
+    }
 
     struct Meta {
         int cell, wsel;
@@ -225,7 +294,7 @@
         mt.cell = a.cell_list ? a.cell_list[w] : (int)w;
         mt.wsel = 2 * cell_class[mt.cell] + (neg ? 1 : 0);
         mt.dm = (a.flags & 1) ? (uint32_t)dmask[mt.cell] : 0u;
-        mt.mw = FUSED && a.mult && cls > 0 ? (uint32_t)a.mult[(int64_t)mt.cell * 16 + e] : 1u;
+        mt.mw = FUSED && !RS && a.mult && cls > 0 ? (uint32_t)a.mult[(int64_t)mt.cell * 16 + e] : 1u;
         return mt;
     };
     double2 pw2[8];
@@ -313,7 +382,18 @@
         double out = sv + acc;
         if (cls > 0 && ((me.dm >> (cls - 1)) & 1u)) out = 0.0;
         if (live && (!FUSED || a.out)) a.out[o] = out;
-        if constexpr (FUSED) {
+        if constexpr (RS) {
+            if (has) xs[lp] = out;
+            RsList rsl;
+#pragma unroll
+            for (int q = 0; q < 8; ++q) rsl.e[q] = rst[q];
+            const double tmp = rs_sum(rsl, xs);
+            if (rs_lane && me.valid) {
+                a.rcoarse[(int64_t)me.cell * a.ldrc + t] = tmp;
+                if (a.rcoarse2) a.rcoarse2[(int64_t)me.cell * a.ldrc + t] = rs_masked(rsl, me.dm, tmp);
+            }
+        }
+        if constexpr (FUSED && !RS) {
             if (has) {
                 const uint32_t mu = me.mw;
                 pap += (double)mu * (ctr * out);
@@ -336,6 +416,26 @@
     }
 }
 
+template <bool FUSED>
+__global__ void __launch_bounds__(64, 4)
+k_apply_pack(LevelDev lv, const uint16_t *__restrict__ dmask, const int32_t *__restrict__ cell_class, ApplyArgs a)
+{
+    apply_pack_body<FUSED, false>(lv, dmask, cell_class, a);
+}
+
+__global__ void __launch_bounds__(64, 4)
+k_apply_pack_rs(LevelDev lv, const uint16_t *__restrict__ dmask, const int32_t *__restrict__ cell_class, ApplyArgs a)
+{
+    apply_pack_body<true, true>(lv, dmask, cell_class, a);
+}
+
+bool apply_small_restricts(const Launch &L, const LevelDev &lv)
+{
+    return L.fold_restrict_small && L.apply_small && L.apply_threads == 0 && L.weight_cache && lv.wcache && lv.dim == 3 && lv.ncls == 15 &&
+           lv.nf <= 192 && lv.nf >= 4 && lv.m <= 63 && lv.pos32 && lv.lpos && lv.rptr && lv.ridx && lv.nf_coarse >= 1 &&
+           lv.nf_coarse <= ((lv.nf <= 16 && L.apply_pack) ? 16 : 64);
+}
+
 bool apply_small_ok(const Launch &L, const LevelDev &lv, const MeshDev &mesh, const ApplyArgs &a, bool fused)
 {
     if (!L.apply_small || L.apply_threads != 0) return false;
@@ -343,7 +443,9 @@
     if (lv.dim != 3 || lv.ncls != 15 || lv.nf > 192 || lv.nf < 4 || lv.m > 63 || !lv.pos32 || !lv.lpos) return false;
     if (a.flags & (2 | 8 | 16)) return false;
     if (!(a.alpha == 1.0 || a.alpha == -1.0) || a.lambda != mesh.wc_lambda) return false;
-    if (a.rcoarse) return false;
+    if (a.rcoarse && !(fused && a.src && !a.xcoarse && lv.rptr && lv.ridx && lv.nf_coarse >= 1 && lv.nf_coarse <= (lv.nf <= 16 ? 16 : 64) &&
+                       (!a.rcoarse2 || (lv.rs_bit && (a.flags & 1)))))
+        return false;
     if (!fused) return !a.xcoarse;
     if ((a.x3 || a.xacc) && !a.x2) return false;
     if (a.x3 && a.xacc) return false;
@@ -362,12 +464,19 @@
     if ((a.flags & 1) && !mesh.dmask) throw std::runtime_error("operator apply: constraint requested without a Dirichlet mask");
     if ((a.flags & 128) && !(fused && a.x3 && a.x2 && a.xout && !a.xcoarse))
         throw std::runtime_error("operator apply: the zero-input form exists for the residual with two pending x-updates only");
+    if (a.rcoarse && !(fused && a.ldrc > 0 && lv.rptr && lv.ridx && lv.nf_coarse >= 1 && lv.nf_coarse <= 64))
+        throw std::runtime_error("operator apply: epilogue restriction where the small-level kernels cannot take it");
+    if (a.rcoarse2 && !(a.rcoarse && lv.rs_bit && mesh.dmask && (a.flags & 1)))
+        throw std::runtime_error("operator apply: the constrained copy of the coarse column needs the epilogue restriction, its entity bits and the cell masks");
     a.nwork = nblocks;
     if (lv.nf <= 16 && L.apply_pack && nblocks >= 4 && nblocks < (int64_t(1) << 31)) {
         const int64_t nquad = (nblocks + 3) / 4;
         const dim3 gq((unsigned)std::min<int64_t>(nquad, (int64_t)16 * L.num_cu)), bq(64);
         const size_t ldsq = sizeof(double) * (size_t)(4 * (lv.lds_g0 + lv.nf + lv.lds_g1) + 64);
-        if (fused)
+        if (a.rcoarse) {
+            if (lv.nf_coarse > 16) throw std::runtime_error("operator apply: epilogue restriction of a packed level with more than 16 coarse slots");
+            hipLaunchKernelGGL(k_apply_pack_rs, gq, bq, ldsq + 16 * 8 * sizeof(uint32_t), L.stream, lv, mesh.dmask, mesh.cell_class, a);
+        } else if (fused)
             hipLaunchKernelGGL((k_apply_pack<true>), gq, bq, ldsq, L.stream, lv, mesh.dmask, mesh.cell_class, a);
         else
             hipLaunchKernelGGL((k_apply_pack<false>), gq, bq, ldsq, L.stream, lv, mesh.dmask, mesh.cell_class, a);
@@ -375,10 +484,15 @@
         if (L.n_small_launches) *L.n_small_launches += 1;
         return;
     }
-    const int64_t grid = std::min<int64_t>(nblocks, (int64_t)(lv.nf > 64 ? 16 : 20) * L.num_cu);
+    const int64_t grid = std::min<int64_t>(nblocks, (int64_t)(lv.nf > 64 || a.rcoarse ? 16 : 20) * L.num_cu);
     const size_t lds = sizeof(double) * (size_t)(SW + lv.lds_g0 + lv.nf + lv.lds_g1 + 64);
     const dim3 g((unsigned)grid), b(64);
-    if (lv.nf > 64) {
+    if (a.rcoarse) {
+        if (lv.nf > 64)
+            hipLaunchKernelGGL((k_apply_small_rs<3>), g, b, lds, L.stream, lv, mesh.dmask, mesh.cell_class, a);
+        else
+            hipLaunchKernelGGL((k_apply_small_rs<1>), g, b, lds, L.stream, lv, mesh.dmask, mesh.cell_class, a);
+    } else if (lv.nf > 64) {
         if (fused)
             hipLaunchKernelGGL((k_apply_small<3, true>), g, b, lds, L.stream, lv, mesh.dmask, mesh.cell_class, a);
         else
diff --git a/homogenization.jl_amd/csrc/hmg_apply_wave.hip b/homogenization.jl_amd/csrc/hmg_apply_wave.hip
--- a/homogenization.jl_amd/csrc/hmg_apply_wave.hip
+++ b/homogenization.jl_amd/csrc/hmg_apply_wave.hip
@@ -352,6 +352,12 @@
                         if (q < nv) xs[pos[q]] = ki[r][q];
                 }
             double *rc = a.rcoarse + cell * a.ldrc;
+            double *rc2 = a.rcoarse2 ? a.rcoarse2 + cell * a.ldrc : nullptr;
+            uint32_t dm2 = 0u;
+            if (rc2) {
+                const uint32_t w2 = HMG_KP(uint32_t, dmask)[cell >> 1];
+                dm2 = (cell & 1) ? w2 >> 16 : w2 & 0xffffu;
+            }
 #pragma unroll
             for (int q = 0; q < 3; ++q) {
                 const int c = lane + 64 * q;
@@ -368,6 +374,7 @@
                         tmp = u < n ? t2 : tmp;
                     }
                     rc[c] = tmp;
+                    if (rc2) rc2[c] = ((dm2 >> lv.rs_bit[c]) & 1u) ? 0.0 : tmp;
                 }
             }
         }
@@ -427,7 +434,7 @@
     if (a.xcoarse && a.rcoarse) return false;
     if ((a.x3 || a.xacc) && !(a.x2 && a.xout)) return false;
     if (a.xcoarse) return a.src && a.xout && lv.wave_par && lv.wave_cl && lv.nf_coarse == WNFC && !a.x2 && !a.xacc && !a.x3;
-    if (a.rcoarse) return a.src && lv.wave_rs && lv.nf_coarse == WNFC;
+    if (a.rcoarse) return a.src && lv.wave_rs && lv.nf_coarse == WNFC && (!a.rcoarse2 || lv.rs_bit);
     return true;
 }
 
@@ -442,6 +449,8 @@
     if ((a.flags & 1) && !mesh.dmask) throw std::runtime_error("operator apply: constraint requested without a Dirichlet mask");
     if (a.xcoarse && !a.xout) throw std::runtime_error("operator apply: folded prolongation without xout");
     if (a.rcoarse && a.ldrc <= 0) throw std::runtime_error("operator apply: epilogue restriction without the coarse column stride");
+    if (a.rcoarse2 && !(a.rcoarse && lv.rs_bit && mesh.dmask))
+        throw std::runtime_error("operator apply: the constrained copy of the coarse column needs the epilogue restriction, its entity bits and the cell masks");
     if ((a.flags & 128) && !(fused && a.x3 && a.x2 && a.xout && !a.xcoarse))
         throw std::runtime_error("operator apply: the zero-input form exists for the residual with two pending x-updates only");
     a.nwork = nblocks;
diff --git a/homogenization.jl_amd/csrc/hmg_context.cpp b/homogenization.jl_amd/csrc/hmg_context.cpp
--- a/homogenization.jl_amd/csrc/hmg_context.cpp
+++ b/homogenization.jl_amd/csrc/hmg_context.cpp
@@ -203,6 +203,7 @@
     c->L.restrict_slab2 = 1;
     c->L.apply_pack = 1;
     c->L.apply_small = 1;
+    c->L.fold_restrict_small = 1;
     c->L.n_small_launches = &c->small_launches;
     c->L.n_wc_launches = &c->wc_launches;
     c->L.apply_wg512 = 1;
@@ -255,6 +256,8 @@
     if (n == "lazy_top_form") return ctx->last_top_form;
     if (n == "lazy_pre_form") return ctx->last_pre_form;
     if (n == "coarse_x_folds") return ctx->coarse_x_folds;
+    if (n == "entry_folds") return ctx->last_entry_folds;
+    if (n == "restrict_folds") return ctx->last_restrict_folds;
     if (n == "cell_moments_kernel_ns") return ctx->moments_kernel_ns;
     if (n == "cell_moments_download_ns") return ctx->moments_download_ns;
     if (n == "comm_nranks") return ctx->comm ? ctx->comm_nranks : 0;
@@ -277,7 +280,7 @@
     static const std::pair<const char *, bool hmg_ctx::*> flags[] = {
         {"coarse_probe", &hmg_ctx::coarse_probe}, {"fuse_cg", &hmg_ctx::fuse_cg_default}, {"fold_x", &hmg_ctx::fold_x},
         {"swap_rp", &hmg_ctx::swap_rp}, {"fold_prolong", &hmg_ctx::fold_prolong}, {"zero_entry", &hmg_ctx::zero_entry},
-        {"fold_restrict", &hmg_ctx::fold_restrict}, {"lazy_dead", &hmg_ctx::lazy_dead}, {"lazy_pre", &hmg_ctx::lazy_pre}, {"fold_coarse_x", &hmg_ctx::fold_coarse_x}, {"fold_faces", &hmg_ctx::fold_faces},
+        {"fold_restrict", &hmg_ctx::fold_restrict}, {"fold_entry", &hmg_ctx::fold_entry}, {"lazy_dead", &hmg_ctx::lazy_dead}, {"lazy_pre", &hmg_ctx::lazy_pre}, {"fold_coarse_x", &hmg_ctx::fold_coarse_x}, {"fold_faces", &hmg_ctx::fold_faces},
         {"lean_post", &hmg_ctx::lean_post}, {"lazy_post", &hmg_ctx::lazy_post}, {"prolong_in_image", &hmg_ctx::prolong_in_image},
         {"comm_rehearsal", &hmg_ctx::comm_rehearsal}};
     for (const auto &f : flags)
@@ -291,6 +294,8 @@
         ctx->L.apply_wg512 = value != 0;
     else if (n == "apply_pack")
         ctx->L.apply_pack = value != 0;
+    else if (n == "fold_restrict_small")
+        ctx->L.fold_restrict_small = value != 0;
     else if (n == "apply_small")
         ctx->L.apply_small = value != 0;
     else if (n == "weight_cache")
diff --git a/homogenization.jl_amd/csrc/hmg_device.hpp b/homogenization.jl_amd/csrc/hmg_device.hpp
--- a/homogenization.jl_amd/csrc/hmg_device.hpp
+++ b/homogenization.jl_amd/csrc/hmg_device.hpp
@@ -53,6 +53,7 @@
     const uint32_t *rs_word;
     const double *rs_w;
     const uint16_t *rs_lp;
+    const uint8_t *rs_bit;
     const int32_t *rptr, *ridx;
     const double *dphi;
     const uint32_t *wave_tab;
@@ -126,6 +127,7 @@
     double *out;
     double *rcoarse;
     int64_t ldrc;
+    double *rcoarse2;
     const double *scal;
     int s_num, s_den;
     double *blockpart;
@@ -164,6 +166,7 @@
     int weight_cache;
     int apply_pack;
     int apply_small;
+    int fold_restrict_small;
     int64_t *n_small_launches;
     int64_t *n_wc_launches;
     int apply_wave;
@@ -195,6 +198,7 @@
                              double *xf);
 int64_t launch_norm2_unique_wide(const Launch &L, const LevelDev &lv, const MeshDev &mesh, const double *x);
 bool apply_small_ok(const Launch &L, const LevelDev &lv, const MeshDev &mesh, const ApplyArgs &a, bool fused);
+bool apply_small_restricts(const Launch &L, const LevelDev &lv);
 void launch_apply_small(const Launch &L, const LevelDev &lv, const MeshDev &mesh, const ApplyArgs &a, bool fused);
 void launch_weight_cache(const Launch &L, const LevelDev &lv, const double *coef_rep, int nclasses, double lambda, double *wcache);
 
@@ -204,7 +208,8 @@
 void launch_restrict_slab(const Launch &L, const LevelDev &fine_rtab, const MeshDev &mesh, const SlabTables &st, int ldc,
                           const double *rf, double *bc);
 void launch_restrict(const Launch &L, const LevelDev &fine, const LevelDev &coarse, int64_t ncells,
-                     const double *rf, double *bc);
+                     const double *rf, double *bc, double *bc2 = nullptr, const uint16_t *dmask = nullptr);
+bool restrict_masks(const LevelDev &fine);
 void launch_prolong_add(const Launch &L, const LevelDev &fine, const LevelDev &coarse, int64_t ncells,
                         const double *xc, double *xf);
 
diff --git a/homogenization.jl_amd/csrc/hmg_host.hpp b/homogenization.jl_amd/csrc/hmg_host.hpp
--- a/homogenization.jl_amd/csrc/hmg_host.hpp
+++ b/homogenization.jl_amd/csrc/hmg_host.hpp
@@ -174,6 +174,7 @@
     std::vector<uint32_t> rs_word;
     std::vector<double> rs_w;
     std::vector<uint16_t> rs_lp;
+    std::vector<uint8_t> rs_bit;
 };
 TransferTables build_transfer_tables(const LevelTables &T, const LevelTables *coarse, const BlockedInterior &blk);
 
diff --git a/homogenization.jl_amd/csrc/hmg_kernel_tables.cpp b/homogenization.jl_amd/csrc/hmg_kernel_tables.cpp
--- a/homogenization.jl_amd/csrc/hmg_kernel_tables.cpp
+++ b/homogenization.jl_amd/csrc/hmg_kernel_tables.cpp
@@ -233,6 +233,16 @@
             X.par32[q] = (uint32_t)T.par_a[q] | ((uint32_t)T.par_b[q] << 16);
         }
     }
+    if (coarse) {
+        const LevelTables &C = *coarse;
+        X.rs_bit.assign((size_t)C.nf, (uint8_t)31);
+        for (int c = 0; c < C.ncorner; ++c) X.rs_bit[(size_t)c] = (uint8_t)(C.nface + C.nedge + c);
+        for (int e = 0; e < C.nedge; ++e)
+            for (int q = 0; q < C.nei; ++q) X.rs_bit[(size_t)(C.off_edge + e * C.nei + q)] = (uint8_t)(C.nface + e);
+        for (int f = 0; f < C.nface; ++f)
+            for (int q = 0; q < C.nfi; ++q) X.rs_bit[(size_t)(C.off_face + f * C.nfi + q)] = (uint8_t)f;
+        if (C.nface + C.nedge + C.ncorner > 16) throw std::runtime_error("restriction tables: more entities than mask bits");
+    }
     if (!(coarse && T.dim == 3 && blk.nblk > 0 && T.nf <= 0xffff)) return X;
     const LevelTables &C = *coarse;
     const LatticeIndex fslot(T);
diff --git a/homogenization.jl_amd/csrc/hmg_kernels.hip b/homogenization.jl_amd/csrc/hmg_kernels.hip
--- a/homogenization.jl_amd/csrc/hmg_kernels.hip
+++ b/homogenization.jl_amd/csrc/hmg_kernels.hip
@@ -86,6 +86,10 @@
     }
     for (int q = tid; q < lv.lds_g0; q += NT) smem[WS + q] = 0.0;
     for (int q = tid; q < lv.lds_g1; q += NT) xs[nf + q] = 0.0;
+    if constexpr (RS && RB != 0) {
+        static_assert(WSZ_RB >= 64, "spare LDS entry behind the corners' rows");
+        if (tid == NT - 1) reinterpret_cast<unsigned long long *>(smem)[62] = (unsigned long long)(a.rcoarse2 ? a.rcoarse2 + cell * a.ldrc : nullptr);
+    }
     const int m = lv.m;
     constexpr int NW = NT / 64, WPF = NW / 4 > 0 ? NW / 4 : 1, NE = NW >= 6 ? 1 : 2;
     constexpr int FI = RB && NT == 512 ? 4 : 2;
@@ -607,6 +611,7 @@
         }
         __syncthreads();
         double *rc = a.rcoarse + cell * a.ldrc;
+        double *rc2 = reinterpret_cast<double *>((unsigned long long)__double_as_longlong(lds_ld(smem + 62)));
         if (lv.rs_lp) {
             for (int c = tid; c < lv.nf_coarse; c += NT) {
                 const int b = lv.rptr[c], n = lv.rptr[c + 1] - b;
@@ -619,6 +624,7 @@
                 for (int q = 1; q < 15; ++q)
                     if (q < n) tmp += 0.5 * lds_ld(xs + lp[q]);
                 rc[c] = tmp;
+                if (NT <= 256 && rc2) rc2[c] = ((dm >> lv.rs_bit[c]) & 1u) ? 0.0 : tmp;
             }
         } else
         for (int c = tid; c < lv.nf_coarse; c += NT) {
@@ -641,7 +647,9 @@
             acc += w[12] * at(-B);
             acc += w[13] * lds_ld(xs + L + A + 1 - len);
             acc += w[14] * at(len - B);
-            rc[c] = 0.0 + acc;
+            const double v = 0.0 + acc;
+            rc[c] = v;
+            if (rc2) rc2[c] = (cls > 0 && ((dm >> (cls - 1)) & 1u)) ? 0.0 : v;
         }
     }
     if (FUSED && !RS) {
@@ -904,6 +912,7 @@
 
 bool apply_restricts(const Launch &L, const LevelDev &lv)
 {
+    if (apply_small_restricts(L, lv)) return true;
     if (!(lv.dim == 3 && apply_lds_bytes(lv) <= 160 * 1024 && L.apply_threads == 0 && lv.rs_word &&
           lv.rs_w && lv.nf_coarse > 0 && lv.nei <= 64 && lv.nedge == 6 && lv.ncorner == 4))
         return false;
@@ -954,6 +963,8 @@
 {
     auto kern = k_apply<DIM, NT, SPT, FUSED, RB, WD, CG, RS, WC, LF>;
     if (a.rcoarse && !RS) throw std::runtime_error("operator apply: this instantiation cannot restrict in its epilogue");
+    if (a.rcoarse2 && !(a.rcoarse && lv.rs_bit && mesh.dmask && (a.flags & 1)))
+        throw std::runtime_error("operator apply: the constrained copy of the coarse column needs the epilogue restriction, its entity bits and the constraint (flags bit 0)");
     if (a.xc_p && !(CG && LF == 5)) throw std::runtime_error("operator apply: this instantiation cannot finish the coarse x");
     if (a.x4 && LF != 4) throw std::runtime_error("operator apply: this instantiation cannot carry a third pending x-update");
     if ((a.flags & 128) && !(FUSED && (RS || RB == 0)))
@@ -1407,7 +1418,7 @@
 
 template <int NT, bool USE_LDS>
 __global__ void __launch_bounds__(NT)
-k_restrict(LevelDev fine, int nfc, int ldc, const double *__restrict__ rf, double *bc)
+k_restrict(LevelDev fine, int nfc, int ldc, const double *__restrict__ rf, double *bc, double *bc2, const uint16_t *__restrict__ dmask)
 {
     extern __shared__ double smem[];
     const int64_t cell = blockIdx.x;
@@ -1432,6 +1443,8 @@
         fs = smem;
     }
     double *c = bc + cell * ldc;
+    double *c2 = bc2 ? bc2 + cell * ldc : nullptr;
+    const uint32_t dm2 = bc2 ? (uint32_t)dmask[cell] : 0u;
     for (int t = threadIdx.x; t < nfc; t += NT) {
         const int b = fine.rptr[t], n = fine.rptr[t + 1] - b;
         int idx[15];
@@ -1443,6 +1456,7 @@
         for (int q = 1; q < 15; ++q)
             if (q < n) tmp += 0.5 * fs[idx[q]];
         c[t] = tmp;
+        if (c2) c2[t] = ((dm2 >> fine.rs_bit[t]) & 1u) ? 0.0 : tmp;
     }
 }
 
@@ -1496,26 +1510,29 @@
     check_launch();
 }
 
+bool restrict_masks(const LevelDev &fine) { return fine.rs_bit != nullptr && sizeof(double) * (size_t)fine.nf <= 160 * 1024; }
+
 void launch_restrict(const Launch &L, const LevelDev &fine, const LevelDev &coarse, int64_t ncells,
-                     const double *rf, double *bc)
+                     const double *rf, double *bc, double *bc2, const uint16_t *dmask)
 {
     size_t lds = sizeof(double) * fine.nf;
+    if (bc2 && !(restrict_masks(fine) && dmask)) throw std::runtime_error("restriction: this level cannot write the constrained copy of the coarse column");
     if (fine.nf <= 256) {
         hipLaunchKernelGGL((k_restrict<64, true>), dim3((unsigned)ncells), dim3(64), lds, L.stream, fine, coarse.nf,
-                           coarse.ld, rf, bc);
+                           coarse.ld, rf, bc, bc2, dmask);
     } else if (lds <= 160 * 1024 && fine.nf > 2048) {
         auto k = k_restrict<1024, true>;
         if (lds > 48 * 1024)
             HMG_HIP_CHECK(hipFuncSetAttribute((const void *)k, hipFuncAttributeMaxDynamicSharedMemorySize, (int)lds));
-        hipLaunchKernelGGL(k, dim3((unsigned)ncells), dim3(1024), lds, L.stream, fine, coarse.nf, coarse.ld, rf, bc);
+        hipLaunchKernelGGL(k, dim3((unsigned)ncells), dim3(1024), lds, L.stream, fine, coarse.nf, coarse.ld, rf, bc, bc2, dmask);
     } else if (lds <= 160 * 1024) {
         auto k = k_restrict<256, true>;
         if (lds > 48 * 1024)
             HMG_HIP_CHECK(hipFuncSetAttribute((const void *)k, hipFuncAttributeMaxDynamicSharedMemorySize, (int)lds));
-        hipLaunchKernelGGL(k, dim3((unsigned)ncells), dim3(256), lds, L.stream, fine, coarse.nf, coarse.ld, rf, bc);
+        hipLaunchKernelGGL(k, dim3((unsigned)ncells), dim3(256), lds, L.stream, fine, coarse.nf, coarse.ld, rf, bc, bc2, dmask);
     } else {
         hipLaunchKernelGGL((k_restrict<256, false>), dim3((unsigned)ncells), dim3(256), 0, L.stream, fine, coarse.nf,
-                           coarse.ld, rf, bc);
+                           coarse.ld, rf, bc, bc2, dmask);
     }
     check_launch();
 }
diff --git a/homogenization.jl_amd/csrc/hmg_objects.hpp b/homogenization.jl_amd/csrc/hmg_objects.hpp
--- a/homogenization.jl_amd/csrc/hmg_objects.hpp
+++ b/homogenization.jl_amd/csrc/hmg_objects.hpp
@@ -103,6 +103,7 @@
     DevBuf<uint32_t> rs_word;
     DevBuf<double> rs_w;
     DevBuf<uint16_t> rs_lp;
+    DevBuf<uint8_t> rs_bit;
     DevBuf<uint16_t> blk_slot;
     DevBuf<uint32_t> wave_tab, wave_lpos, wave_par, wave_cl, wave_rs;
     DevBuf<double> wcache;
@@ -165,6 +166,7 @@
     int lazy_top = 2;
     bool zero_entry = true;
     bool fold_restrict = true;
+    bool fold_entry = true;
     bool prolong_in_image = true;
     int device = 0;
     hipStream_t stream = nullptr;
@@ -196,6 +198,8 @@
     int64_t smoother_diag_builds = 0;
     int64_t moments_kernel_ns = 0, moments_download_ns = 0;
     int64_t coarse_x_folds = 0;
+    int last_restrict_folds = 0;
+    int last_entry_folds = 0;
     int last_pre_form = 0;
     int last_top_form = 0;
     bool vec_pool_on = true;
@@ -351,7 +355,7 @@
 
 void set_slab(hmg_grid *g, const LevelDev &lv);
 void apply(hmg_grid *g, const LevelDev &lv, double alpha, const double *x, const double *src, double *out, int mask);
-void restrict_level(hmg_grid *g, int level_fine, const double *rf, double *bc);
+void restrict_level(hmg_grid *g, int level_fine, const double *rf, double *bc, double *bc2 = nullptr);
 void interface_sum(hmg_grid *g, const LevelDev &lv, double *x, bool faces = true);
 void scalar_sum(hmg_grid *g, int slot, int count);
 bool reserve_top_spare(hmg_grid *g, bool must);
diff --git a/homogenization.jl_amd/csrc/hmg_smooth.cpp b/homogenization.jl_amd/csrc/hmg_smooth.cpp
--- a/homogenization.jl_amd/csrc/hmg_smooth.cpp
+++ b/homogenization.jl_amd/csrc/hmg_smooth.cpp
@@ -63,10 +63,16 @@
     tr.stop();
 }
 
-void restrict_level(hmg_grid *g, int level_fine, const double *rf, double *bc)
+static bool restrict_level_masks(const hmg_grid *g, int level_fine)
+{
+    return !g->lb[(size_t)level_fine - 1]->slab_rs_head.p && g->md.dmask && restrict_masks(g->ld[(size_t)level_fine - 1]);
+}
+
+void restrict_level(hmg_grid *g, int level_fine, const double *rf, double *bc, double *bc2)
 {
     const LevelDev &fine = lev(g, level_fine), &coarse = lev(g, level_fine - 1);
     const LevelBufs &B = *g->lb[level_fine - 1];
+    need(!bc2 || restrict_level_masks(g, level_fine), "restriction: this level cannot write the constrained copy of the coarse column");
     if (B.slab_rs_head.p) {
         LevelDev fr = fine;
         fr.ctab = B.rtab.p;
@@ -82,7 +88,7 @@
         launch_restrict_slab(g->ctx->L, fr, g->md, st, coarse.ld, rf, bc);
         return;
     }
-    launch_restrict(g->ctx->L, fine, coarse, g->md.ncells, rf, bc);
+    launch_restrict(g->ctx->L, fine, coarse, g->md.ncells, rf, bc, bc2, bc2 ? g->md.dmask : nullptr);
 }
 
 void interface_sum(hmg_grid *g, const LevelDev &lv, double *x, bool faces)
@@ -225,6 +231,7 @@
     Tail tail = Tail::Full;
     bool hand_up = false;
     bool x_zero = false;
+    bool r_ready = false;
 };
 
 struct DeferredX {
@@ -373,8 +380,10 @@
         a.flags = 1;
         if (f.x_zero) {
             need(!xcoarse, "zero initial guess with a coarse-grid correction");
-            launch_copy(L, r->d, b->d, n);
-            launch_mask(L, lv, g->md, r->d, 0);
+            if (!f.r_ready) {
+                launch_copy(L, r->d, b->d, n);
+                launch_mask(L, lv, g->md, r->d, 0);
+            }
             interface_sum(g, lv, r->d);
         } else if (xcoarse) {
             a.xcoarse = xcoarse->d;
@@ -602,17 +611,22 @@
     return true;
 }
 
-int vcycle_down(hmg_grid *g, int k, int steps, hmg_vec **st, bool inside = false, bool x_zero = false, int steps_next = -1)
+int vcycle_down(hmg_grid *g, int k, int steps, hmg_vec **st, bool inside = false, bool x_zero = false, int steps_next = -1,
+                bool r_ready = false, bool *r_delivered = nullptr)
 {
     hmg_vec **cur = st + 5 * (k - 1);
     hmg_vec **nxt = st + 5 * (k - 2);
     const Launch &L = g->ctx->L;
     SmoothForm form = smooth_form(g, k, steps, Role::Pre);
     need(!x_zero || form.tail == Tail::DeadDefer2, "zero initial guess: the pre-smoother does not defer both x-updates");
+    need(!r_ready || x_zero, "a first residual delivered from above belongs to the zero initial guess");
     form.x_zero = x_zero;
+    form.r_ready = r_ready;
     const DeferredX dx = smooth(g, k, steps, cur[0], cur[1], cur[2], cur[3], cur[4], form);
     const int deferred = dx.rs < 0 ? 0 : dx.three_updates ? 3 : dx.two_updates ? 2 : 1;
     const bool skip_fill = inside && steps_next >= 0 && zero_entry_ok(g, k - 1, steps_next);
+    const bool may_deliver = r_delivered && skip_fill && k - 1 >= 2 && g->ctx->fold_entry && g->ctx->fold_restrict && g->md.dmask;
+    if (r_delivered) *r_delivered = false;
     if (dx.rs >= 0) {
         ApplyArgs a{};
         a.alpha = -1.0;
@@ -645,6 +659,11 @@
             if (inside) a.out = nullptr;
             a.rcoarse = nxt[1]->d;
             a.ldrc = lev(g, k - 1).ld;
+            if (may_deliver && lev(g, k).rs_bit) {
+                a.rcoarse2 = nxt[2]->d;
+                *r_delivered = true;
+            }
+            if (inside && apply_small_restricts(L, lev(g, k))) g->ctx->last_restrict_folds += 1;
             apply_then_sum(g, lev(g, k), a, true, -1, -1, false);
             if (!skip_fill) launch_fill(L, nxt[0]->d, vec_len(nxt[0]), 0.0);
             return deferred;
@@ -653,7 +672,11 @@
     } else {
         apply(g, lev(g, k), -1.0, cur[0]->d, cur[1]->d, cur[2]->d, 1);
     }
-    restrict_level(g, k, cur[2]->d, nxt[1]->d);
+    if (may_deliver && restrict_level_masks(g, k)) {
+        restrict_level(g, k, cur[2]->d, nxt[1]->d, nxt[2]->d);
+        *r_delivered = true;
+    } else
+        restrict_level(g, k, cur[2]->d, nxt[1]->d);
     if (!skip_fill) launch_fill(L, nxt[0]->d, vec_len(nxt[0]), 0.0);
     return deferred;
 }
@@ -683,7 +706,8 @@
     return apply_folds_coarse_x(c->L, lv) && smooth_form(g, k - 1, steps_below, Role::PostBelow).tail == Tail::DeadX2;
 }
 
-DeferredX vcycle_level(hmg_grid *g, int k, int steps, int steps_coarse, hmg_vec **st, bool top, bool zero_guess, bool hand_up)
+DeferredX vcycle_level(hmg_grid *g, int k, int steps, int steps_coarse, hmg_vec **st, bool top, bool zero_guess, bool hand_up,
+                       bool r_ready = false)
 {
     if (k == 1) {
         hmg_vec **cur = st;
@@ -692,9 +716,12 @@
     }
     const bool x_zero = (zero_guess || !top) && zero_entry_ok(g, k, steps);
     if (top && zero_guess && !x_zero) launch_fill(g->ctx->L, st[5 * (k - 1)]->d, vec_len(st[5 * (k - 1)]), 0.0);
-    const int deferred = vcycle_down(g, k, steps, st, true, x_zero, steps_coarse);
+    need(!r_ready || x_zero, "a first residual delivered to a level that is not entered with the unwritten zero guess");
+    bool delivered = false;
+    const int deferred = vcycle_down(g, k, steps, st, true, x_zero, steps_coarse, r_ready, &delivered);
     if (top) g->ctx->last_pre_form = deferred;
-    const DeferredX cx = vcycle_level(g, k - 1, steps_coarse, steps_coarse, st, false, false, coarse_x_folds(g, k, steps_coarse));
+    if (delivered) g->ctx->last_entry_folds += 1;
+    const DeferredX cx = vcycle_level(g, k - 1, steps_coarse, steps_coarse, st, false, false, coarse_x_folds(g, k, steps_coarse), delivered);
     if (top) g->ctx->last_top_form = 0;
     return vcycle_up(g, k, steps, st, top ? Role::PostTop : Role::PostBelow, &cx, hand_up);
 }
@@ -703,6 +730,7 @@
 
 void vcycle(hmg_grid *g, int k, int steps, int steps_coarse, hmg_vec **st, bool top, bool zero_guess)
 {
+    g->ctx->last_entry_folds = g->ctx->last_restrict_folds = 0;
     (void)vcycle_level(g, k, steps, steps_coarse, st, top, zero_guess, false);
 }
 
diff --git a/homogenization.jl_amd/csrc/hmg_upload.cpp b/homogenization.jl_amd/csrc/hmg_upload.cpp
--- a/homogenization.jl_amd/csrc/hmg_upload.cpp
+++ b/homogenization.jl_amd/csrc/hmg_upload.cpp
@@ -117,6 +117,7 @@
         B.rptr.upload(T.rptr, s);
         B.ridx.upload(T.ridx, s);
         B.dphi.upload(T.dphi, s);
+        if (g->ctx) B.rs_bit.upload(X.rs_bit, s);
         B.nslab = sw.nslab;
         B.slab_lds_nodes = sw.lds_nodes;
         B.slab_max_surf = sw.max_surf;
@@ -165,6 +166,7 @@
         D.rs_word = B.rs_word.p;
         D.rs_w = B.rs_w.p;
         D.rs_lp = B.rs_lp.p;
+        D.rs_bit = B.rs_bit.p;
         D.rptr = B.rptr.p;
         D.ridx = B.ridx.p;
         D.dphi = B.dphi.p;
```

Measured after the change: 11.49 billion fine-DOF updates/s, median of 6. About the same (+0.7%).
